# RaptorMai/online-continual-learning

Measured on AMD Instinct MI355X. Metric: replay-step images/sec (SCR, Split-CIFAR100-shaped synthetic stream, Reduced-ResNet18, mem_size 5000), higher is better.
Workload: dtype f32; 1 GPU; BASELINE.json configs[1]: agent=SCR, data=cifar100, eps_mem_batch=100, head=mlp, mem_size=5000, retrieve=random, temp=0.07, update=random; stream_batch=10, parallelism=1 independent stream(s), one per GPU

## Files before the change

include/ocl_hip.h:

```cpp
#ifndef OCL_HIP_H
#define OCL_HIP_H

#include <stdint.h>

#ifdef __cplusplus
extern "C" {
#endif

#define OCL_OK 0
#define OCL_ERR_ARG (-1)
#define OCL_ERR_HIP (-2)
#define OCL_ERR_STATE (-3)
#define OCL_ERR_UNSUPPORTED (-4)

int ocl_version(void);
const char* ocl_last_error(void);
int ocl_init(int device);

int ocl_gather_rows(const void* src, const int64_t* idx, int64_t n, int64_t row_bytes, void* dst,
                    void* stream);
int ocl_scatter_rows(void* dst, const int64_t* idx, int64_t n, int64_t row_bytes, const void* src,
                     void* stream);
int ocl_gather_rows_pair(const void* src_a, int64_t row_bytes_a, void* dst_a, const void* src_b, int64_t row_bytes_b, void* dst_b,
                         const int64_t* idx_host, int64_t* idx_dev, int64_t n, void* stream);
// ... 101 lines not shown
                    const float* gamma, int64_t m_per_group, int groups, int c, float* dy, float* dgamma,
                    float* dbeta, int accumulate, double* scratch, void* stream);

#define OCL_EPI_STATS 1
#define OCL_EPI_AFFINE 2
#define OCL_EPI_RES 4
#define OCL_EPI_RESMASK 8
#define OCL_EPI_RELU 16
#define OCL_EPI_ACCUM 32
#define OCL_EPI_BNB 64

typedef struct {
    int32_t cin, cout, k, stride, hin, win;
    int32_t n, groups, dir, merge, xf, bnb;
    int32_t force_mt, force_nt, force_pipe, force_q4, force_cs, force_cw;
} ocl_test_conv_desc;
typedef struct {
    int32_t family, mt, nt, q4, pipe, wres, ncls, pf, bnb_room, grid_x, grid_y, reserved;
} ocl_test_conv_form;
int ocl_test_conv_plan(const ocl_test_conv_desc* desc, ocl_test_conv_form* forms, int cap);
typedef struct {
    const float* in;
    const float* w;
    float* out;
    int32_t flags;
    int32_t xf;
    const float *scale, *shift, *res, *resmask;
    void* stats;
    const void* xf_stats;
    const float *xf_gamma, *xf_beta;
    float *xf_save_mean, *xf_save_invstd, *xf_running_mean, *xf_running_var;
    int64_t* xf_nbt;
    const float *bnb_y, *bnb_z, *bnb_mean, *bnb_invstd, *bnb_gamma, *bnb_beta;
} ocl_test_conv_ops;
int ocl_test_conv(const ocl_test_conv_desc* desc, const ocl_test_conv_ops* ops, ocl_test_conv_form* forms, int cap, void* stream);

typedef struct {
    int32_t cin, cout, k, stride, hin, win, n, xf_groups, wg_target, reserved;
} ocl_test_wgrad_desc;
typedef struct {
    int32_t mtw, ntw, q_rgw, pf, multi, s, grid_x, grid_y;
} ocl_test_wgrad_form;
typedef struct {
    const float* x;
    const float* dy;
    float* grad;
    int32_t xf;
    int32_t reserved;
    const float *xf_mean, *xf_invstd, *xf_gamma, *xf_beta;
} ocl_test_wgrad_ops;
int ocl_test_wgrad(const ocl_test_wgrad_desc* descs, const ocl_test_wgrad_ops* ops, int n_layers, int multi, int accumulate,
                   ocl_test_wgrad_form* forms, void* stream);

typedef struct {
    const float* y; float* z; const float* res; const void* stats;
    const float *gamma, *beta; float *running_mean, *running_var; int64_t* nbt; float *save_mean, *save_invstd;
    const float *frozen_mean, *frozen_var;
    const float* yb; const void* stats_b; const float *gamma_b, *beta_b; float *running_mean_b, *running_var_b; int64_t* nbt_b;
    float *save_mean_b, *save_invstd_b; const float *frozen_mean_b, *frozen_var_b;
    int64_t m_per_group; int32_t groups, c, relu; float momentum, eps; int32_t reserved;
} ocl_test_bn_fwd_args;
int ocl_test_bn_fwd(const ocl_test_bn_fwd_args* a, void* stream);
typedef struct {
    const float* dz; const float* z;
    const float* y[2]; const float* mean[2]; const float* invstd[2]; const float* gamma[2]; const float* beta[2];
    float* dy[2]; float* dgamma[2]; float* dbeta[2];
    int64_t m_per_group; int32_t groups, c, nsets, accumulate, frozen, mask_from_y, one_pass, reserved;
} ocl_test_bn_bwd_args;
int ocl_test_bn_bwd(const ocl_test_bn_bwd_args* a, void* stream);
int ocl_test_bn_apply_e(const float* d, const float* y, const float* mean, const float* invstd, const float* gamma, const void* esums,
                        int64_t m_per_group, int groups, int c, float* dy, float* dgamma, float* dbeta, int accumulate, void* stream);

typedef struct {
    int32_t layer, dir, wg_merged, reserved;
    ocl_test_conv_desc desc;
    ocl_test_conv_form form;
    ocl_test_wgrad_desc wdesc;
    ocl_test_wgrad_form wform;
} ocl_test_net_form;
int ocl_test_net_forms(int hw, int nf, int n, int groups, int train, ocl_test_net_form* out, int cap);

enum {
    OCL_SOP_ROWS = 0, OCL_SOP_PAIR = 1, OCL_SOP_U8 = 2, OCL_SOP_SGD = 3, OCL_SOP_COSINE = 4, OCL_SOP_CE = 5, OCL_SOP_CE_SEG = 6,
    OCL_SOP_KD = 7, OCL_SOP_MIR = 8, OCL_SOP_SUPCON = 9, OCL_SOP_KNN = 10, OCL_SOP_COL_REDUCE = 11, OCL_SOP_ASER = 12,
    OCL_SOP_ARGSORT = 13, OCL_SOP_NCM_MEANS = 14, OCL_SOP_NCM_PREDICT = 15, OCL_SOP_GEMM = 16
};
enum {
    OCL_PATH_ROWS_COPY16 = 1,
    OCL_PATH_ROWS_COPY16_YCAP = 2,
    OCL_PATH_ROWS_COPY4 = 3,
    OCL_PATH_ROWS_COPY4_YCAP = 4,
    OCL_PATH_PAIR_FUSED = 5,
    OCL_PATH_PAIR_FUSED_BLOOP = 6,
    OCL_PATH_PAIR_FALLBACK = 7,
    OCL_PATH_U8_GATHER = 8,
    OCL_PATH_SGD_VEC = 9,
    OCL_PATH_SGD_TAIL = 10,
    OCL_PATH_SGD_GRID_CAP = 11,
    OCL_PATH_SGD_REFUSED = 12,
    OCL_PATH_COS_VEC_ONE = 13,
    OCL_PATH_COS_VEC_MULTI = 14,
    OCL_PATH_COS_VEC_CAP = 15,
    OCL_PATH_COS_SCALAR_ONE = 16,
    OCL_PATH_COS_SCALAR_MULTI = 17,
// ... 51 lines not shown
```

online-continual-learning_amd/csrc/conv.h:

```cpp
#pragma once
#include "common.h"
#include <vector>

namespace ocl {

constexpr int kStatReps = 8;

struct alignas(16) StatCell {
    unsigned long long lo;
    long long hi;
};

enum ConvEpi : int {
    EPI_STORE = 0,
    EPI_STATS = 1,
    EPI_AFFINE = 2,
    EPI_RES = 4,
    EPI_RESMASK = 8,
    EPI_RELU = 16,
    EPI_ACCUM = 32,
    EPI_BNB = 64,
};

struct ConvArgs {
// ... 22 lines not shown
    int n_splits;
    const float* wT;
    int C4tot, WPT;
    int Qc, Qpad;
    int QS, nstage, wres;
    int pipe;
    int aligned;
    int cls_pack, cls_oyx;
    unsigned m_tpg, m_tpi, m_lw, m_ppi, m_kc4, m_pc, m_pr;
    int xf;
    int patch_floats;
    int qstat_off;
    const StatCell* xf_stats;
    int64_t xf_rep_stride;
    int64_t xf_m_per_group;
    const float* xf_gamma;
    const float* xf_beta;
    float* xf_save_mean;
    float* xf_save_invstd;
    float* xf_running_mean;
    float* xf_running_var;
    int64_t* xf_nbt;
    float xf_momentum, xf_eps;
    const float* bnb_y;
    const float* bnb_z;
    const float* bnb_mean;
    const float* bnb_invstd;
    const float* bnb_gamma;
    const float* bnb_beta;
    int bnb_lds;
    const int* blob;
    int off_tdesc, off_pu, off_loc, blob_ints;
    unsigned long long* trace;
};

struct ConvPlan {
    ConvArgs a;
    int cs;
    int cw;
    int q4;
    int MT, NT;
    int grid_x, grid_y;
    size_t lds_bytes;
    hipEvent_t ready;
    hipStream_t ready_stream;
};

struct ConvGeomDesc {
    int N, groups;
    int Hin, Win, Cin;
    int Hout, Wout, Cout;
    int LH, LW, os, oy0, ox0, is;
    int ntaps;
    int tdy[9], tdx[9], tw[9];
    int force_MT, force_NT, force_bpc;
    int force_cs;
    int force_q4;
    int force_pipe;
    int force_cw;
    int WPT;
    int xf;
    int bnb;
    int ncls;
    int cls_ntaps[4], cls_oy[4], cls_ox[4];
};

// ... 111 lines not shown
constexpr int kMaxInputSegments = 8;
struct InputSegments {
    const float* x[kMaxInputSegments];
    int first[kMaxInputSegments];
    int n;
};
int launch_nchw3_to_nhwc4_segments(const InputSegments& sg, float* out, int N, int H, int W, hipStream_t s);

struct BnFwdArgs {
    const float* y;
    float* z;
    const float* res;
    const StatCell* stats;
    int64_t stat_rep_stride;
    const float* gamma;
    const float* beta;
    float* running_mean;
    float* running_var;
    int64_t* nbt;
    float* save_mean;
    float* save_invstd;
    int64_t m_per_group;
    int G, C, relu;
    float momentum, eps;
    const float* frozen_mean;
    const float* frozen_var;
    const float* yb;
    const StatCell* stats_b;
    const float *gamma_b, *beta_b;
    float *running_mean_b, *running_var_b;
    int64_t* nbt_b;
    float *save_mean_b, *save_invstd_b;
    const float *frozen_mean_b, *frozen_var_b;
};
int launch_bn_fwd(const BnFwdArgs& a, hipStream_t s);
int launch_bn_apply_saved(const float* y, const float* mean, const float* invstd, const float* gamma, const float* beta, float* z,
                          int64_t m_per_group, int G, int C, hipStream_t s);

struct BnFoldDesc {
    int64_t gamma_off, beta_off, stat_off, out_off;
    int C;
};
int launch_bn_fold(const float* params, const float* running, float* out, const BnFoldDesc* descs_dev, int n_bn, float eps,
                   hipStream_t s);

struct BnBwdArgs {
    const float* dz;
    const float* z;
    int64_t m_per_group;
    int G, C;
    int nsets;
    const float* y[2];
    const float* mean[2];
    const float* invstd[2];
    const float* gamma[2];
    float* dy[2];
    float* dgamma[2];
    float* dbeta[2];
    StatCell* sums;
    unsigned* barrier;
    StatCell* fsums;
    StatCell* fsums_b;
    int accumulate;
    unsigned* err;
    int frozen;
    int mask_from_y;
    const float* beta[2];
};
int launch_bn_bwd(const BnBwdArgs& a, hipStream_t s);
struct BnApplyEArgs {
    const float* d;
    const float* y;
    const float* mean;
    const float* invstd;
    const float* gamma;
    float* dy;
    float* dgamma;
    float* dbeta;
    const StatCell* esums;
    int64_t esums_rep_stride;
    int64_t m_per_group;
    int G, C, accumulate;
};
int launch_bn_apply_e(const BnApplyEArgs& a, hipStream_t s);
int bn_bwd_last_path();
void bn_bwd_tune(int block_cap, int unroll, int phase);
void bn_bwd_fused_enable(int on);

int launch_avgpool_fwd(const float* z, float* feat, int N, int H, int W, int C, hipStream_t s);
int launch_avgpool_bwd(const float* dfeat, float* dz, int N, int H, int W, int C, hipStream_t s);

int launch_l2norm_fwd(const float* v, float* out, float* norms, int n, int d, hipStream_t s, float* out2 = nullptr);
int launch_l2norm_bwd(const float* out, const float* norms, const float* dout, float* dv, int n, int d, hipStream_t s);
int launch_relu_bwd(const float* dy, const float* a, float* dx, int64_t n, hipStream_t s);
int launch_colsum(const float* m, int rows, int cols, float* out, int accumulate, hipStream_t s);
int launch_fill(float* p, int64_t n, float v, hipStream_t s);

ConvShape test_conv_shape(const ocl_test_conv_desc& d);
void test_conv_form(const ConvPlan& p, ocl_test_conv_form* f);
void test_wgrad_form(const WgradPlan& p, ocl_test_wgrad_form* f);

int conv_kernels_init();
int wgrad_kernels_init();
int set_deterministic_sums(int on);

}
```

online-continual-learning_amd/csrc/conv.hip:

```cpp
#include "conv_dev.h"
#include "conv_stats_dev.h"
#include <string.h>
#include <algorithm>
#include <type_traits>
#include <cmath>

namespace ocl {




static const int kMaxDevices = 64;
static int g_det_dev[kMaxDevices] = {0};
static int det_host() {
    int dev = 0;
    if (hipGetDevice(&dev) != hipSuccess || dev < 0 || dev >= kMaxDevices) return 0;
    return g_det_dev[dev];
}
int set_deterministic_sums(int on) {
    const int v = on ? 1 : 0;
    int dev = 0;
    OCL_HIP(hipGetDevice(&dev));
    OCL_REQUIRE(dev >= 0 && dev < kMaxDevices, "set_deterministic: device %d", dev);
    OCL_HIP(hipDeviceSynchronize());
// ... 516 lines not shown
                    if (pv_ok && co < a.Cout) {
                        const float4 v = make_float4(acc[mt][nt][0], acc[mt][nt][1], acc[mt][nt][2], acc[mt][nt][3]);
                        s1[mt][0] += v.x; s1[mt][1] += v.y; s1[mt][2] += v.z; s1[mt][3] += v.w;
                        s2[mt][0] = fmaf(v.x, v.x, s2[mt][0]); s2[mt][1] = fmaf(v.y, v.y, s2[mt][1]);
                        s2[mt][2] = fmaf(v.z, v.z, s2[mt][2]); s2[mt][3] = fmaf(v.w, v.w, s2[mt][3]);
                        *(float4*)(a.out + (int64_t)ooff[nt] + ct.z + co) = v;
                    }
                }
            }
        } else
#pragma unroll
        for (int nt = 0; nt < NT; ++nt) {
            const bool pv_ok = ooff[nt] >= 0;
#pragma unroll
            for (int mt = 0; mt < MT; ++mt) {
                const int co = n0 + mt * 16 + 4 * g;
                if (!pv_ok || co >= a.Cout) continue;
                float4 v = make_float4(acc[mt][nt][0], acc[mt][nt][1], acc[mt][nt][2], acc[mt][nt][3]);
                if (flags & EPI_STATS) {
                    s1[mt][0] += v.x; s1[mt][1] += v.y; s1[mt][2] += v.z; s1[mt][3] += v.w;
                    s2[mt][0] = fmaf(v.x, v.x, s2[mt][0]); s2[mt][1] = fmaf(v.y, v.y, s2[mt][1]);
                    s2[mt][2] = fmaf(v.z, v.z, s2[mt][2]); s2[mt][3] = fmaf(v.w, v.w, s2[mt][3]);
                }
                float* op = a.out + (int64_t)ooff[nt] + ct.z + co;
                if (flags & EPI_AFFINE) {
                    const float4 sc = *(const float4*)(a.scale + co), sh = *(const float4*)(a.shift + co);
                    v.x = fmaf(v.x, sc.x, sh.x); v.y = fmaf(v.y, sc.y, sh.y); v.z = fmaf(v.z, sc.z, sh.z); v.w = fmaf(v.w, sc.w, sh.w);
                }
                if (flags & EPI_RES) {
                    const float4 r = *(const float4*)(a.res + (int64_t)ooff[nt] + ct.z + co);
                    v.x += r.x; v.y += r.y; v.z += r.z; v.w += r.w;
                }
                if (flags & EPI_RESMASK) {
                    const float4 r = *(const float4*)(a.res + (int64_t)ooff[nt] + ct.z + co);
                    const float4 m = *(const float4*)(a.resmask + (int64_t)ooff[nt] + ct.z + co);
                    v.x += m.x > 0.f ? r.x : 0.f; v.y += m.y > 0.f ? r.y : 0.f; v.z += m.z > 0.f ? r.z : 0.f; v.w += m.w > 0.f ? r.w : 0.f;
                }
                if (flags & EPI_ACCUM) {
                    const float4 o = *(const float4*)op;
                    v.x += o.x; v.y += o.y; v.z += o.z; v.w += o.w;
                }
                if (BNB && (flags & EPI_BNB)) {
                    const int64_t eo = (int64_t)ooff[nt] + ct.z + co;
                    const float* t = bnt + (size_t)(d1.y * (a.Cout >> 2) + (co >> 2)) * 12;
                    bnb_apply(a, *(const float4*)t, *(const float4*)(t + 4), *(const float4*)(t + 8), eo, v, s1[mt], s2[mt]);
                }
                if (flags & EPI_RELU) {
                    v.x = fmaxf(v.x, 0.f); v.y = fmaxf(v.y, 0.f); v.z = fmaxf(v.z, 0.f); v.w = fmaxf(v.w, 0.f);
                }
                *(float4*)op = v;
            }
        }
        }
        stamp();
    }
    if ((flags & (EPI_STATS | EPI_BNB)) && run_grp >= 0) flush_stats();
    stamp();
}


template <int NTQ, int PF, int STATS, int TRACE = 0>
__global__ void __launch_bounds__(256, 2) conv_q_kernel(const ConvArgs a) {
    extern __shared__ __attribute__((aligned(16))) unsigned char lds_raw[];
    constexpr int MB = kQBlocks, COPW = 4 * MB;
    int* tdesc = (int*)lds_raw;
    int* ctab = tdesc + kMaxWgTiles * 8;
    int* qoff = ctab + 16;
    int* qrow = qoff + a.Qpad;
    float* wl = (float*)(qrow + a.Qpad);
// ... 223 lines not shown
                    float t1 = 0.f, t2 = 0.f;
#pragma unroll
                    for (int nt = 0; nt < NTQ; ++nt) {
                        const float v = ooff[nt] >= 0 ? acc[m][nt][e] : 0.f;
                        t1 += v;
                        t2 = fmaf(v, v, t2);
                    }
                    t1 = row16_sum(t1);
                    t2 = row16_sum(t2);
                    if ((lane & 15) == 0) {
                        rw[m * 4 + e] = t1;
                        rw[COPW + m * 4 + e] = t2;
                    }
                }
            if (lane < 2 * COPW) {
                const float* r0 = qrows + (size_t)(wave * 4) * 2 * COPW + lane;
                qacc[wave * 2 * COPW + lane] += (r0[0] + r0[2 * COPW]) + (r0[4 * COPW] + r0[6 * COPW]);
            }
        }
        auto epi_one = [&](int nt, int m, float (&b1)[4], float (&b2)[4]) __attribute__((always_inline)) {
            const int co = 4 * m;
            if (ooff[nt] < 0 || co >= a.Cout) return;
            float4 v = make_float4(acc[m][nt][0], acc[m][nt][1], acc[m][nt][2], acc[m][nt][3]);
            float* op = a.out + (int64_t)ooff[nt] + co;
            if (flags & EPI_AFFINE) {
                const float4 sc = *(const float4*)(a.scale + co), sh = *(const float4*)(a.shift + co);
                v.x = fmaf(v.x, sc.x, sh.x); v.y = fmaf(v.y, sc.y, sh.y); v.z = fmaf(v.z, sc.z, sh.z); v.w = fmaf(v.w, sc.w, sh.w);
            }
            if (flags & EPI_RES) {
                const float4 r = *(const float4*)(a.res + (int64_t)ooff[nt] + co);
                v.x += r.x; v.y += r.y; v.z += r.z; v.w += r.w;
            }
            if (flags & EPI_RESMASK) {
                const float4 r = *(const float4*)(a.res + (int64_t)ooff[nt] + co);
                const float4 mk = *(const float4*)(a.resmask + (int64_t)ooff[nt] + co);
                v.x += mk.x > 0.f ? r.x : 0.f; v.y += mk.y > 0.f ? r.y : 0.f; v.z += mk.z > 0.f ? r.z : 0.f; v.w += mk.w > 0.f ? r.w : 0.f;
            }
            if (flags & EPI_ACCUM) {
                const float4 o = *(const float4*)op;
                v.x += o.x; v.y += o.y; v.z += o.z; v.w += o.w;
            }
            if (STATS == 2 && (flags & EPI_BNB)) {
                const float* t = bnt + (size_t)(d1.y * (a.Cout >> 2) + m) * 12;
                bnb_apply(a, *(const float4*)t, *(const float4*)(t + 4), *(const float4*)(t + 8), (int64_t)ooff[nt] + co, v, b1, b2);
            }
            if (flags & EPI_RELU) {
                v.x = fmaxf(v.x, 0.f); v.y = fmaxf(v.y, 0.f); v.z = fmaxf(v.z, 0.f); v.w = fmaxf(v.w, 0.f);
            }
            *(float4*)op = v;
        };
        if (STATS == 2 && (flags & EPI_BNB)) {
            float* rw = qrows + (size_t)(wave * 4 + (lane >> 4)) * 2 * COPW;
#pragma unroll
            for (int m = 0; m < MB; ++m) {
                float b1[4] = {0.f, 0.f, 0.f, 0.f}, b2[4] = {0.f, 0.f, 0.f, 0.f};
#pragma unroll
                for (int nt = 0; nt < NTQ; ++nt) epi_one(nt, m, b1, b2);
#pragma unroll
                for (int e = 0; e < 4; ++e) {
                    const float r1 = row16_sum(b1[e]), r2 = row16_sum(b2[e]);
                    if ((lane & 15) == 0) {
                        rw[m * 4 + e] = r1;
                        rw[COPW + m * 4 + e] = r2;
                    }
                }
            }
            if (lane < 2 * COPW) {
                const float* r0 = qrows + (size_t)(wave * 4) * 2 * COPW + lane;
                qacc[wave * 2 * COPW + lane] += (r0[0] + r0[2 * COPW]) + (r0[4 * COPW] + r0[6 * COPW]);
// ... 220 lines not shown
        const float* rj = patch0 + (size_t)(wave * 64 + lane) * 4;
        const size_t ws = (size_t)a.patch_floats;
        const float4 p0 = *(const float4*)(rj), p1 = *(const float4*)(rj + ws);
        const float4 p2 = *(const float4*)(rj + 2 * ws), p3 = *(const float4*)(rj + 3 * ws);
        v = make_float4((p0.x + p1.x) + (p2.x + p3.x), (p0.y + p1.y) + (p2.y + p3.y), (p0.z + p1.z) + (p2.z + p3.z), (p0.w + p1.w) + (p2.w + p3.w));
    }
    int oo = ooff[0];
#pragma unroll
    for (int nt = 1; nt < NT; ++nt) oo = wave == nt ? ooff[nt] : oo;
    const int co = n0 + 4 * g;
    const bool live = oo >= 0 && co < a.Cout;
    if (flags & EPI_STATS) {
        const float4 z = live ? v : make_float4(0.f, 0.f, 0.f, 0.f);
        const float s1x = row16_sum(z.x), s1y = row16_sum(z.y), s1z = row16_sum(z.z), s1w = row16_sum(z.w);
        const float s2x = row16_sum(z.x * z.x), s2y = row16_sum(z.y * z.y), s2z = row16_sum(z.z * z.z), s2w = row16_sum(z.w * z.w);
        if (r16 < 8 && co < a.Cout) {
            const int j = r16;
            const float v = j == 0 ? s1x : j == 1 ? s1y : j == 2 ? s1z : j == 3 ? s1w : j == 4 ? s2x : j == 5 ? s2y : j == 6 ? s2z : s2w;
            StatCell* st_ = a.stats + (int64_t)((blockIdx.x + blockIdx.y + wave) % kStatReps) * a.stat_rep_stride + ((int64_t)d1.y * 2) * a.Cout + co;
            fx_add<FXM>(st_ + (j >> 2) * a.Cout + (j & 3), (double)v);
        }
    }
    float* op = a.out + (int64_t)oo + co;
    if (live) {
        if (flags & EPI_AFFINE) {
            const float4 sc = *(const float4*)(a.scale + co), sh = *(const float4*)(a.shift + co);
            v.x = fmaf(v.x, sc.x, sh.x); v.y = fmaf(v.y, sc.y, sh.y); v.z = fmaf(v.z, sc.z, sh.z); v.w = fmaf(v.w, sc.w, sh.w);
        }
        if (flags & EPI_RES) {
            const float4 r = *(const float4*)(a.res + (int64_t)oo + co);
            v.x += r.x; v.y += r.y; v.z += r.z; v.w += r.w;
        }
        if (flags & EPI_RESMASK) {
            const float4 r = *(const float4*)(a.res + (int64_t)oo + co);
            const float4 mk = *(const float4*)(a.resmask + (int64_t)oo + co);
            v.x += mk.x > 0.f ? r.x : 0.f; v.y += mk.y > 0.f ? r.y : 0.f; v.z += mk.z > 0.f ? r.z : 0.f; v.w += mk.w > 0.f ? r.w : 0.f;
        }
        if (flags & EPI_ACCUM) {
            const float4 o = *(const float4*)op;
            v.x += o.x; v.y += o.y; v.z += o.z; v.w += o.w;
        }
    }
    if (BNB && (flags & EPI_BNB)) {
        float b1[4] = {0.f, 0.f, 0.f, 0.f}, b2[4] = {0.f, 0.f, 0.f, 0.f};
        if (live) {
            const int j = d1.y * a.Cout + co;
            const float4 mu = *(const float4*)(a.bnb_mean + j);
            float4 sc = make_float4(0.f, 0.f, 0.f, 0.f), sh = sc;
            if (!a.bnb_z) {
                const float4 is = *(const float4*)(a.bnb_invstd + j), gm = *(const float4*)(a.bnb_gamma + co), bt = *(const float4*)(a.bnb_beta + co);
                bn_scale_shift(gm.x, bt.x, mu.x, is.x, sc.x, sh.x); bn_scale_shift(gm.y, bt.y, mu.y, is.y, sc.y, sh.y);
                bn_scale_shift(gm.z, bt.z, mu.z, is.z, sc.z, sh.z); bn_scale_shift(gm.w, bt.w, mu.w, is.w, sc.w, sh.w);
            }
            bnb_apply(a, sc, sh, mu, (int64_t)oo + co, v, b1, b2);
        }
        const float s1x = row16_sum(b1[0]), s1y = row16_sum(b1[1]), s1z = row16_sum(b1[2]), s1w = row16_sum(b1[3]);
        const float s2x = row16_sum(b2[0]), s2y = row16_sum(b2[1]), s2z = row16_sum(b2[2]), s2w = row16_sum(b2[3]);
        if (r16 < 8 && co < a.Cout) {
            const int j = r16;
            const float v = j == 0 ? s1x : j == 1 ? s1y : j == 2 ? s1z : j == 3 ? s1w : j == 4 ? s2x : j == 5 ? s2y : j == 6 ? s2z : s2w;
            StatCell* st_ = a.stats + (int64_t)((blockIdx.x + blockIdx.y + wave) % kStatReps) * a.stat_rep_stride + ((int64_t)d1.y * 2) * a.Cout + co;
            fx_add<FXM>(st_ + (j >> 2) * a.Cout + (j & 3), (double)v);
        }
    }
    if (!live) return;
    if (flags & EPI_RELU) {
        v.x = fmaxf(v.x, 0.f); v.y = fmaxf(v.y, 0.f); v.z = fmaxf(v.z, 0.f); v.w = fmaxf(v.w, 0.f);
    }
    *(float4*)op = v;
// ... 848 lines not shown
            a.save_mean[(int64_t)g * a.C + c] = (float)mean;
            a.save_invstd[(int64_t)g * a.C + c] = (float)invstd;
        }
    }
    if (blockIdx.x == 0 && g == 0 && a.running_mean)
        bn_running_update(a.stats, a.stat_rep_stride, a.G, a.C, M, a.momentum, a.eps, a.running_mean, a.running_var, a.nbt, tid, 256);
    float* scb = sm + 2 * a.C;
    float* shb = sm + 3 * a.C;
    if (a.yb) {
        for (int c = tid; c < a.C; c += 256) {
            double mean, var;
            bn_batch_moments(a.stats_b, a.stat_rep_stride, g, c, a.C, M, a.eps, mean, var);
            if (a.frozen_mean_b) {
                mean = (double)a.frozen_mean_b[c];
                var = (double)a.frozen_var_b[c];
            }
            const double invstd = 1.0 / sqrt(var + (double)a.eps);
            bn_scale_shift(a.gamma_b[c], a.beta_b[c], (float)mean, (float)invstd, scb[c], shb[c]);
            if (blockIdx.x == 0) {
                a.save_mean_b[(int64_t)g * a.C + c] = (float)mean;
                a.save_invstd_b[(int64_t)g * a.C + c] = (float)invstd;
            }
        }
        if (blockIdx.x == 0 && g == 0 && a.running_mean_b)
            bn_running_update(a.stats_b, a.stat_rep_stride, a.G, a.C, M, a.momentum, a.eps, a.running_mean_b, a.running_var_b, a.nbt_b, tid, 256);
    }
    __syncthreads();
    const int C4 = a.C >> 2;
    const int64_t units = a.m_per_group * C4;
    const float4* y4 = (const float4*)a.y + (int64_t)g * units;
    const float4* b4 = a.yb ? (const float4*)a.yb + (int64_t)g * units : nullptr;
    const float4* r4 = a.res ? (const float4*)a.res + (int64_t)g * units : nullptr;
    float4* z4 = (float4*)a.z + (int64_t)g * units;
    for (int64_t u = (int64_t)blockIdx.x * 256 + tid; u < units; u += (int64_t)gridDim.x * 256) {
        const int c = (int)(u % C4) * 4;
        float4 v = y4[u];
        v.x = __fmaf_rn(v.x, sc[c], sh[c]);
        v.y = __fmaf_rn(v.y, sc[c + 1], sh[c + 1]);
        v.z = __fmaf_rn(v.z, sc[c + 2], sh[c + 2]);
        v.w = __fmaf_rn(v.w, sc[c + 3], sh[c + 3]);
        if (r4) {
            const float4 r = r4[u];
            v.x += r.x; v.y += r.y; v.z += r.z; v.w += r.w;
        }
        if (b4) {
            float4 r = b4[u];
            r.x = __fmaf_rn(r.x, scb[c], shb[c]);
            r.y = __fmaf_rn(r.y, scb[c + 1], shb[c + 1]);
            r.z = __fmaf_rn(r.z, scb[c + 2], shb[c + 2]);
            r.w = __fmaf_rn(r.w, scb[c + 3], shb[c + 3]);
            v.x += r.x; v.y += r.y; v.z += r.z; v.w += r.w;
        }
        if (a.relu) {
            v.x = fmaxf(v.x, 0.f); v.y = fmaxf(v.y, 0.f); v.z = fmaxf(v.z, 0.f); v.w = fmaxf(v.w, 0.f);
        }
        z4[u] = v;
    }
}

int launch_bn_fwd(const BnFwdArgs& a, hipStream_t s) {
    const int64_t units = a.m_per_group * (a.C / 4);
    const int bx = (int)std::max<int64_t>(1, std::min<int64_t>(1024, (units + 1023) / 1024));
    ProfScope ps(PROF_BN, s);
    hipLaunchKernelGGL(bn_fwd_kernel, dim3(bx, a.G), dim3(256), (size_t)a.C * (a.yb ? 16 : 8), s, a);
    OCL_LAUNCH_CHECK();
    return OCL_OK;
}

__global__ void __launch_bounds__(256) bn_apply_saved_kernel(const float* __restrict__ y, const float* __restrict__ mean, const float* __restrict__ invstd,
                                                             const float* __restrict__ gamma, const float* __restrict__ beta, float* __restrict__ z,
                                                             int64_t m_per_group, int C) {
    const int g = blockIdx.y, C4 = C >> 2;
    const int64_t units = m_per_group * C4;
    for (int64_t u = (int64_t)blockIdx.x * 256 + threadIdx.x; u < units; u += (int64_t)gridDim.x * 256) {
        const int c = (int)(u % C4) * 4;
        float4 v = ((const float4*)y)[(int64_t)g * units + u];
        float o[4] = {v.x, v.y, v.z, v.w};
#pragma unroll
        for (int e = 0; e < 4; ++e) {
            float sc, sh;
            bn_scale_shift(gamma[c + e], beta[c + e], mean[(int64_t)g * C + c + e], invstd[(int64_t)g * C + c + e], sc, sh);
            o[e] = fmaxf(__fmaf_rn(o[e], sc, sh), 0.f);
        }
        ((float4*)z)[(int64_t)g * units + u] = make_float4(o[0], o[1], o[2], o[3]);
    }
}
int launch_bn_apply_saved(const float* y, const float* mean, const float* invstd, const float* gamma, const float* beta, float* z,
                          int64_t m_per_group, int G, int C, hipStream_t s) {
    const int64_t units = m_per_group * (C / 4);
    const int bx = (int)std::max<int64_t>(1, std::min<int64_t>(1024, (units + 1023) / 1024));
    hipLaunchKernelGGL(bn_apply_saved_kernel, dim3(bx, G), dim3(256), 0, s, y, mean, invstd, gamma, beta, z, m_per_group, C);
    OCL_LAUNCH_CHECK();
    return OCL_OK;
}

__global__ void __launch_bounds__(256) bn_fold_kernel(const float* __restrict__ params, const float* __restrict__ running,
                                                      float* __restrict__ out, const BnFoldDesc* __restrict__ descs, float eps) {
    const BnFoldDesc d = descs[blockIdx.x];
    for (int c = threadIdx.x; c < d.C; c += 256) {
        const float rm = running[d.stat_off + c], rv = running[d.stat_off + d.C + c];
        const float invstd = (float)(1.0 / sqrt((double)rv + (double)eps));
        const float scale = params[d.gamma_off + c] * invstd;
        out[d.out_off + c] = scale;
        out[d.out_off + d.C + c] = params[d.beta_off + c] - rm * scale;
    }
}
int launch_bn_fold(const float* params, const float* running, float* out, const BnFoldDesc* descs_dev, int n_bn, float eps,
                   hipStream_t s) {
    ProfScope ps(PROF_BN, s);
    hipLaunchKernelGGL(bn_fold_kernel, dim3(n_bn), dim3(256), 0, s, params, running, out, descs_dev, eps);
    OCL_LAUNCH_CHECK();
    return OCL_OK;
}

template <int U>
__global__ void __launch_bounds__(256) bn_bwd_reduce_kernel(const BnBwdArgs a) {
    extern __shared__ __attribute__((aligned(16))) float sm[];
    const int C4 = a.C >> 2;
    const int PT = 256 / C4;
    const int tid = threadIdx.x;
    const int c4 = tid % C4, pl = tid / C4;
    const int g = blockIdx.y;
    const int64_t M = a.m_per_group;
    const int64_t per = (M + gridDim.x - 1) / gridDim.x;
    const int64_t pbeg = (int64_t)blockIdx.x * per, pend = min(M, pbeg + per);
    float4 sd[2], sx[2];
    float4 mean[2], istd[2];
#pragma unroll
    for (int k = 0; k < 2; ++k) {
        sd[k] = sx[k] = make_float4(0.f, 0.f, 0.f, 0.f);
        mean[k] = istd[k] = make_float4(0.f, 0.f, 0.f, 0.f);
    }
    if (pl < PT) {
#pragma unroll
        for (int k = 0; k < 2; ++k)
            if (k < a.nsets) {
                mean[k] = *(const float4*)(a.mean[k] + (int64_t)g * a.C + c4 * 4);
                istd[k] = *(const float4*)(a.invstd[k] + (int64_t)g * a.C + c4 * 4);
            }
        const float4* dz4 = (const float4*)a.dz + (int64_t)g * M * C4;
        const float4* z4 = a.z ? (const float4*)a.z + (int64_t)g * M * C4 : nullptr;
        const float4* y40 = (const float4*)a.y[0] + (int64_t)g * M * C4;
        const float4* y41 = a.nsets > 1 ? (const float4*)a.y[1] + (int64_t)g * M * C4 : y40;
        const int64_t step = (int64_t)PT * C4;
        const int64_t eend = pend * C4;
        int64_t e = (pbeg + pl) * C4 + c4;
        float4 msc = make_float4(0.f, 0.f, 0.f, 0.f), msh = msc;
        if (a.mask_from_y) {
            const float4 gm = *(const float4*)(a.gamma[0] + c4 * 4), bt = *(const float4*)(a.beta[0] + c4 * 4);
            bn_scale_shift(gm.x, bt.x, mean[0].x, istd[0].x, msc.x, msh.x); bn_scale_shift(gm.y, bt.y, mean[0].y, istd[0].y, msc.y, msh.y);
            bn_scale_shift(gm.z, bt.z, mean[0].z, istd[0].z, msc.z, msh.z); bn_scale_shift(gm.w, bt.w, mean[0].w, istd[0].w, msc.w, msh.w);
        }
        auto consume = [&](float4 d, float4 zz, const float4& ya, const float4& yb) __attribute__((always_inline)) {
            if (a.mask_from_y)
                zz = make_float4(__fmaf_rn(ya.x, msc.x, msh.x), __fmaf_rn(ya.y, msc.y, msh.y), __fmaf_rn(ya.z, msc.z, msh.z), __fmaf_rn(ya.w, msc.w, msh.w));
            if (z4 || a.mask_from_y) {
                d.x = zz.x > 0.f ? d.x : 0.f; d.y = zz.y > 0.f ? d.y : 0.f;
                d.z = zz.z > 0.f ? d.z : 0.f; d.w = zz.w > 0.f ? d.w : 0.f;
            }
#pragma unroll
            for (int k = 0; k < 2; ++k)
                if (k < a.nsets) {
                    const float4& y = k ? yb : ya;
                    sd[k].x += d.x; sd[k].y += d.y; sd[k].z += d.z; sd[k].w += d.w;
                    sx[k].x = fmaf(d.x, (y.x - mean[k].x) * istd[k].x, sx[k].x);
                    sx[k].y = fmaf(d.y, (y.y - mean[k].y) * istd[k].y, sx[k].y);
                    sx[k].z = fmaf(d.z, (y.z - mean[k].z) * istd[k].z, sx[k].z);
                    sx[k].w = fmaf(d.w, (y.w - mean[k].w) * istd[k].w, sx[k].w);
                }
        };
        const float4 zero4 = make_float4(0.f, 0.f, 0.f, 0.f);
        for (; e + (U - 1) * step < eend; e += U * step) {
            float4 d[U], zz[U], ya[U], yb[U];
#pragma unroll
            for (int u = 0; u < U; ++u) {
                d[u] = dz4[e + u * step];
                zz[u] = z4 ? z4[e + u * step] : zero4;
                ya[u] = y40[e + u * step];
                yb[u] = a.nsets > 1 ? y41[e + u * step] : zero4;
            }
#pragma unroll
            for (int u = 0; u < U; ++u) consume(d[u], zz[u], ya[u], yb[u]);
        }
        for (; e < eend; e += step)
            consume(dz4[e], z4 ? z4[e] : zero4, y40[e], a.nsets > 1 ? y41[e] : zero4);
    }
    float* base = sm;
    if (pl < PT) {
#pragma unroll
        for (int k = 0; k < 2; ++k)
            if (k < a.nsets) {
                *(float4*)(base + ((size_t)(k * 2 + 0) * PT + pl) * a.C + c4 * 4) = sd[k];
                *(float4*)(base + ((size_t)(k * 2 + 1) * PT + pl) * a.C + c4 * 4) = sx[k];
            }
    }
    __syncthreads();
    for (int j = tid; j < a.nsets * 2 * a.C; j += 256) {
        const int c = j % a.C, kk = j / a.C;
        double t = 0.0;
        for (int r = 0; r < PT; ++r) t += (double)base[((size_t)kk * PT + r) * a.C + c];
        const int k = kk >> 1, which = kk & 1;
        fx_add(&a.sums[(((int64_t)k * a.G + g) * 2 + which) * a.C + c], t);
    }
}

__global__ void __launch_bounds__(256) bn_bwd_apply_kernel(const BnBwdArgs a) {
    extern __shared__ __attribute__((aligned(16))) float sm[];
    const int g = blockIdx.y, tid = threadIdx.x;
    const double Md = (double)a.m_per_group;
    for (int j = tid; j < a.nsets * a.C; j += 256) {
        const int c = j % a.C, k = j / a.C;
        const StatCell cdy = a.sums[(((int64_t)k * a.G + g) * 2 + 0) * a.C + c], cdx = a.sums[(((int64_t)k * a.G + g) * 2 + 1) * a.C + c];
        const double sdy = fx_decode(cdy.hi, cdy.lo), sdx = fx_decode(cdx.hi, cdx.lo);
        float* s = sm + (size_t)k * 6 * a.C;
        const float istd = a.invstd[k][(int64_t)g * a.C + c];
        s[c] = a.frozen ? 0.f : (float)(sdy / Md);
        s[a.C + c] = a.frozen ? 0.f : (float)(sdx / Md);
        s[2 * a.C + c] = a.gamma[k][c] * istd;
        s[3 * a.C + c] = a.mean[k][(int64_t)g * a.C + c];
        s[4 * a.C + c] = istd;
        if (a.mask_from_y) {
            float sc_, sh_;
            bn_scale_shift(a.gamma[k][c], a.beta[k][c], a.mean[k][(int64_t)g * a.C + c], istd, sc_, sh_);
            s[5 * a.C + c] = sh_;
        }
        if (blockIdx.x == 0 && g == 0) {
            double dg = 0.0, db = 0.0;
            for (int gg = 0; gg < a.G; ++gg) {
                const StatCell cb = a.sums[(((int64_t)k * a.G + gg) * 2 + 0) * a.C + c], cg = a.sums[(((int64_t)k * a.G + gg) * 2 + 1) * a.C + c];
                db += fx_decode(cb.hi, cb.lo);
                dg += fx_decode(cg.hi, cg.lo);
            }
            if (a.accumulate) {
                a.dgamma[k][c] += (float)dg;
                a.dbeta[k][c] += (float)db;
            } else {
                a.dgamma[k][c] = (float)dg;
                a.dbeta[k][c] = (float)db;
            }
        }
    }
    __syncthreads();
    const int C4 = a.C >> 2;
    const int64_t units = a.m_per_group * C4;
    for (int64_t u = (int64_t)blockIdx.x * 256 + tid; u < units; u += (int64_t)gridDim.x * 256) {
        const int c = (int)(u % C4) * 4;
        const int64_t e = (int64_t)g * units + u;
        float4 d = ((const float4*)a.dz)[e];
        if (a.z) {
            const float4 zz = ((const float4*)a.z)[e];
            d.x = zz.x > 0.f ? d.x : 0.f; d.y = zz.y > 0.f ? d.y : 0.f;
            d.z = zz.z > 0.f ? d.z : 0.f; d.w = zz.w > 0.f ? d.w : 0.f;
        } else if (a.mask_from_y) {
            const float4 y = ((const float4*)a.y[0])[e];
            d.x = __fmaf_rn(y.x, sm[2 * a.C + c], sm[5 * a.C + c]) > 0.f ? d.x : 0.f;
            d.y = __fmaf_rn(y.y, sm[2 * a.C + c + 1], sm[5 * a.C + c + 1]) > 0.f ? d.y : 0.f;
            d.z = __fmaf_rn(y.z, sm[2 * a.C + c + 2], sm[5 * a.C + c + 2]) > 0.f ? d.z : 0.f;
            d.w = __fmaf_rn(y.w, sm[2 * a.C + c + 3], sm[5 * a.C + c + 3]) > 0.f ? d.w : 0.f;
        }
#pragma unroll
        for (int k = 0; k < 2; ++k)
            if (k < a.nsets) {
                const float* s = sm + (size_t)k * 6 * a.C;
                const float4 y = ((const float4*)a.y[k])[e];
                float4 o;
                o.x = s[2 * a.C + c] * (d.x - s[c] - (y.x - s[3 * a.C + c]) * s[4 * a.C + c] * s[a.C + c]);
                o.y = s[2 * a.C + c + 1] * (d.y - s[c + 1] - (y.y - s[3 * a.C + c + 1]) * s[4 * a.C + c + 1] * s[a.C + c + 1]);
                o.z = s[2 * a.C + c + 2] * (d.z - s[c + 2] - (y.z - s[3 * a.C + c + 2]) * s[4 * a.C + c + 2] * s[a.C + c + 2]);
                o.w = s[2 * a.C + c + 3] * (d.w - s[c + 3] - (y.w - s[3 * a.C + c + 3]) * s[4 * a.C + c + 3] * s[a.C + c + 3]);
                ((float4*)a.dy[k])[e] = o;
            }
    }
}

constexpr int kBnFusedThreads = 512;
constexpr int kBnFusedReps = 8;
#ifndef OCL_BN_FLAT
#define OCL_BN_FLAT 40
#endif
constexpr int kBnFusedFlat = OCL_BN_FLAT;
template <int E, int NS = 1>
__global__ void __launch_bounds__(kBnFusedThreads) bn_bwd_fused_kernel(const BnBwdArgs a) {
    __shared__ float4 red[1 + NS][kBnFusedThreads];
    __shared__ float kk[1 + NS][4 * 40];
    __shared__ bool timed_out;
    const int C4 = a.C >> 2;
    const int tid = threadIdx.x;
    if (tid == 0) timed_out = false;
    const int wpg = gridDim.x / a.G;
    const int g = blockIdx.x / wpg;
    const int S = (wpg * kBnFusedThreads / C4) * C4;
    const int gt = (blockIdx.x - g * wpg) * kBnFusedThreads + tid;
    const int c4 = gt % C4;
    const int64_t M = a.m_per_group;
    const int64_t units = M * C4;
    const float4* dz4 = (const float4*)a.dz + (int64_t)g * units;
    const float4* z4 = a.z ? (const float4*)a.z + (int64_t)g * units : nullptr;
    const bool live = g < a.G && gt < S;
    float4 d[E], xh[NS][E];
    float4 sd = make_float4(0.f, 0.f, 0.f, 0.f), sx[NS];
#pragma unroll
    for (int k = 0; k < NS; ++k) sx[k] = sd;
    if (live) {
        float4 zz[E];
#pragma unroll
        for (int e = 0; e < E; ++e) {
            const int64_t u = (int64_t)gt + (int64_t)e * S;
            const bool in = u < units;
            const int64_t uu = in ? u : 0;
            d[e] = dz4[uu];
#pragma unroll
            for (int k = 0; k < NS; ++k) xh[k][e] = ((const float4*)a.y[k] + (int64_t)g * units)[uu];
            zz[e] = z4 ? z4[uu] : make_float4(1.f, 1.f, 1.f, 1.f);
            if (!in) d[e] = make_float4(0.f, 0.f, 0.f, 0.f);
        }
        if (a.mask_from_y) {
            const float4 gm = *(const float4*)(a.gamma[0] + c4 * 4), bt = *(const float4*)(a.beta[0] + c4 * 4);
            const float4 mn = *(const float4*)(a.mean[0] + (int64_t)g * a.C + c4 * 4), is = *(const float4*)(a.invstd[0] + (int64_t)g * a.C + c4 * 4);
            float4 sc, sh;
            bn_scale_shift(gm.x, bt.x, mn.x, is.x, sc.x, sh.x); bn_scale_shift(gm.y, bt.y, mn.y, is.y, sc.y, sh.y);
            bn_scale_shift(gm.z, bt.z, mn.z, is.z, sc.z, sh.z); bn_scale_shift(gm.w, bt.w, mn.w, is.w, sc.w, sh.w);
#pragma unroll
            for (int e = 0; e < E; ++e)
                zz[e] = make_float4(__fmaf_rn(xh[0][e].x, sc.x, sh.x), __fmaf_rn(xh[0][e].y, sc.y, sh.y), __fmaf_rn(xh[0][e].z, sc.z, sh.z),
                                    __fmaf_rn(xh[0][e].w, sc.w, sh.w));
        }
#pragma unroll
        for (int e = 0; e < E; ++e) {
            d[e].x = zz[e].x > 0.f ? d[e].x : 0.f; d[e].y = zz[e].y > 0.f ? d[e].y : 0.f;
            d[e].z = zz[e].z > 0.f ? d[e].z : 0.f; d[e].w = zz[e].w > 0.f ? d[e].w : 0.f;
            sd.x += d[e].x; sd.y += d[e].y; sd.z += d[e].z; sd.w += d[e].w;
        }
#pragma unroll
        for (int k = 0; k < NS; ++k) {
            const float4 mean = *(const float4*)(a.mean[k] + (int64_t)g * a.C + c4 * 4);
            const float4 istd = *(const float4*)(a.invstd[k] + (int64_t)g * a.C + c4 * 4);
#pragma unroll
            for (int e = 0; e < E; ++e) {
                xh[k][e].x = (xh[k][e].x - mean.x) * istd.x; xh[k][e].y = (xh[k][e].y - mean.y) * istd.y;
                xh[k][e].z = (xh[k][e].z - mean.z) * istd.z; xh[k][e].w = (xh[k][e].w - mean.w) * istd.w;
                sx[k].x = fmaf(d[e].x, xh[k][e].x, sx[k].x); sx[k].y = fmaf(d[e].y, xh[k][e].y, sx[k].y);
                sx[k].z = fmaf(d[e].z, xh[k][e].z, sx[k].z); sx[k].w = fmaf(d[e].w, xh[k][e].w, sx[k].w);
            }
        }
    }
    red[0][tid] = sd;
// ... 67 lines not shown
            const float4 istd = *(const float4*)(a.invstd[k] + (int64_t)g * a.C + c4 * 4);
            const float4 sc = make_float4(gm.x * istd.x, gm.y * istd.y, gm.z * istd.z, gm.w * istd.w);
            float4* o4 = (float4*)a.dy[k] + (int64_t)g * units;
#pragma unroll
            for (int e = 0; e < E; ++e) {
                const int64_t u = (int64_t)gt + (int64_t)e * S;
                if (u < units) {
                    float4 o;
                    o.x = sc.x * (d[e].x - k1.x - xh[k][e].x * k2.x);
                    o.y = sc.y * (d[e].y - k1.y - xh[k][e].y * k2.y);
                    o.z = sc.z * (d[e].z - k1.z - xh[k][e].z * k2.z);
                    o.w = sc.w * (d[e].w - k1.w - xh[k][e].w * k2.w);
                    o4[u] = o;
                }
            }
        }
    }
}

constexpr int kBnChanThreads = 512;
template <int E, int NS>
__global__ void __launch_bounds__(kBnChanThreads) bn_bwd_chan_kernel(const BnBwdArgs a) {
    constexpr int NW = kBnChanThreads / 64;
    __shared__ double wred[1 + NS][4][NW];
    __shared__ double tot[2][1 + NS][4];
    __shared__ float kk[2][1 + NS][4];
    const int c4 = blockIdx.x, tid = threadIdx.x, lane = tid & 63, wave = tid >> 6;
    const int C4 = a.C >> 2;
    const int T = kBnChanThreads / a.G;
    const int g = tid / T, pt = tid - g * T;
    const int64_t M = a.m_per_group;
    const float4 f4z = make_float4(0.f, 0.f, 0.f, 0.f);
    const int64_t base = (int64_t)g * M * C4 + c4;
    float4 d[E], xh[NS][E], zz[E];
    float4 sd = f4z, sx[NS];
#pragma unroll
    for (int k = 0; k < NS; ++k) sx[k] = f4z;
#pragma unroll
    for (int e = 0; e < E; ++e) {
        const int64_t pix = pt + (int64_t)e * T;
        const bool in = pix < M;
        const int64_t u = base + (in ? pix : 0) * C4;
        d[e] = ((const float4*)a.dz)[u];
#pragma unroll
        for (int k = 0; k < NS; ++k) xh[k][e] = ((const float4*)a.y[k])[u];
        zz[e] = a.z ? ((const float4*)a.z)[u] : make_float4(1.f, 1.f, 1.f, 1.f);
        if (!in) d[e] = f4z;
    }
    if (a.mask_from_y) {
        const float4 gm = *(const float4*)(a.gamma[0] + c4 * 4), bt = *(const float4*)(a.beta[0] + c4 * 4);
        const float4 mn = *(const float4*)(a.mean[0] + (int64_t)g * a.C + c4 * 4), is = *(const float4*)(a.invstd[0] + (int64_t)g * a.C + c4 * 4);
        float4 sc, sh;
        bn_scale_shift(gm.x, bt.x, mn.x, is.x, sc.x, sh.x); bn_scale_shift(gm.y, bt.y, mn.y, is.y, sc.y, sh.y);
        bn_scale_shift(gm.z, bt.z, mn.z, is.z, sc.z, sh.z); bn_scale_shift(gm.w, bt.w, mn.w, is.w, sc.w, sh.w);
#pragma unroll
        for (int e = 0; e < E; ++e)
            zz[e] = make_float4(__fmaf_rn(xh[0][e].x, sc.x, sh.x), __fmaf_rn(xh[0][e].y, sc.y, sh.y), __fmaf_rn(xh[0][e].z, sc.z, sh.z),
                                __fmaf_rn(xh[0][e].w, sc.w, sh.w));
    }
#pragma unroll
    for (int e = 0; e < E; ++e) {
        d[e].x = zz[e].x > 0.f ? d[e].x : 0.f; d[e].y = zz[e].y > 0.f ? d[e].y : 0.f;
        d[e].z = zz[e].z > 0.f ? d[e].z : 0.f; d[e].w = zz[e].w > 0.f ? d[e].w : 0.f;
        sd.x += d[e].x; sd.y += d[e].y; sd.z += d[e].z; sd.w += d[e].w;
    }
#pragma unroll
    for (int k = 0; k < NS; ++k) {
        const float4 mean = *(const float4*)(a.mean[k] + (int64_t)g * a.C + c4 * 4);
        const float4 istd = *(const float4*)(a.invstd[k] + (int64_t)g * a.C + c4 * 4);
#pragma unroll
        for (int e = 0; e < E; ++e) {
            xh[k][e].x = (xh[k][e].x - mean.x) * istd.x; xh[k][e].y = (xh[k][e].y - mean.y) * istd.y;
            xh[k][e].z = (xh[k][e].z - mean.z) * istd.z; xh[k][e].w = (xh[k][e].w - mean.w) * istd.w;
            sx[k].x = fmaf(d[e].x, xh[k][e].x, sx[k].x); sx[k].y = fmaf(d[e].y, xh[k][e].y, sx[k].y);
            sx[k].z = fmaf(d[e].z, xh[k][e].z, sx[k].z); sx[k].w = fmaf(d[e].w, xh[k][e].w, sx[k].w);
        }
    }
    auto wsum = [&](float v) __attribute__((always_inline)) -> double {
        double t = (double)v;
// ... 40 lines not shown
#pragma unroll
    for (int k = 0; k < NS; ++k) {
        const float4 k2 = *(const float4*)&kk[g][1 + k][0];
        const float4 gm = *(const float4*)(a.gamma[k] + c4 * 4);
        const float4 istd = *(const float4*)(a.invstd[k] + (int64_t)g * a.C + c4 * 4);
        const float4 sc = make_float4(gm.x * istd.x, gm.y * istd.y, gm.z * istd.z, gm.w * istd.w);
#pragma unroll
        for (int e = 0; e < E; ++e) {
            const int64_t pix = pt + (int64_t)e * T;
            if (pix < M) {
                float4 o;
                o.x = sc.x * (d[e].x - k1.x - xh[k][e].x * k2.x);
                o.y = sc.y * (d[e].y - k1.y - xh[k][e].y * k2.y);
                o.z = sc.z * (d[e].z - k1.z - xh[k][e].z * k2.z);
                o.w = sc.w * (d[e].w - k1.w - xh[k][e].w * k2.w);
                ((float4*)a.dy[k])[base + pix * C4] = o;
            }
        }
    }
}

static int g_bn_bwd_cap = 0, g_bn_bwd_unroll = 0, g_bn_bwd_phase = 0;
void bn_bwd_tune(int cap, int unroll, int phase) { g_bn_bwd_cap = cap; g_bn_bwd_unroll = unroll; g_bn_bwd_phase = phase; }

static int g_bn_fused = -1;
static int g_num_cus = 0;
void bn_bwd_fused_enable(int on) { g_bn_fused = on; }

static int g_bn_bwd_last_path = 0;
int bn_bwd_last_path() { return g_bn_bwd_last_path; }

int launch_bn_bwd(const BnBwdArgs& a, hipStream_t s) {
    OCL_REQUIRE(a.nsets == 1 || a.nsets == 2, "bn_bwd: nsets=%d", a.nsets);
    const int C4 = a.C / 4, PT = 256 / C4;
    if (g_bn_fused < 0) {
        const char* e = getenv("OCL_BN_FUSED");
        g_bn_fused = e ? atoi(e) : 1;
    }
    static const bool bn_chan = [] { const char* e = getenv("OCL_BN_CHAN"); return !(e && e[0] == '0'); }();
    if (bn_chan && g_bn_fused && !a.frozen && g_bn_bwd_phase == 0 && a.G <= 2 && C4 >= 16 && a.m_per_group * a.G <= kBnChanThreads) {
        ProfScope ps(PROF_BN, s);
        g_bn_bwd_last_path = 1010 + a.nsets;
        if (a.nsets == 2) hipLaunchKernelGGL((bn_bwd_chan_kernel<1, 2>), dim3(C4), dim3(kBnChanThreads), 0, s, a);
        else hipLaunchKernelGGL((bn_bwd_chan_kernel<1, 1>), dim3(C4), dim3(kBnChanThreads), 0, s, a);
        OCL_LAUNCH_CHECK();
        return OCL_OK;
    }
    if (g_bn_fused && a.barrier && a.fsums && (a.nsets == 1 || a.fsums_b) && a.G <= 2 && a.C <= 160 && g_bn_bwd_phase == 0 && !a.frozen) {
        if (!g_num_cus) {
            int dev = 0;
            hipDeviceProp_t prop;
            OCL_HIP(hipGetDevice(&dev));
            OCL_HIP(hipGetDeviceProperties(&prop, dev));
            int b3 = 0, b6 = 0, b12 = 0, c3 = 0, c6 = 0;
            OCL_HIP(hipOccupancyMaxActiveBlocksPerMultiprocessor(&b3, bn_bwd_fused_kernel<3>, kBnFusedThreads, 0));
            OCL_HIP(hipOccupancyMaxActiveBlocksPerMultiprocessor(&b6, bn_bwd_fused_kernel<6>, kBnFusedThreads, 0));
            OCL_HIP(hipOccupancyMaxActiveBlocksPerMultiprocessor(&b12, bn_bwd_fused_kernel<12>, kBnFusedThreads, 0));
            OCL_HIP(hipOccupancyMaxActiveBlocksPerMultiprocessor(&c3, (bn_bwd_fused_kernel<3, 2>), kBnFusedThreads, 0));
            OCL_HIP(hipOccupancyMaxActiveBlocksPerMultiprocessor(&c6, (bn_bwd_fused_kernel<6, 2>), kBnFusedThreads, 0));
            if (std::min(std::min(b3, std::min(b6, b12)), std::min(c3, c6)) < 1) g_bn_fused = 0;
            g_num_cus = std::max(2, prop.multiProcessorCount);
        }
        const int64_t total_units = a.m_per_group * C4 * a.G;
        const int per_thread = a.nsets == 2 ? 5 : 6;
        int grid = (int)std::min<int64_t>(g_num_cus, std::max<int64_t>(8, (total_units + kBnFusedThreads * per_thread - 1) / (kBnFusedThreads * per_thread)));
        grid = std::max(a.G, grid / a.G * a.G);
// ... 1 lines not shown
        const int64_t S = (int64_t)(wpg * kBnFusedThreads / C4) * C4;
        const int64_t need = (a.m_per_group * C4 + S - 1) / S;
        if (a.nsets == 2 && need <= 6 && g_bn_fused) {
            ProfScope ps(PROF_BN, s);
            BnBwdArgs af = a;
            af.err = async_error_word_device();
            g_bn_bwd_last_path = 2000 + (need <= 3 ? 30 : 60) + 2;
            if (need <= 3) hipLaunchKernelGGL((bn_bwd_fused_kernel<3, 2>), dim3(grid), dim3(kBnFusedThreads), 0, s, af);
            else hipLaunchKernelGGL((bn_bwd_fused_kernel<6, 2>), dim3(grid), dim3(kBnFusedThreads), 0, s, af);
            OCL_LAUNCH_CHECK();
            return OCL_OK;
        }
        if (a.nsets == 1 && need <= 12 && g_bn_fused) {
            ProfScope ps(PROF_BN, s);
            BnBwdArgs af = a;
            af.err = async_error_word_device();
            g_bn_bwd_last_path = 2000 + (need <= 3 ? 30 : need <= 6 ? 60 : 120) + 1;
            if (need <= 3) hipLaunchKernelGGL(bn_bwd_fused_kernel<3>, dim3(grid), dim3(kBnFusedThreads), 0, s, af);
            else if (need <= 6) hipLaunchKernelGGL(bn_bwd_fused_kernel<6>, dim3(grid), dim3(kBnFusedThreads), 0, s, af);
            else hipLaunchKernelGGL(bn_bwd_fused_kernel<12>, dim3(grid), dim3(kBnFusedThreads), 0, s, af);
            OCL_LAUNCH_CHECK();
            return OCL_OK;
        }
    }
    const int U = g_bn_bwd_unroll ? g_bn_bwd_unroll : 4;
    const int passes = g_bn_bwd_cap > 1024 ? (g_bn_bwd_cap > 2048 ? 2 : 4) : (g_bn_bwd_cap == 0 && a.m_per_group / PT < 1024 ? 4 : 8);
    const int cap = g_bn_bwd_cap ? g_bn_bwd_cap : 1024;
    const int64_t per_block_pixels = (int64_t)PT * passes;
    const int bx = (int)std::max<int64_t>(1, std::min<int64_t>(std::max(1, cap / a.G), (a.m_per_group + per_block_pixels - 1) / per_block_pixels));
    ProfScope ps(PROF_BN, s);
    g_bn_bwd_last_path = 3000 + a.nsets;
    const size_t sm1 = (size_t)a.nsets * 2 * PT * a.C * 4;
    if (g_bn_bwd_phase != 2) {
        if (U == 1) hipLaunchKernelGGL(bn_bwd_reduce_kernel<1>, dim3(bx, a.G), dim3(256), sm1, s, a);
        else if (U == 2) hipLaunchKernelGGL(bn_bwd_reduce_kernel<2>, dim3(bx, a.G), dim3(256), sm1, s, a);
        else hipLaunchKernelGGL(bn_bwd_reduce_kernel<4>, dim3(bx, a.G), dim3(256), sm1, s, a);
        OCL_LAUNCH_CHECK();
    }
    if (g_bn_bwd_phase == 1) return OCL_OK;
    const int64_t units = a.m_per_group * C4;
    const int bx2 = (int)std::max<int64_t>(1, std::min<int64_t>(1024, (units + 1023) / 1024));
    hipLaunchKernelGGL(bn_bwd_apply_kernel, dim3(bx2, a.G), dim3(256), (size_t)a.nsets * 6 * a.C * 4, s, a);
    OCL_LAUNCH_CHECK();
    return OCL_OK;
}

__global__ void __launch_bounds__(256) bn_bwd_apply_e_kernel(const BnApplyEArgs a) {
    extern __shared__ __attribute__((aligned(16))) float sm[];
    const int g = blockIdx.y, tid = threadIdx.x;
    const double Md = (double)a.m_per_group;
    for (int c = tid; c < a.C; c += 256) {
        const float istd = a.invstd[(int64_t)g * a.C + c];
        double s1, s2;
        fx_total2(a.esums, a.esums_rep_stride, ((int64_t)g * 2 + 0) * a.C + c, ((int64_t)g * 2 + 1) * a.C + c, s1, s2);
        sm[c] = (float)(s1 / Md);
        sm[a.C + c] = (float)(s2 * (double)istd / Md);
        sm[2 * a.C + c] = a.gamma[c] * istd;
        sm[3 * a.C + c] = a.mean[(int64_t)g * a.C + c];
        sm[4 * a.C + c] = istd;
        if (blockIdx.x == 0 && g == 0) {
            double dg = 0.0, db = 0.0;
            for (int gg = 0; gg < a.G; ++gg) {
                double t1, t2;
                fx_total2(a.esums, a.esums_rep_stride, ((int64_t)gg * 2 + 0) * a.C + c, ((int64_t)gg * 2 + 1) * a.C + c, t1, t2);
                db += t1;
                dg += t2 * (double)a.invstd[(int64_t)gg * a.C + c];
            }
// ... 131 lines not shown
    OCL_LAUNCH_CHECK();
    return OCL_OK;
}

__global__ void __launch_bounds__(256) colsum_kernel(const float* __restrict__ m, int rows, int cols, float* __restrict__ out,
                                                     int accumulate) {
    __shared__ float red[8][33];
    const int cl = threadIdx.x & 31, rl = threadIdx.x >> 5;
    const int c = blockIdx.x * 32 + cl;
    float s = 0.f;
    if (c < cols)
        for (int r = rl; r < rows; r += 8) s += m[(int64_t)r * cols + c];
    red[rl][cl] = s;
    __syncthreads();
    if (rl == 0 && c < cols) {
        const float v = ((red[0][cl] + red[1][cl]) + (red[2][cl] + red[3][cl])) + ((red[4][cl] + red[5][cl]) + (red[6][cl] + red[7][cl]));
        out[c] = accumulate ? out[c] + v : v;
    }
}
int launch_colsum(const float* m, int rows, int cols, float* out, int accumulate, hipStream_t s) {
    ProfScope ps(PROF_HEAD, s);
    hipLaunchKernelGGL(colsum_kernel, dim3(cdiv(cols, 32)), dim3(256), 0, s, m, rows, cols, out, accumulate);
    OCL_LAUNCH_CHECK();
    return OCL_OK;
}

__global__ void __launch_bounds__(256) fill_kernel(float* __restrict__ p, int64_t n, float v) {
    for (int64_t i = (int64_t)blockIdx.x * 256 + threadIdx.x; i < n; i += (int64_t)gridDim.x * 256) p[i] = v;
}
int launch_fill(float* p, int64_t n, float v, hipStream_t s) {
    if (n <= 0) return OCL_OK;
    ProfScope ps(PROF_HEAD, s);
    hipLaunchKernelGGL(fill_kernel, dim3((unsigned)std::min<int64_t>(1024, (n + 255) / 256)), dim3(256), 0, s, p, n, v);
    OCL_LAUNCH_CHECK();
    return OCL_OK;
}

int conv_kernels_init() {
    static bool done_dev[kMaxDevices] = {false};
    int dev = 0;
    OCL_HIP(hipGetDevice(&dev));
    OCL_REQUIRE(dev >= 0 && dev < kMaxDevices, "conv_kernels_init: device %d", dev);
    bool& done = done_dev[dev];
    if (done) return OCL_OK;
    {
        const char* e = getenv("OCL_DETERMINISTIC");
        if (e && e[0] == '1') {
            int rc = set_deterministic_sums(1);
            if (rc != OCL_OK) return rc;
        }
    }
    if (int rc = wgrad_kernels_init()) return rc;
    if (int rc = convw_kernels_init()) return rc;
    for (int m = 1; m <= 5; ++m)
        for (int n = 1; n <= 2; ++n)
            for (int pf = 4; pf <= 8; pf += 4)
                for (int res = 0; res < 2; ++res)
                    OCL_HIP(hipFuncSetAttribute((const void*)convt_fn(m, n, pf, res), hipFuncAttributeMaxDynamicSharedMemorySize, (int)kLdsLimit));
    for (int m = 1; m <= 5; ++m)
        for (int pf = 4; pf <= 8; pf += 4)
            for (int res = 0; res < 2; ++res)
                OCL_HIP(hipFuncSetAttribute((const void*)convt_fn(m, 1, pf, res, 1), hipFuncAttributeMaxDynamicSharedMemorySize, (int)kLdsLimit));
    for (int m = 1; m <= 5; ++m)
        for (int pf = 4; pf <= 8; pf += 4)
            for (int cls = 0; cls < 2; ++cls)
                OCL_HIP(hipFuncSetAttribute((const void*)convt_fn(m, 1, pf, 0, cls, 1), hipFuncAttributeMaxDynamicSharedMemorySize, (int)kLdsLimit));
// ... 25 lines not shown
```

online-continual-learning_amd/csrc/conv_dev.h:

```cpp
#pragma once
#include "conv.h"

namespace ocl {

static const size_t kLdsLimit = 160 * 1024;
static const size_t kLdsTarget = 72 * 1024;
constexpr int kQBlocks = 5;

__device__ __forceinline__ int fdiv(int u, int d, float inv, int& rem) {
    int q = (int)((float)u * inv);
    int r = u - q * d;
    if (r < 0) { --q; r += d; }
    else if (r >= d) { ++q; r -= d; }
    rem = r;
    return q;
}

typedef unsigned int u32x4 __attribute__((ext_vector_type(4)));
constexpr int kOob = 0x7fffffff;
__device__ __forceinline__ __amdgpu_buffer_rsrc_t make_rsrc(const void* p) {
    return __builtin_amdgcn_make_buffer_rsrc(const_cast<void*>(p), 0, 0x7ffffff0, 0x00020000);
}
__device__ __forceinline__ float4 buf_load16(__amdgpu_buffer_rsrc_t r, int byte_off) {
    const u32x4 v = __builtin_amdgcn_raw_buffer_load_b128(r, byte_off, 0, 0);
    return make_float4(__uint_as_float(v.x), __uint_as_float(v.y), __uint_as_float(v.z), __uint_as_float(v.w));
}

__device__ __forceinline__ int tap_sel(const int (&tab)[9], int t) {
    int v = tab[0];
#pragma unroll
    for (int i = 1; i < 9; ++i) v = (t == i) ? tab[i] : v;
    return v;
}

constexpr int kPatchPF = 8;
constexpr int kConvPatchPF = 8;

__device__ __forceinline__ void bn_scale_shift(float gamma, float beta, float mean, float invstd, float& sc, float& sh) {
    sc = gamma * invstd;
    sh = __fmaf_rn(-mean, sc, beta);
}

}
```

online-continual-learning_amd/csrc/convw.hip:

```cpp
#include "conv_stats_dev.h"
#include <string.h>
#include <stdlib.h>
#include <algorithm>
#include <vector>
#include <type_traits>

namespace ocl {

constexpr int kWNU = 16;
constexpr int kWWaves = 4;
constexpr int kWOob = (int)0x80010000;

__host__ __device__ constexpr int wunit_pack(int go16, int c4, int pr, int pc, int il) { return go16 | (c4 << 13) | (pr << 19) | (pc << 23) | (il << 29); }

__device__ __forceinline__ void lds_dma16(__amdgpu_buffer_rsrc_t rs, float* lds_dst, int voff) {
    __builtin_amdgcn_raw_ptr_buffer_load_lds(rs, (__attribute__((address_space(3))) void*)lds_dst, 16, voff, 0, 0, 0);
}

#ifndef OCL_CW_FAKE_B
#define OCL_CW_FAKE_B 0
#endif
#ifndef OCL_CW_SGB
#define OCL_CW_SGB 1
#endif
// ... 313 lines not shown
                        if (pv_ok && co < a.Cout) {
                            const float4 v = make_float4(acc[0][mt][nt][0], acc[0][mt][nt][1], acc[0][mt][nt][2], acc[0][mt][nt][3]);
                            s1[mt][0] += v.x; s1[mt][1] += v.y; s1[mt][2] += v.z; s1[mt][3] += v.w;
                            s2[mt][0] = fmaf(v.x, v.x, s2[mt][0]); s2[mt][1] = fmaf(v.y, v.y, s2[mt][1]);
                            s2[mt][2] = fmaf(v.z, v.z, s2[mt][2]); s2[mt][3] = fmaf(v.w, v.w, s2[mt][3]);
                            *(float4*)(a.out + (int64_t)ooff[nt] + co) = v;
                        }
                    }
                }
            } else
#pragma unroll
            for (int nt = 0; nt < NT; ++nt) {
                const bool pv_ok = ooff[nt] >= 0;
#pragma unroll
                for (int mt = 0; mt < MT; ++mt) {
                    const int co = n0 + mt * 16 + 4 * g;
                    if (!pv_ok || co >= a.Cout) continue;
                    float4 v = make_float4(acc[0][mt][nt][0], acc[0][mt][nt][1], acc[0][mt][nt][2], acc[0][mt][nt][3]);
                    if (flags & EPI_STATS) {
                        s1[mt][0] += v.x; s1[mt][1] += v.y; s1[mt][2] += v.z; s1[mt][3] += v.w;
                        s2[mt][0] = fmaf(v.x, v.x, s2[mt][0]); s2[mt][1] = fmaf(v.y, v.y, s2[mt][1]);
                        s2[mt][2] = fmaf(v.z, v.z, s2[mt][2]); s2[mt][3] = fmaf(v.w, v.w, s2[mt][3]);
                    }
                    float* op = a.out + (int64_t)ooff[nt] + co;
                    if (flags & EPI_AFFINE) {
                        const float4 sc = *(const float4*)(a.scale + co), sh = *(const float4*)(a.shift + co);
                        v.x = fmaf(v.x, sc.x, sh.x); v.y = fmaf(v.y, sc.y, sh.y); v.z = fmaf(v.z, sc.z, sh.z); v.w = fmaf(v.w, sc.w, sh.w);
                    }
                    if (flags & EPI_RES) {
                        const float4 r = *(const float4*)(a.res + (int64_t)ooff[nt] + co);
                        v.x += r.x; v.y += r.y; v.z += r.z; v.w += r.w;
                    }
                    if (flags & EPI_RESMASK) {
                        const float4 r = *(const float4*)(a.res + (int64_t)ooff[nt] + co);
                        const float4 m = *(const float4*)(a.resmask + (int64_t)ooff[nt] + co);
                        v.x += m.x > 0.f ? r.x : 0.f; v.y += m.y > 0.f ? r.y : 0.f; v.z += m.z > 0.f ? r.z : 0.f; v.w += m.w > 0.f ? r.w : 0.f;
                    }
                    if (flags & EPI_ACCUM) {
                        const float4 o = *(const float4*)op;
                        v.x += o.x; v.y += o.y; v.z += o.z; v.w += o.w;
                    }
                    if (BNB && (flags & EPI_BNB)) {
                        const int64_t eo = (int64_t)ooff[nt] + co;
                        const float* tq = bnt + (size_t)(t_grp * (a.Cout >> 2) + (co >> 2)) * 12;
                        bnb_apply(a, *(const float4*)tq, *(const float4*)(tq + 4), *(const float4*)(tq + 8), eo, v, s1[mt], s2[mt]);
                    }
                    if (flags & EPI_RELU) {
                        v.x = fmaxf(v.x, 0.f); v.y = fmaxf(v.y, 0.f); v.z = fmaxf(v.z, 0.f); v.w = fmaxf(v.w, 0.f);
                    }
                    *(float4*)op = v;
                }
            }
            cur_c = 0;
            ++cur_t;
        } else {
            ++cur_c;
        }
        stamp();
    }
    if (flags & (EPI_STATS | EPI_BNB)) {
        double* slot = (double*)patch;
#pragma unroll
        for (int mt = 0; mt < MT; ++mt)
#pragma unroll
            for (int e = 0; e < 4; ++e) {
                const float x = row16_sum(s1[mt][e]), y = row16_sum(s2[mt][e]);
                if (r16 == 0) {
                    slot[mt * 16 + 4 * g + e] = (double)x;
                    slot[COPW + mt * 16 + 4 * g + e] = (double)y;
// ... 329 lines not shown
                        const int co = n0 + mt * 16 + 4 * g;
                        if (co < a.Cout) {
                            const float4 v = make_float4(acc[0][mt][nt][0], acc[0][mt][nt][1], acc[0][mt][nt][2], acc[0][mt][nt][3]);
                            s1[mt][0] += v.x; s1[mt][1] += v.y; s1[mt][2] += v.z; s1[mt][3] += v.w;
                            s2[mt][0] = fmaf(v.x, v.x, s2[mt][0]); s2[mt][1] = fmaf(v.y, v.y, s2[mt][1]);
                            s2[mt][2] = fmaf(v.z, v.z, s2[mt][2]); s2[mt][3] = fmaf(v.w, v.w, s2[mt][3]);
                            *(float4*)(a.out + (int64_t)ooff[nt] + co) = v;
                        }
                    }
                }
            } else
#pragma unroll
            for (int nt = 0; nt < NT; ++nt) {
#pragma unroll
                for (int mt = 0; mt < MT; ++mt) {
                    const int co = n0 + mt * 16 + 4 * g;
                    if (co >= a.Cout) continue;
                    float4 v = make_float4(acc[0][mt][nt][0], acc[0][mt][nt][1], acc[0][mt][nt][2], acc[0][mt][nt][3]);
                    if (flags & EPI_STATS) {
                        s1[mt][0] += v.x; s1[mt][1] += v.y; s1[mt][2] += v.z; s1[mt][3] += v.w;
                        s2[mt][0] = fmaf(v.x, v.x, s2[mt][0]); s2[mt][1] = fmaf(v.y, v.y, s2[mt][1]);
                        s2[mt][2] = fmaf(v.z, v.z, s2[mt][2]); s2[mt][3] = fmaf(v.w, v.w, s2[mt][3]);
                    }
                    float* op = a.out + (int64_t)ooff[nt] + co;
                    if (flags & EPI_AFFINE) {
                        const float4 sc = *(const float4*)(a.scale + co), sh = *(const float4*)(a.shift + co);
                        v.x = fmaf(v.x, sc.x, sh.x); v.y = fmaf(v.y, sc.y, sh.y); v.z = fmaf(v.z, sc.z, sh.z); v.w = fmaf(v.w, sc.w, sh.w);
                    }
                    if (flags & EPI_RES) {
                        const float4 r = *(const float4*)(a.res + (int64_t)ooff[nt] + co);
                        v.x += r.x; v.y += r.y; v.z += r.z; v.w += r.w;
                    }
                    if (flags & EPI_RESMASK) {
                        const float4 r = *(const float4*)(a.res + (int64_t)ooff[nt] + co);
                        const float4 m = *(const float4*)(a.resmask + (int64_t)ooff[nt] + co);
                        v.x += m.x > 0.f ? r.x : 0.f; v.y += m.y > 0.f ? r.y : 0.f; v.z += m.z > 0.f ? r.z : 0.f; v.w += m.w > 0.f ? r.w : 0.f;
                    }
                    if (flags & EPI_ACCUM) {
                        const float4 o = *(const float4*)op;
                        v.x += o.x; v.y += o.y; v.z += o.z; v.w += o.w;
                    }
                    if (BNB && (flags & EPI_BNB)) {
                        const int64_t eo = (int64_t)ooff[nt] + co;
                        const float* tq = bnt + (size_t)(t_grp * (a.Cout >> 2) + (co >> 2)) * 12;
                        bnb_apply(a, *(const float4*)tq, *(const float4*)(tq + 4), *(const float4*)(tq + 8), eo, v, s1[mt], s2[mt]);
                    }
                    if (flags & EPI_RELU) {
                        v.x = fmaxf(v.x, 0.f); v.y = fmaxf(v.y, 0.f); v.z = fmaxf(v.z, 0.f); v.w = fmaxf(v.w, 0.f);
                    }
                    *(float4*)op = v;
                }
            }
            cur_c = 0;
            ++cur_t;
        } else {
            ++cur_c;
        }
        stamp();
    };
    for (int j = 0; j < n_items; j += 2) {
        item(std::integral_constant<int, 0>());
        if (j + 1 < n_items) item(std::integral_constant<int, 1>());
    }
    if (flags & (EPI_STATS | EPI_BNB)) {
        double* slot = (double*)patch;
#pragma unroll
        for (int mt = 0; mt < MT; ++mt)
#pragma unroll
            for (int e = 0; e < 4; ++e) {
// ... 264 lines not shown
```

online-continual-learning_amd/csrc/layer_api.hip:

```cpp
#include "conv.h"
#include <string.h>
#include <algorithm>
#include <vector>

using namespace ocl;

namespace ocl {

ConvShape test_conv_shape(const ocl_test_conv_desc& d) {
    ConvShape s;
    memset(&s, 0, sizeof(s));
    s.Cin = d.cin; s.CinT = d.cin == 3 ? 4 : d.cin; s.Cout = d.cout; s.k = d.k; s.stride = d.stride;
    s.Hin = d.hin; s.Win = d.win;
    const int pad = d.k == 3 ? 1 : 0;
    s.Ho = (d.hin + 2 * pad - d.k) / d.stride + 1;
    s.Wo = (d.win + 2 * pad - d.k) / d.stride + 1;
    s.CoutP = pack_width(d.cout);
    s.CiP = d.cin == 3 ? 0 : pack_width(d.cin);
    return s;
}

static int test_conv_geoms(const ocl_test_conv_desc& d, std::vector<ConvGeomDesc>* out) {
    OCL_REQUIRE(d.n > 0 && d.groups > 0 && (d.k == 1 || d.k == 3) && (d.stride == 1 || d.stride == 2) && d.hin > 0 && d.win > 0 &&
                    (d.cin == 3 || d.cin % 4 == 0) && d.cout % 4 == 0 && (d.dir == 0 || d.dir == 1),
// ... 111 lines not shown
    OCL_REQUIRE(!(o->flags & EPI_BNB) || (d.bnb && d.dir == 1 && o->bnb_y && o->bnb_mean && o->bnb_invstd && o->bnb_gamma && o->bnb_beta),
                "test_conv: EPI_BNB without its reservation / operands");
    int rc = conv_kernels_init();
    if (rc != OCL_OK) return rc;
    std::vector<ConvGeomDesc> gs;
    if ((rc = test_conv_geoms(d, &gs)) != OCL_OK) return rc;
    const ConvShape c = test_conv_shape(d);
    hipStream_t s = (hipStream_t)stream;
    Scratch sc;
    sc.s = s;
    PackDesc pd;
    memset(&pd, 0, sizeof(pd));
    pd.w_off = 0; pd.Cout = c.Cout; pd.Cin = c.Cin; pd.ntaps = c.k * c.k; pd.CinP = c.CinT; pd.CoutP = c.CoutP; pd.CiP = c.CiP;
    const size_t pack_floats = d.dir == 0 ? (size_t)pd.ntaps * c.CinT * c.CoutP : (size_t)pd.ntaps * c.Cout * c.CiP;
    pd.tf_off = d.dir == 0 ? 0 : -1;
    pd.td_off = d.dir == 0 ? -1 : 0;
    float* pack = (float*)sc.take((pack_floats + 65536) * 4, 0);
    PackDesc* pd_dev = (PackDesc*)sc.take(sizeof(PackDesc), 0);
    if (!pack || !pd_dev) { set_error("test_conv: out of device memory"); return OCL_ERR_HIP; }
    OCL_HIP(hipMemsetD32Async((hipDeviceptr_t)(pack + pack_floats), 0x45800000, 65536, s));
    OCL_HIP(hipMemcpyAsync(pd_dev, &pd, sizeof(pd), hipMemcpyHostToDevice, s));
    if ((rc = launch_pack_weights(o->w, pack, pd_dev, 1, c.Cout * c.Cin * pd.ntaps, s, d.dir == 0 ? PACK_TF : PACK_TD)) != OCL_OK) return rc;
    for (size_t i = 0; i < gs.size(); ++i) {
        ConvPlan p;
        if ((rc = plan_conv(gs[i], &p)) != OCL_OK) return rc;
        if ((int)i < cap && forms) test_conv_form(p, &forms[i]);
        if ((rc = conv_plan_finalize(&p, nullptr, s)) != OCL_OK) {
            conv_plan_release(&p);
            return rc;
        }
        ConvPlan q = p;
        ConvArgs& a = q.a;
        a.in = o->in; a.wT = pack; a.out = o->out; a.flags = o->flags;
        a.scale = o->scale; a.shift = o->shift; a.res = o->res; a.resmask = o->resmask;
        a.stats = (StatCell*)o->stats;
        a.stat_rep_stride = (int64_t)gs[i].groups * 2 * (d.dir == 0 ? c.Cout : c.Cin);
        if (o->xf) {
            a.xf = 1;
            a.xf_stats = (const StatCell*)o->xf_stats;
            a.xf_rep_stride = (int64_t)d.groups * 2 * c.Cin;
            a.xf_m_per_group = (int64_t)(d.n / d.groups) * c.Hin * c.Win;
            a.xf_gamma = o->xf_gamma; a.xf_beta = o->xf_beta;
            a.xf_save_mean = o->xf_save_mean; a.xf_save_invstd = o->xf_save_invstd;
            a.xf_running_mean = o->xf_running_mean; a.xf_running_var = o->xf_running_var; a.xf_nbt = o->xf_nbt;
            a.xf_momentum = 0.1f; a.xf_eps = 1e-5f;
        }
        if (o->flags & EPI_BNB) {
            if (a.bnb_lds < 0) {
                conv_plan_release(&p);
                set_error("test_conv: plan has no room for the BatchNorm-backward epilogue");
                return OCL_ERR_STATE;
            }
            a.bnb_y = o->bnb_y; a.bnb_z = o->bnb_z; a.bnb_mean = o->bnb_mean; a.bnb_invstd = o->bnb_invstd;
            a.bnb_gamma = o->bnb_gamma; a.bnb_beta = o->bnb_beta;
        }
        rc = launch_conv(q, s);
        if (rc == OCL_OK && hipStreamSynchronize(s) != hipSuccess) rc = OCL_ERR_HIP;
        conv_plan_release(&p);
        if (rc != OCL_OK) return rc;
    }
    return (int)gs.size();
}

int ocl_test_wgrad(const ocl_test_wgrad_desc* descs, const ocl_test_wgrad_ops* ops, int n_layers, int multi, int accumulate,
                   ocl_test_wgrad_form* forms, void* stream) {
    OCL_REQUIRE(descs && n_layers >= 1 && n_layers <= kMaxReduceLayers && n_layers <= kMaxWgradMulti, "test_wgrad: %d layers", n_layers);
    std::vector<WgradPlan> plans((size_t)n_layers);
// ... 39 lines not shown
        memset(&m, 0, sizeof(m));
        m.partial = partial;
        m.grads = ops[0].grad;
        m.accumulate = accumulate;
        m.n = n_layers;
        for (int i = 0; i < n_layers; ++i) {
            OCL_REQUIRE(ops[i].grad >= ops[0].grad, "test_wgrad: multi wants the layers' gradients in one array, the first layer's first");
            wgrad_reduce_layer(plans[i], off[i], ops[i].grad - ops[0].grad, &m.L[i]);
        }
        if (rc == OCL_OK) rc = launch_wgrad_reduce_multi(m, s);
        (void)hipStreamSynchronize(s);
        wgrad_multi_release(&t);
        if (rc != OCL_OK) return rc;
    }
    OCL_HIP(hipStreamSynchronize(s));
    return OCL_OK;
}

int ocl_test_bn_fwd(const ocl_test_bn_fwd_args* t, void* stream) {
    OCL_REQUIRE(t && t->y && t->z && t->stats && t->gamma && t->beta && t->save_mean && t->save_invstd, "test_bn_fwd: null pointer");
    OCL_REQUIRE(t->groups >= 1 && t->c % 4 == 0 && t->m_per_group > 0, "test_bn_fwd: bad sizes");
    int rc = conv_kernels_init();
    if (rc != OCL_OK) return rc;
    BnFwdArgs a;
    memset(&a, 0, sizeof(a));
    a.y = t->y; a.z = t->z; a.res = t->res; a.stats = (const StatCell*)t->stats; a.stat_rep_stride = (int64_t)t->groups * 2 * t->c;
    a.gamma = t->gamma; a.beta = t->beta; a.running_mean = t->running_mean; a.running_var = t->running_var; a.nbt = t->nbt;
    a.save_mean = t->save_mean; a.save_invstd = t->save_invstd;
    a.m_per_group = t->m_per_group; a.G = t->groups; a.C = t->c; a.relu = t->relu; a.momentum = t->momentum; a.eps = t->eps;
    a.frozen_mean = t->frozen_mean; a.frozen_var = t->frozen_var;
    a.yb = t->yb; a.stats_b = (const StatCell*)t->stats_b; a.gamma_b = t->gamma_b; a.beta_b = t->beta_b;
    a.running_mean_b = t->running_mean_b; a.running_var_b = t->running_var_b; a.nbt_b = t->nbt_b;
    a.save_mean_b = t->save_mean_b; a.save_invstd_b = t->save_invstd_b; a.frozen_mean_b = t->frozen_mean_b; a.frozen_var_b = t->frozen_var_b;
    hipStream_t s = (hipStream_t)stream;
    if ((rc = launch_bn_fwd(a, s)) != OCL_OK) return rc;
    OCL_HIP(hipStreamSynchronize(s));
    return OCL_OK;
}

int ocl_test_bn_bwd(const ocl_test_bn_bwd_args* t, void* stream) {
    OCL_REQUIRE(t && t->dz && (t->nsets == 1 || t->nsets == 2) && t->groups >= 1 && t->c % 4 == 0 && t->m_per_group > 0, "test_bn_bwd: bad arguments");
    for (int k = 0; k < t->nsets; ++k)
        OCL_REQUIRE(t->y[k] && t->mean[k] && t->invstd[k] && t->gamma[k] && t->dy[k] && t->dgamma[k] && t->dbeta[k], "test_bn_bwd: null pointer (set %d)", k);
    OCL_REQUIRE(!t->mask_from_y || (t->nsets == 1 && !t->z && t->beta[0]), "test_bn_bwd: mask_from_y wants one set, no z, beta");
    int rc = conv_kernels_init();
    if (rc != OCL_OK) return rc;
    hipStream_t s = (hipStream_t)stream;
    Scratch sc;
    sc.s = s;
    BnBwdArgs a;
    memset(&a, 0, sizeof(a));
    a.dz = t->dz; a.z = t->z; a.m_per_group = t->m_per_group; a.G = t->groups; a.C = t->c; a.nsets = t->nsets;
    for (int k = 0; k < 2; ++k) {
        a.y[k] = t->y[k]; a.mean[k] = t->mean[k]; a.invstd[k] = t->invstd[k]; a.gamma[k] = t->gamma[k]; a.beta[k] = t->beta[k];
        a.dy[k] = t->dy[k]; a.dgamma[k] = t->dgamma[k]; a.dbeta[k] = t->dbeta[k];
    }
    a.accumulate = t->accumulate; a.frozen = t->frozen; a.mask_from_y = t->mask_from_y;
    const size_t cells = (size_t)t->nsets * t->groups * 2 * t->c;
    a.sums = (StatCell*)sc.take(cells * sizeof(StatCell), 0);
    if (t->one_pass) {
        const size_t fcells = (size_t)8 * 2 * 2 * t->c;
        a.fsums = (StatCell*)sc.take((fcells + 8) * sizeof(StatCell), 0);
        if (a.fsums) a.barrier = (unsigned*)(a.fsums + fcells);
        if (t->nsets == 2) a.fsums_b = (StatCell*)sc.take((fcells + 8) * sizeof(StatCell), 0);
    }
    if (!a.sums || (t->one_pass && (!a.fsums || !a.barrier || (t->nsets == 2 && !a.fsums_b)))) {
        set_error("test_bn_bwd: out of device memory");
        return OCL_ERR_HIP;
    }
    if ((rc = launch_bn_bwd(a, s)) != OCL_OK) return rc;
    OCL_HIP(hipStreamSynchronize(s));
    return bn_bwd_last_path();
}

int ocl_test_bn_apply_e(const float* d, const float* y, const float* mean, const float* invstd, const float* gamma, const void* esums,
                        int64_t m_per_group, int groups, int c, float* dy, float* dgamma, float* dbeta, int accumulate, void* stream) {
    OCL_REQUIRE(d && y && mean && invstd && gamma && esums && dy && dgamma && dbeta, "test_bn_apply_e: null pointer");
    int rc = conv_kernels_init();
    if (rc != OCL_OK) return rc;
    BnApplyEArgs a;
    memset(&a, 0, sizeof(a));
    a.d = d; a.y = y; a.mean = mean; a.invstd = invstd; a.gamma = gamma; a.dy = dy; a.dgamma = dgamma; a.dbeta = dbeta;
    a.esums = (const StatCell*)esums; a.esums_rep_stride = (int64_t)groups * 2 * c;
    a.m_per_group = m_per_group; a.G = groups; a.C = c; a.accumulate = accumulate;
    hipStream_t s = (hipStream_t)stream;
    if ((rc = launch_bn_apply_e(a, s)) != OCL_OK) return rc;
    OCL_HIP(hipStreamSynchronize(s));
    return OCL_OK;
}

int ocl_set_deterministic(int on) { return set_deterministic_sums(on); }

}
```

online-continual-learning_amd/csrc/net.hip:

```cpp
#include "conv.h"
#include <chrono>
#include <string.h>
#include <stdlib.h>
#include <string>
#include <vector>
#include <map>
#include <algorithm>
#include <tuple>
#include <array>

using namespace ocl;

namespace {

const int kGmax = 8;

struct TensorInfo {
    std::string name;
    int64_t off;
    int ndim;
    int64_t shape[4];
    int64_t numel;
};
struct BnInfo {
    std::string name;
    int C;
    int gamma_t, beta_t;
    int64_t stat_off;
    int64_t arena_off;
    int64_t fused_off;
    int64_t save_off;
};
struct ConvInfo : ConvShape {
    int w_t;
    int bn;
    int64_t tf_off, td_off;
    int64_t y_off;
    int xf_src;
};
struct BlockInfo {
    int conv1, conv2, convs;
    int64_t a1_off, z_off;
};

struct PlanSet {
    std::vector<ConvPlan> fwd;
    std::vector<std::vector<ConvPlan>> dgrad;
    std::vector<WgradPlan> wgrad;
    std::vector<int64_t> partial_off;
    bool batched_reduce = false;
    std::vector<char> dgrad_bnb;
    std::vector<int> wgrad_target;
};

}

struct ocl_net {
    ocl_net_desc d;
    std::vector<TensorInfo> tensors;
    std::vector<BnInfo> bns;
    std::vector<ConvInfo> convs;
    std::vector<BlockInfo> blocks;
    int64_t n_params = 0, n_stats = 0;
    int feat_dim = 0, out_dim = 0, Hf = 0, Wf = 0;
    int t_linear_w = -1, t_linear_b = -1, t_h0_w = -1, t_h0_b = -1, t_h2_w = -1, t_h2_b = -1;

    int64_t ws_bytes = 0;
    int64_t slot_bytes = 0, slot_base = 0;
    int64_t x4_off = 0, zstem_off = 0, save_off_base = 0, feat_off = 0, h1_off = 0, h2_off = 0, norms_off = 0, out_off = 0;
    int64_t slot_floats = 0;
    int64_t gbuf_floats = 0;
    int64_t off_g[5] = {0, 0, 0, 0, 0};
    static const int kDyRing = 6;
    int64_t off_dy[6] = {0, 0, 0, 0, 0, 0};
    static const int kDyKeep = 24;
    int64_t off_dykeep = 0, dykeep_floats = 0;
    int64_t off_partial = 0, partial_floats = 0;
    int64_t off_stats = 0, stats_doubles = 0, stats_rep_stride = 0;
    int64_t off_bsums = 0, bsums_doubles = 0;
    int64_t off_pack = 0, pack_floats = 0;
    int64_t off_fold = 0, fold_floats = 0;
    int64_t off_descs = 0;
    int64_t off_head = 0, head_floats = 0;
    int64_t max_act_floats = 0;

    float* params = nullptr;
    float* grads = nullptr;
    float* running = nullptr;
    int64_t* nbt = nullptr;
    unsigned char* ws = nullptr;
    bool bound = false;
    bool descs_uploaded = false;
    const float* pack_src = nullptr;
    int pack_have = 0;
    hipStream_t pack_stream = nullptr;
    bool bsums_clean = false;
    int pack_need_fwd = 0, pack_need_bwd = 0;

    int dbg_stop = -1;
    float* dbg_role[5] = {nullptr, nullptr, nullptr, nullptr, nullptr};
    std::vector<int> slot_n, slot_groups;
// ... 142 lines not shown

    int64_t pk = 0;
    for (auto& cv : n->convs) {
        cv.CoutP = pack_width(cv.Cout);
        cv.tf_off = pk;
        pk += (int64_t)cv.k * cv.k * cv.CinT * cv.CoutP;
        if (cv.Cin != 3) {
            cv.CiP = pack_width(cv.Cin);
            pk = align_up(pk, 64);
            cv.td_off = pk;
            pk += (int64_t)cv.k * cv.k * cv.Cout * cv.CiP;
        } else {
            cv.CiP = 0;
            cv.td_off = -1;
        }
        pk = align_up(pk, 64);
    }
    n->pack_floats = pk;

    const int64_t N = d.max_batch;
    int64_t o = 0;
    auto take = [&](int64_t nfl) {
        const int64_t r = o;
        o = align_up(o + nfl, 64);
        return r;
    };
    n->x4_off = take(N * d.in_h * d.in_w * 4);
    int64_t max_act = N * d.in_h * d.in_w * 4;
    for (auto& cv : n->convs) {
        const int64_t sz = N * cv.Ho * cv.Wo * cv.Cout;
        cv.y_off = take(sz);
        max_act = std::max(max_act, sz);
    }
    n->zstem_off = take(N * n->convs[0].Ho * n->convs[0].Wo * n->convs[0].Cout);
    for (auto& b : n->blocks) {
        const ConvInfo& c1 = n->convs[b.conv1];
        const int64_t sz = N * c1.Ho * c1.Wo * c1.Cout;
        b.a1_off = take(sz);
        b.z_off = take(sz);
    }
    n->save_off_base = o;
    for (auto& b : n->bns) {
        b.save_off = take((int64_t)2 * kGmax * b.C);
    }
    n->feat_off = take(N * n->feat_dim);
    n->h1_off = take(N * n->feat_dim);
    n->h2_off = take(N * std::max(n->out_dim, 1));
    n->norms_off = take(N);
    n->out_off = take(N * n->out_dim);
    n->slot_floats = o;
    n->max_act_floats = max_act;

    int64_t w = 0;
    auto takeb = [&](int64_t bytes) {
        const int64_t r = w;
        w = align_up(w + bytes, 256);
        return r;
    };
    n->gbuf_floats = max_act;
    for (int i = 0; i < 5; ++i) n->off_g[i] = takeb(max_act * 4);
    for (int i = 0; i < ocl_net::kDyRing; ++i) n->off_dy[i] = takeb(max_act * 4);
    n->dykeep_floats = align_up(max_act, 64);
    n->off_dykeep = takeb(n->dykeep_floats * 4 * ocl_net::kDyKeep);
    int64_t pmax = 0;
    for (auto& cv : n->convs) {
        WgradPlan wp;
        int rc = plan_wgrad((int)N, cv.Hin, cv.Win, cv.CinT, cv.Ho, cv.Wo, cv.Cout, cv.k, cv.stride, &wp);
        if (rc != OCL_OK) return rc;
        pmax = std::max<int64_t>(pmax, (int64_t)wp.partial_floats);
    }
    n->partial_floats = std::max<int64_t>(pmax, (int64_t)(64ll << 20) / 4) + 1024;
    n->off_partial = takeb(n->partial_floats * 4);
// ... 147 lines not shown
        fd[i].out_off = n->bns[i].stat_off;
        fd[i].C = n->bns[i].C;
    }
    unsigned char* dst = n->ws + n->off_descs;
    OCL_HIP(hipMemcpyAsync(dst, pd.data(), pd.size() * sizeof(PackDesc), hipMemcpyHostToDevice, s));
    OCL_HIP(hipMemcpyAsync(dst + align_up((int64_t)(pd.size() * sizeof(PackDesc)), 64), fd.data(), fd.size() * sizeof(BnFoldDesc),
                           hipMemcpyHostToDevice, s));
    OCL_HIP(hipMemsetAsync(n->ws + n->off_pack, 0, n->pack_floats * 4, s));
    OCL_HIP(hipStreamSynchronize(s));
    n->descs_uploaded = true;
    return OCL_OK;
}
static const PackDesc* pack_descs(const ocl_net* n) { return (const PackDesc*)(n->ws + n->off_descs); }
static const BnFoldDesc* fold_descs(const ocl_net* n) {
    return (const BnFoldDesc*)(n->ws + n->off_descs + align_up((int64_t)(n->convs.size() * sizeof(PackDesc)), 64));
}

struct BnbEpi {
    const float *y, *z, *mean, *invstd, *gamma, *beta;
    StatCell* sums;
    int64_t rep_stride;
};

struct XfBn {
    const StatCell* stats;
    const float *gamma, *beta;
    float *save_mean, *save_invstd, *running_mean, *running_var;
    int64_t* nbt;
    int64_t m_per_group;
};

static int run_conv(ocl_net* n, ConvPlan& cached, const float* in, const float* wT, float* out, int flags, StatCell* stats,
                    const float* scale, const float* shift, const float* res, const float* resmask, hipStream_t s, const XfBn* xf = nullptr,
                    const BnbEpi* be = nullptr) {
    if (!cached.a.blob) {
        int rc = conv_plan_finalize(&cached, &n->plan_arena, s);
        if (rc != OCL_OK) return rc;
    }
    if (cached.ready && s != cached.ready_stream && !n->capturing) OCL_HIP(hipStreamWaitEvent(s, cached.ready, 0));
    ConvPlan p = cached;
    if (xf) {
        p.a.xf = 1;
        p.a.xf_stats = xf->stats;
        p.a.xf_rep_stride = n->stats_rep_stride;
        p.a.xf_m_per_group = xf->m_per_group;
        p.a.xf_gamma = xf->gamma; p.a.xf_beta = xf->beta;
        p.a.xf_save_mean = xf->save_mean; p.a.xf_save_invstd = xf->save_invstd;
        p.a.xf_running_mean = xf->running_mean; p.a.xf_running_var = xf->running_var; p.a.xf_nbt = xf->nbt;
        p.a.xf_momentum = 0.1f; p.a.xf_eps = 1e-5f;
    }
    p.a.stat_rep_stride = n->stats_rep_stride;
    p.a.in = in;
    p.a.wT = wT;
    p.a.out = out;
    p.a.flags = flags;
    p.a.stats = stats;
    p.a.scale = scale;
    p.a.shift = shift;
    p.a.res = res;
    p.a.resmask = resmask;
    if (be) {
        if (p.a.bnb_lds < 0) {
            set_error("run_conv: plan has no room for the BatchNorm-backward epilogue");
            return OCL_ERR_STATE;
        }
        p.a.flags |= EPI_BNB;
        p.a.stats = be->sums;
        p.a.stat_rep_stride = be->rep_stride;
        p.a.bnb_y = be->y; p.a.bnb_z = be->z;
        p.a.bnb_mean = be->mean; p.a.bnb_invstd = be->invstd; p.a.bnb_gamma = be->gamma; p.a.bnb_beta = be->beta;
    }
    return launch_conv(p, s);
}

static int head_forward(ocl_net* n, const float* P, float* feat, float* h1, float* h2, float* norms, float* out, int N,
                        hipStream_t s, float* out2, bool* wrote_out2) {
    const int FD = n->feat_dim;
    auto T = [&](int t) { return P + n->tensors[t].off; };
    int rc = OCL_OK;
    switch (n->d.head) {
        case 0:
            rc = ocl_gemm_small(feat, FD, 1, T(n->t_linear_w), 1, FD, out, n->out_dim, N, n->out_dim, FD, T(n->t_linear_b), 0, 0, s);
            break;
        case 1:
            rc = ocl_gemm_small(feat, FD, 1, T(n->t_h0_w), 1, FD, h1, FD, N, FD, FD, T(n->t_h0_b), 1, 0, s);
            if (rc) return rc;
            rc = ocl_gemm_small(h1, FD, 1, T(n->t_h2_w), 1, FD, h2, n->out_dim, N, n->out_dim, FD, T(n->t_h2_b), 0, 0, s);
            if (rc) return rc;
            rc = launch_l2norm_fwd(h2, out, norms, N, n->out_dim, s, out2);
            *wrote_out2 = true;
            break;
        case 2:
            rc = ocl_gemm_small(feat, FD, 1, T(n->t_h2_w), 1, FD, h2, n->out_dim, N, n->out_dim, FD, T(n->t_h2_b), 0, 0, s);
            if (rc) return rc;
            rc = launch_l2norm_fwd(h2, out, norms, N, n->out_dim, s, out2);
            *wrote_out2 = true;
            break;
        default:
            rc = launch_l2norm_fwd(feat, out, norms, N, FD, s, out2);
            *wrote_out2 = true;
            break;
    }
    return rc;
}

static const int kSideExtraMinBatch = [] { const char* e = getenv("OCL_SIDE_EXTRA_MIN"); return e ? atoi(e) : 96; }();

static int ensure_side_stream(ocl_net* n) {
    if (n->s2) return OCL_OK;
    {
        int lo = 0, hi = 0;
        OCL_HIP(hipDeviceGetStreamPriorityRange(&lo, &hi));
        OCL_HIP(hipStreamCreateWithPriority(&n->s2, hipStreamNonBlocking, lo));
    }
    for (int i = 0; i < ocl_net::kDyRing; ++i) OCL_HIP(hipEventCreateWithFlags(&n->ev_done[i], hipEventDisableTiming));
    OCL_HIP(hipEventCreateWithFlags(&n->ev_join, hipEventDisableTiming));
    OCL_HIP(hipEventCreateWithFlags(&n->ev_fork, hipEventDisableTiming));
    for (int i = 0; i < 48; ++i) {
        hipEvent_t e;
        OCL_HIP(hipEventCreateWithFlags(&e, hipEventDisableTiming));
        n->ev_ready.push_back(e);
    }
    return OCL_OK;
}

static int side_wait(ocl_net* n, hipStream_t s) {
    hipEvent_t e = n->ev_ready[n->ev_next++ % n->ev_ready.size()];
    OCL_HIP(hipEventRecord(e, s));
    OCL_HIP(hipStreamWaitEvent(n->s2, e, 0));
// ... 131 lines not shown
    net->params = params;
    net->grads = grads;
    net->running = running;
    net->nbt = nbt;
    net->ws = (unsigned char*)workspace;
    net->bound = true;
    net->descs_uploaded = false;
    net->pack_src = nullptr;
    for (size_t i = 0; i < net->slot_valid.size(); ++i) net->slot_valid[i] = false;
    for (auto& kv : net->graphs)
        if (kv.second.exec) (void)hipGraphExecDestroy(kv.second.exec);
    net->graphs.clear();
    return OCL_OK;
}

}

static bool dbg_skip_bn2fwd() {
    static const bool v = [] { const char* e = getenv("OCL_DEBUG_SKIP_BN2FWD"); return e && e[0] == '1'; }();
    return v;
}
static bool dbg_skip_shortcut() {
    static const bool v = [] { const char* e = getenv("OCL_DEBUG_SKIP_SHORTCUT"); return e && e[0] == '1'; }();
    return v;
}

static int trunk_forward_train(ocl_net* n, PlanSet* ps, const float* P, float* S, int Nc, int G, bool upd, float* feat, hipStream_t st,
                               bool side = false, bool frozen = false, bool fuse = false) {
    const int img0 = 0, g0 = 0;
    float* pack = (float*)(n->ws + n->off_pack);
    StatCell* stats = n->statsbuf();
    int rc = OCL_OK;
    auto at = [&](int64_t off, const ConvInfo& c) { return S + off + (int64_t)img0 * c.Ho * c.Wo * c.Cout; };
    auto bn_fwd = [&](int conv_i, const float* y, float* z, const float* res, int relu, hipStream_t st, int conv_b = -1) -> int {
        const ConvInfo& c = n->convs[conv_i];
        const BnInfo& b = n->bns[c.bn];
        BnFwdArgs a;
        memset(&a, 0, sizeof(a));
        a.y = y; a.z = z; a.res = res;
        a.stats = stats + b.arena_off;
        a.stat_rep_stride = n->stats_rep_stride;
        a.gamma = P + n->tensors[b.gamma_t].off;
        a.beta = P + n->tensors[b.beta_t].off;
        a.running_mean = upd ? n->running + b.stat_off : nullptr;
        a.running_var = upd ? n->running + b.stat_off + b.C : nullptr;
        a.nbt = upd ? n->nbt + c.bn : nullptr;
        a.save_mean = S + b.save_off + (int64_t)g0 * b.C;
        a.save_invstd = S + b.save_off + (int64_t)kGmax * b.C + (int64_t)g0 * b.C;
        a.m_per_group = (int64_t)(Nc / G) * c.Ho * c.Wo;
        a.G = G; a.C = b.C; a.relu = relu;
        a.momentum = 0.1f; a.eps = 1e-5f;
        if (frozen) {
            a.frozen_mean = n->running + b.stat_off;
            a.frozen_var = n->running + b.stat_off + b.C;
        }
        if (conv_b >= 0) {
            const ConvInfo& cb = n->convs[conv_b];
            const BnInfo& bb = n->bns[cb.bn];
            a.yb = at(cb.y_off, cb);
            a.stats_b = stats + bb.arena_off;
            a.gamma_b = P + n->tensors[bb.gamma_t].off;
            a.beta_b = P + n->tensors[bb.beta_t].off;
            a.running_mean_b = upd ? n->running + bb.stat_off : nullptr;
            a.running_var_b = upd ? n->running + bb.stat_off + bb.C : nullptr;
            a.nbt_b = upd ? n->nbt + cb.bn : nullptr;
            a.save_mean_b = S + bb.save_off + (int64_t)g0 * bb.C;
            a.save_invstd_b = S + bb.save_off + (int64_t)kGmax * bb.C + (int64_t)g0 * bb.C;
            if (frozen) {
                a.frozen_mean_b = n->running + bb.stat_off;
                a.frozen_var_b = n->running + bb.stat_off + bb.C;
            }
        }
        return launch_bn_fwd(a, st);
    };
    auto conv_stats = [&](int conv_i, const float* in, hipStream_t st) -> int {
        const ConvInfo& c = n->convs[conv_i];
        return run_conv(n, ps->fwd[conv_i], in, pack + c.tf_off, at(c.y_off, c), EPI_STATS, stats + n->bns[c.bn].arena_off, nullptr,
                        nullptr, nullptr, nullptr, st);
    };
    const ConvInfo& c0 = n->convs[0];
    const float* x4 = S + n->x4_off + (int64_t)img0 * n->d.in_h * n->d.in_w * 4;
    if ((rc = conv_stats(0, x4, st))) return rc;
    float* cur = at(n->zstem_off, c0);
    if ((rc = bn_fwd(0, at(c0.y_off, c0), cur, nullptr, 1, st))) return rc;
    for (auto& b : n->blocks) {
        const ConvInfo& c1 = n->convs[b.conv1];
        const ConvInfo& c2 = n->convs[b.conv2];
        float* a1 = at(b.a1_off, c1);
        float* z = at(b.z_off, c2);
        const float* res = cur;
        if (b.convs >= 0) {
            hipStream_t ss = side ? n->s2 : st;
            if (side && (rc = side_wait(n, st))) return rc;
            if (!dbg_skip_shortcut() && (rc = conv_stats(b.convs, cur, ss))) return rc;
            res = nullptr;
        }
        if ((rc = conv_stats(b.conv1, cur, st))) return rc;
        if (fuse) {
            const BnInfo& b1 = n->bns[c1.bn];
            XfBn xf;
            xf.stats = stats + b1.arena_off;
            xf.gamma = P + n->tensors[b1.gamma_t].off;
            xf.beta = P + n->tensors[b1.beta_t].off;
            xf.save_mean = S + b1.save_off;
            xf.save_invstd = S + b1.save_off + (int64_t)kGmax * b1.C;
            xf.running_mean = upd ? n->running + b1.stat_off : nullptr;
            xf.running_var = upd ? n->running + b1.stat_off + b1.C : nullptr;
            xf.nbt = upd ? n->nbt + c1.bn : nullptr;
            xf.m_per_group = (int64_t)(Nc / G) * c1.Ho * c1.Wo;
            if ((rc = run_conv(n, ps->fwd[b.conv2], at(c1.y_off, c1), pack + c2.tf_off, at(c2.y_off, c2), EPI_STATS,
                               stats + n->bns[c2.bn].arena_off, nullptr, nullptr, nullptr, nullptr, st, &xf)))
                return rc;
        } else {
            if ((rc = bn_fwd(b.conv1, at(c1.y_off, c1), a1, nullptr, 1, st))) return rc;
            if ((rc = conv_stats(b.conv2, a1, st))) return rc;
        }
        if (b.convs >= 0 && side && (rc = side_join(n, st))) return rc;
        if (!(dbg_skip_bn2fwd() && &b != &n->blocks.back()) && (rc = bn_fwd(b.conv2, at(c2.y_off, c2), z, res, 1, st, b.convs))) return rc;
        cur = z;
    }
    if (!feat) return OCL_OK;
    return launch_avgpool_fwd(cur, feat, Nc, n->Hf, n->Wf, n->convs[n->blocks.back().conv2].Cout, st);
}

extern "C" {

int ocl_net_forward(ocl_net* n, const float* x, int N, int groups, uint32_t flags, const float* params_override, float* feat_out,
                    float* out, int slot, void* stream) {
    OCL_REQUIRE(x, "net_forward: null input");
    const float* xs[1] = {x};
    const int32_t ns[1] = {N};
    return ocl_net_forward_segments(n, xs, ns, 1, groups, flags, params_override, feat_out, out, slot, stream);
}

int ocl_net_forward_segments(ocl_net* n, const float* const* xs, const int32_t* ns, int nseg, int groups, uint32_t flags,
                             const float* params_override, float* feat_out, float* out, int slot, void* stream) {
    OCL_REQUIRE(n && n->bound, "net_forward: net not bound");
    if (int arc = check_async_error("net_forward")) return arc;
    OCL_REQUIRE(xs && ns && nseg >= 1 && nseg <= kMaxInputSegments, "net_forward: %d input segments (1 .. %d)", nseg, kMaxInputSegments);
    InputSegments sg;
    memset(&sg, 0, sizeof(sg));
    int N = 0;
    for (int i = 0; i < nseg; ++i) {
        OCL_REQUIRE(xs[i] && ns[i] > 0, "net_forward: segment %d is empty", i);
        sg.x[i] = xs[i];
        sg.first[i] = N;
        N += ns[i];
    }
    sg.n = nseg;
    OCL_REQUIRE(N > 0 && N <= n->d.max_batch, "net_forward: n=%d (max_batch %d)", N, n->d.max_batch);
    OCL_REQUIRE(groups >= 1 && groups <= kGmax && N % groups == 0, "net_forward: groups=%d must divide n=%d (<= %d)", groups, N, kGmax);
    OCL_REQUIRE(slot >= 0 && slot < n->d.n_slots, "net_forward: slot %d", slot);
    hipStream_t s = (hipStream_t)stream;
    const bool frozen = (flags & OCL_FWD_FROZEN_BN) != 0;
// ... 103 lines not shown
    }
    if (feat_out && !feat_direct) OCL_HIP(hipMemcpyAsync(feat_out, feat, (size_t)N * n->feat_dim * 4, hipMemcpyDeviceToDevice, s));
    if (out && want_head && !(wrote && head_out2))
        OCL_HIP(hipMemcpyAsync(out, S + n->out_off, (size_t)N * n->out_dim * 4, hipMemcpyDeviceToDevice, s));
    if (train && (flags & OCL_FWD_SAVE_TAPE) && !params_override) {
        n->slot_valid[slot] = true;
        n->slot_frozen[slot] = frozen;
        n->slot_n[slot] = N;
        n->slot_groups[slot] = groups;
    }
    return OCL_OK;
}

}

static int trunk_backward(ocl_net* n, PlanSet* ps, const float* P, float* Gr, float* S, int Nc, int G, int accumulate, const float* dfeat,
                          hipStream_t s, hipStream_t side, bool frozen = false, bool fused = false) {
    const int img0 = 0, g0 = 0;
    float* pack = (float*)(n->ws + n->off_pack);
    float* partial = n->partialbuf();
    StatCell* bsums = n->bsumsbuf();
    int rc = OCL_OK;
    if (!n->bsums_clean) OCL_HIP(hipMemsetAsync(bsums, 0, n->bsums_doubles * sizeof(StatCell), s));
    n->bsums_clean = false;
    auto T = [&](int t) { return P + n->tensors[t].off; };
    auto GT = [&](int t) { return Gr + n->tensors[t].off; };
    auto at = [&](int64_t off, const ConvInfo& c) { return S + off + (int64_t)img0 * c.Ho * c.Wo * c.Cout; };
    float* gA = n->gbuf(0);
    float* gD = n->gbuf(3);
    float* gE = n->gbuf(4);
    float* gB = nullptr;
    float* gC = nullptr;
    const int Clast = n->convs[n->blocks.back().conv2].Cout;
    if ((rc = launch_avgpool_bwd(dfeat, gA, Nc, n->Hf, n->Wf, Clast, s))) return rc;

    const bool two_streams = side != nullptr;
    hipStream_t sw = two_streams ? side : s;
    n->dy_next = 0;
    for (int i = 0; i < ocl_net::kDyRing; ++i) n->ev_done_pending[i] = false;
    const bool batched = Nc < kTwoStreamMinBatch && ps->batched_reduce && n->dbg_stop < 0;
    static const bool env_multi = [] { const char* e = getenv("OCL_WGRAD_MULTI"); return !e || e[0] != '0'; }();
    int n_dy = 1;
    for (auto& b : n->blocks) n_dy += b.convs >= 0 ? 3 : 2;
    const bool defer = env_multi && batched && !two_streams && !n->capturing && n_dy <= ocl_net::kDyKeep;
    static const bool env_keep = [] { const char* e = getenv("OCL_DY_KEEP"); return !e || e[0] != '0'; }();
    const bool keep = defer || (env_keep && two_streams && n_dy <= ocl_net::kDyKeep);
    static const int env_flush = [] { const char* e = getenv("OCL_WGRAD_FLUSH"); return e ? std::max(1, atoi(e)) : 0; }();
    const int flush_every = env_flush > 0 ? env_flush : (Nc >= 128 ? 3 : 1);
    const bool coarse = two_streams && keep && flush_every > 1;
    std::vector<WgradPlan> deferred;
    auto take_dy = [&](int* slot_out) -> float* {
        if (keep) {
            *slot_out = n->dy_next;
            return n->dykeep(n->dy_next++);
        }
        const int r = n->dy_next;
        n->dy_next = (r + 1) % ocl_net::kDyRing;
        if (two_streams && n->ev_done_pending[r]) {
            (void)hipStreamWaitEvent(s, n->ev_done[r], 0);
            n->ev_done_pending[r] = false;
        }
        *slot_out = r;
        return n->dybuf(r);
    };
    auto publish = [&]() -> int {
        return two_streams && !coarse ? side_wait(n, s) : OCL_OK;
    };
    auto release = [&](int r) -> int {
        if (!two_streams || keep) return OCL_OK;
        OCL_HIP(hipEventRecord(n->ev_done[r], sw));
        n->ev_done_pending[r] = true;
        return OCL_OK;
    };

    auto bn_bwd = [&](const float* dz, const float* zmask, int conv_a, float* dya, int conv_b, float* dyb, bool from_y = false) -> int {
        BnBwdArgs a;
        memset(&a, 0, sizeof(a));
        const ConvInfo& ca = n->convs[conv_a];
        a.dz = dz; a.z = zmask;
        a.mask_from_y = from_y ? 1 : 0;
        a.m_per_group = (int64_t)(Nc / G) * ca.Ho * ca.Wo;
        a.G = G; a.C = ca.Cout;
        a.nsets = conv_b >= 0 ? 2 : 1;
        const int cs[2] = {conv_a, conv_b};
        float* dys[2] = {dya, dyb};
        for (int k = 0; k < a.nsets; ++k) {
            const ConvInfo& c = n->convs[cs[k]];
            const BnInfo& b = n->bns[c.bn];
            a.y[k] = at(c.y_off, c);
            a.mean[k] = S + b.save_off + (int64_t)g0 * b.C;
            a.invstd[k] = S + b.save_off + (int64_t)kGmax * b.C + (int64_t)g0 * b.C;
            a.gamma[k] = T(b.gamma_t);
            a.beta[k] = T(b.beta_t);
            a.dy[k] = dys[k];
            a.dgamma[k] = GT(b.gamma_t);
            a.dbeta[k] = GT(b.beta_t);
        }
        a.sums = bsums + n->bns[ca.bn].arena_off;
        if (G <= 2) {
            a.fsums = bsums + n->bns[ca.bn].fused_off;
            a.barrier = (unsigned*)(a.fsums + (int64_t)8 * 2 * 2 * ca.Cout);
            if (conv_b >= 0) a.fsums_b = bsums + n->bns[n->convs[conv_b].bn].fused_off;
        }
        if (conv_b >= 0 && 2 * G > kGmax) {
            set_error("bn_bwd: groups=%d too large for a shared reduction arena", G);
            return OCL_ERR_ARG;
        }
        a.accumulate = accumulate;
        a.frozen = frozen ? 1 : 0;
        return launch_bn_bwd(a, s);
    };
    WgradReduceMulti rm;
// ... 31 lines not shown
                int r = launch_wgrad(wp, sw);
                if (r) return r;
                wgrad_reduce_layer(wp, off, n->tensors[n->convs[conv_i].w_t].off, &rm.L[rm.n++]);
                return OCL_OK;
            }
        }
        wp.a.partial = batched ? partial + ps->partial_off[conv_i] : partial;
        if (defer) {
            deferred.push_back(wp);
            wgrad_reduce_layer(wp, ps->partial_off[conv_i], n->tensors[n->convs[conv_i].w_t].off, &rm.L[rm.n++]);
            return OCL_OK;
        }
        int r = launch_wgrad(wp, sw);
        if (r) return r;
        if (batched) {
            wgrad_reduce_layer(wp, ps->partial_off[conv_i], n->tensors[n->convs[conv_i].w_t].off, &rm.L[rm.n++]);
            return OCL_OK;
        }
        return launch_wgrad_reduce(wp, GT(n->convs[conv_i].w_t), accumulate, sw);
    };
    auto flush_pending = [&]() -> int {
        if (pending.empty()) return OCL_OK;
        int r = side_wait(n, s);
        for (size_t i = 0; i < pending.size() && !r; ++i) r = wgrad_now(pending[i].conv_i, pending[i].xin, pending[i].dy, pending[i].xf_conv);
        pending.clear();
        return r;
    };
    auto wgrad = [&](int conv_i, const float* xin, const float* dy, int xf_conv = -1) -> int {
        if (!coarse) return wgrad_now(conv_i, xin, dy, xf_conv);
        pending.push_back({conv_i, xin, dy, xf_conv});
        return (int)pending.size() >= flush_every ? flush_pending() : OCL_OK;
    };
    auto dgrad = [&](int conv_i, const float* dy, float* dx, const float* res, const float* resmask, int extra_flags,
                     const BnbEpi* be = nullptr) -> int {
        const ConvInfo& c = n->convs[conv_i];
        for (auto& p : ps->dgrad[conv_i]) {
            int fl = extra_flags | (res ? (resmask ? EPI_RESMASK : EPI_RES) : 0);
            int r = run_conv(n, p, dy, pack + c.td_off, dx, fl, nullptr, nullptr, nullptr, res, resmask, s, nullptr, be);
            if (r) return r;
        }
        return OCL_OK;
    };
    auto bnb_desc = [&](int bn_conv, const float* zmask) -> BnbEpi {
        const ConvInfo& c = n->convs[bn_conv];
        const BnInfo& b = n->bns[c.bn];
        BnbEpi e;
        e.y = at(c.y_off, c);
        e.z = zmask;
        e.mean = S + b.save_off;
        e.invstd = S + b.save_off + (int64_t)kGmax * b.C;
        e.gamma = T(b.gamma_t);
        e.beta = T(b.beta_t);
        e.sums = bsums + b.fused_off;
        e.rep_stride = (int64_t)G * 2 * b.C;
        return e;
    };
    auto bn_apply_e = [&](int bn_conv, const float* d, float* dy) -> int {
        const ConvInfo& c = n->convs[bn_conv];
        const BnInfo& b = n->bns[c.bn];
        BnApplyEArgs a;
        memset(&a, 0, sizeof(a));
        a.d = d; a.y = at(c.y_off, c); a.dy = dy;
        a.mean = S + b.save_off;
        a.invstd = S + b.save_off + (int64_t)kGmax * b.C;
        a.gamma = T(b.gamma_t);
        a.dgamma = GT(b.gamma_t);
        a.dbeta = GT(b.beta_t);
        a.esums = bsums + b.fused_off;
        a.esums_rep_stride = (int64_t)G * 2 * b.C;
        a.m_per_group = (int64_t)(Nc / G) * c.Ho * c.Wo;
        a.G = G; a.C = b.C; a.accumulate = accumulate;
        return launch_bn_apply_e(a, s);
    };

    auto stop_here = [&](int bi, int step) -> bool {
        if (n->dbg_stop != bi * 10 + step) return false;
        n->dbg_role[0] = gA; n->dbg_role[1] = gB; n->dbg_role[2] = gC; n->dbg_role[3] = gD; n->dbg_role[4] = gE;
        return true;
    };
    if (stop_here(99, 0)) return OCL_OK;
    bool prev_epi = false;
    const ConvInfo& c0 = n->convs[0];
    for (int bi = (int)n->blocks.size() - 1; bi >= 0; --bi) {
        const BlockInfo& b = n->blocks[bi];
        const ConvInfo& c1 = n->convs[b.conv1];
        const ConvInfo& c2 = n->convs[b.conv2];
        const float* xin = bi == 0 ? at(n->zstem_off, c0) : at(n->blocks[bi - 1].z_off, n->convs[n->blocks[bi - 1].conv2]);
        const float* a1 = at(b.a1_off, c1);
        const float* z = at(b.z_off, c2);
        int rB, rC = -1;
        gB = take_dy(&rB);
        if (b.convs >= 0) gC = take_dy(&rC);
        if (prev_epi) {
            if ((rc = bn_apply_e(b.conv2, gA, gB))) return rc;
        } else if ((rc = bn_bwd(gA, z, b.conv2, gB, b.convs, gC))) return rc;
        prev_epi = false;
        if (stop_here(bi, 1)) return OCL_OK;
        if ((rc = publish())) return rc;
        if (b.convs >= 0) {
            if (!dbg_skip_shortcut() && (rc = wgrad(b.convs, xin, gC))) return rc;
            if ((rc = release(rC))) return rc;
        }
        if ((rc = fused ? wgrad(b.conv2, at(c1.y_off, c1), gB, b.conv1) : wgrad(b.conv2, a1, gB))) return rc;
        if ((rc = release(rB))) return rc;
        const bool epi1 = ps->dgrad_bnb[b.conv2] && !frozen && G <= 2 && n->dbg_stop < 0;
        BnbEpi be1;
        if (epi1) be1 = bnb_desc(b.conv1, fused ? nullptr : a1);
        if ((rc = dgrad(b.conv2, gB, gD, nullptr, nullptr, 0, epi1 ? &be1 : nullptr))) return rc;
        if (stop_here(bi, 2)) return OCL_OK;
        int rB1;
        float* gB1 = take_dy(&rB1);
        if (epi1) {
            if ((rc = bn_apply_e(b.conv1, gD, gB1))) return rc;
        } else if ((rc = bn_bwd(gD, fused ? nullptr : a1, b.conv1, gB1, -1, nullptr, fused))) return rc;
        gB = gB1;
        if (stop_here(bi, 3)) return OCL_OK;
        if ((rc = publish())) return rc;
        if ((rc = wgrad(b.conv1, xin, gB1))) return rc;
        if ((rc = release(rB1))) return rc;
        if (b.convs >= 0) {
            if ((rc = dgrad(b.conv1, gB1, gE, nullptr, nullptr, 0))) return rc;
            if (stop_here(bi, 4)) return OCL_OK;
            if (!dbg_skip_shortcut() && (rc = dgrad(b.convs, gC, gE, nullptr, nullptr, EPI_ACCUM))) return rc;
        } else {
            const bool single_target = bi == 0 || n->blocks[bi - 1].convs < 0;
            const bool epi2 = ps->dgrad_bnb[b.conv1] && single_target && !frozen && G <= 2 && n->dbg_stop < 0;
            BnbEpi be2;
            if (epi2) be2 = bnb_desc(bi == 0 ? 0 : n->blocks[bi - 1].conv2, xin);
            if ((rc = dgrad(b.conv1, gB1, gE, gA, z, 0, epi2 ? &be2 : nullptr))) return rc;
            prev_epi = epi2;
        }
        if (stop_here(bi, 5)) return OCL_OK;
        std::swap(gA, gE);
    }
    int rS;
    float* gS = take_dy(&rS);
    if (prev_epi) {
        if ((rc = bn_apply_e(0, gA, gS))) return rc;
    } else if ((rc = bn_bwd(gA, at(n->zstem_off, c0), 0, gS, -1, nullptr))) return rc;
    (void)rS;
    if ((rc = flush_pending())) return rc;
    if (two_streams && batched) {
        if ((rc = publish())) return rc;
        if ((rc = wgrad(0, S + n->x4_off + (int64_t)img0 * n->d.in_h * n->d.in_w * 4, gS))) return rc;
        if ((rc = flush_pending())) return rc;
        if (rm.n > 0 && (rc = launch_wgrad_reduce_multi(rm, sw))) return rc;
        OCL_HIP(hipEventRecord(n->ev_join, sw));
        OCL_HIP(hipStreamWaitEvent(s, n->ev_join, 0));
        for (int i = 0; i < ocl_net::kDyRing; ++i) n->ev_done_pending[i] = false;
        return OCL_OK;
    }
    if (two_streams) {
        if (grouped && rm.n > 0) {
            if ((rc = launch_wgrad_reduce_multi(rm, sw))) return rc;
            rm.n = 0;
        }
        WgradPlan wp = ps->wgrad[0];
        wp.a.x = S + n->x4_off + (int64_t)img0 * n->d.in_h * n->d.in_w * 4;
        wp.a.dy = gS;
        wp.a.partial = partial + stem_region / 4;
        if (stem_region / 4 + (int64_t)wp.partial_floats > n->partial_floats) wp.a.partial = nullptr;
        for (size_t i = 1; i < ps->wgrad.size(); ++i)
            if ((int64_t)ps->wgrad[i].partial_floats * 4 > (grouped ? kGroupRegion : (16ll << 20))) wp.a.partial = nullptr;
        if (wp.a.partial && !env_skip_wgrad) {
            if ((rc = launch_wgrad(wp, s))) return rc;
            if ((rc = launch_wgrad_reduce(wp, GT(n->convs[0].w_t), accumulate, s))) return rc;
        }
        OCL_HIP(hipEventRecord(n->ev_join, sw));
        OCL_HIP(hipStreamWaitEvent(s, n->ev_join, 0));
        for (int i = 0; i < ocl_net::kDyRing; ++i) n->ev_done_pending[i] = false;
        sw = s;
        if (wp.a.partial) return OCL_OK;
// ... 51 lines not shown
        OCL_HIP(hipMemcpyAsync(stage, dout, (size_t)N * OD * 4, hipMemcpyDeviceToDevice, s));
        dout = stage;
    }
    float* feat = S + n->feat_off;
    float* h1 = S + n->h1_off;
    float* o = S + n->out_off;
    float* norms = S + n->norms_off;

    static const bool env_single = [] { const char* e = getenv("OCL_SINGLE_STREAM"); return e && e[0] == '1'; }();
    const bool two_streams = n->dbg_stop < 0 && (int64_t)N * n->d.in_h * n->d.in_w >= (int64_t)kTwoStreamMinBatch * 1024 && !prof_on() && !env_single;
    if (two_streams && (rc = ensure_side_stream(n))) return rc;
    auto lin_bwd = [&](const float* dy, int ncol, const float* xin, int kin, int tw, int tb, float* dx) -> int {
        const bool hs_big = (int64_t)N * n->d.in_h * n->d.in_w >= (int64_t)kSideExtraMinBatch * 1024;
        const bool hs = two_streams && hs_big;
        hipStream_t sw = hs ? n->s2 : s;
        int r = hs ? side_wait(n, s) : OCL_OK;
        if (r) return r;
        if ((r = ocl_gemm_small(dy, 1, ncol, xin, kin, 1, GT(tw), kin, ncol, kin, N, nullptr, 0, accumulate, sw))) return r;
        if ((r = launch_colsum(dy, N, ncol, GT(tb), accumulate, sw))) return r;
        if (dx) r = ocl_gemm_small(dy, ncol, 1, T(tw), kin, 1, dx, kin, N, kin, ncol, nullptr, 0, 0, s);
        return r;
    };
    const bool fused_tape = n->slot_fused[slot];
    auto body = [&]() -> int {
        int rc = OCL_OK;
        if (repack) {
            int max_elems = 0;
            for (auto& c : n->convs) max_elems = std::max(max_elems, c.Cout * c.Cin * c.k * c.k);
            if ((rc = launch_pack_weights(P, pack, pack_descs(n), (int)n->convs.size(), max_elems, s, repack_mask))) return rc;
        }
        if (n->d.head == 0) {
            if ((rc = lin_bwd(dout, OD, feat, FD, n->t_linear_w, n->t_linear_b, dfeat))) return rc;
        } else {
            if (!accumulate) {
                if ((rc = launch_fill(GT(n->t_linear_w), n->tensors[n->t_linear_w].numel + n->tensors[n->t_linear_b].numel, 0.f, s))) return rc;
            }
            if (n->d.head == 1) {
                if ((rc = launch_l2norm_bwd(o, norms, dout, dh2, N, OD, s))) return rc;
                if ((rc = lin_bwd(dh2, OD, h1, FD, n->t_h2_w, n->t_h2_b, dh1))) return rc;
                if ((rc = launch_relu_bwd(dh1, h1, dh1, (int64_t)N * FD, s))) return rc;
                if ((rc = lin_bwd(dh1, FD, feat, FD, n->t_h0_w, n->t_h0_b, dfeat))) return rc;
            } else if (n->d.head == 2) {
                if ((rc = launch_l2norm_bwd(o, norms, dout, dh2, N, OD, s))) return rc;
                if ((rc = lin_bwd(dh2, OD, feat, FD, n->t_h2_w, n->t_h2_b, dfeat))) return rc;
            } else {
                if ((rc = launch_l2norm_bwd(o, norms, dout, dfeat, N, FD, s))) return rc;
            }
        }
        n->bsums_clean = !bsums_dirty;
        return trunk_backward(n, ps, P, Gr, S, N, G, accumulate, dfeat, s, two_streams ? n->s2 : nullptr, frozen, fused_tape);
    };
    ocl_net::GraphKey key;
    memset(&key, 0, sizeof(key));
    key.kind = 1; key.N = N; key.G = G; key.slot = slot;
    key.a = (accumulate ? 1 : 0) | (frozen ? 2 : 0) | (fused_tape ? 4 : 0) | (two_streams ? 8 : 0);
    key.b = (repack ? 1 : 0) | (bsums_dirty ? 2 : 0);
    key.c = repack_mask;
    key.p = (uint64_t)(uintptr_t)P;
    rc = two_streams ? body() : run_replayed(n, key, s, body);
    if (repack) {
        n->pack_src = P;
        n->pack_have = repack_mask;
        n->pack_stream = s;
    }
    n->bsums_clean = false;
    return rc;
}

int ocl_test_net_forms(int hw, int nf, int N, int groups, int train, ocl_test_net_form* out, int cap) {
    OCL_REQUIRE(N > 0 && groups > 0 && N % groups == 0 && (train || groups == 1), "test_net_forms: N=%d groups=%d train=%d", N, groups, train);
// ... 108 lines not shown
```

online-continual-learning_amd/ffi.py:

```python
import ctypes as C
import os

import torch

_HERE = os.path.dirname(os.path.abspath(__file__))
LIB_PATH = os.environ.get("OCL_LIB") or os.path.join(_HERE, "libocl_hip.so")
_lib = None

i64 = C.c_int64
i32 = C.c_int32
f32 = C.c_float
vp = C.c_void_p


class NetDesc(C.Structure):
    _fields_ = [("in_h", i32), ("in_w", i32), ("nf", i32), ("n_classes", i32), ("head", i32),
                ("feat_dim", i32), ("max_batch", i32), ("n_slots", i32)]



def _ints(*names):
    return [(n, i32) for n in names]


class TestConvDesc(C.Structure):
    _fields_ = _ints("cin", "cout", "k", "stride", "hin", "win", "n", "groups", "dir", "merge", "xf", "bnb",
                     "force_mt", "force_nt", "force_pipe", "force_q4", "force_cs", "force_cw")


class TestConvForm(C.Structure):
    _fields_ = _ints("family", "mt", "nt", "q4", "pipe", "wres", "ncls", "pf", "bnb_room", "grid_x", "grid_y", "reserved")


class TestConvOps(C.Structure):
    _fields_ = [("in_", vp), ("w", vp), ("out", vp), ("flags", i32), ("xf", i32), ("scale", vp), ("shift", vp), ("res", vp),
                ("resmask", vp), ("stats", vp), ("xf_stats", vp), ("xf_gamma", vp), ("xf_beta", vp), ("xf_save_mean", vp),
                ("xf_save_invstd", vp), ("xf_running_mean", vp), ("xf_running_var", vp), ("xf_nbt", vp), ("bnb_y", vp), ("bnb_z", vp),
                ("bnb_mean", vp), ("bnb_invstd", vp), ("bnb_gamma", vp), ("bnb_beta", vp)]


class TestWgradDesc(C.Structure):
    _fields_ = _ints("cin", "cout", "k", "stride", "hin", "win", "n", "xf_groups", "wg_target", "reserved")


class TestWgradForm(C.Structure):
    _fields_ = _ints("mtw", "ntw", "q_rgw", "pf", "multi", "s", "grid_x", "grid_y")


class TestWgradOps(C.Structure):
    _fields_ = [("x", vp), ("dy", vp), ("grad", vp), ("xf", i32), ("reserved", i32), ("xf_mean", vp), ("xf_invstd", vp),
                ("xf_gamma", vp), ("xf_beta", vp)]


class TestBnFwdArgs(C.Structure):
    _fields_ = [(n, vp) for n in ("y", "z", "res", "stats", "gamma", "beta", "running_mean", "running_var", "nbt", "save_mean",
                                  "save_invstd", "frozen_mean", "frozen_var", "yb", "stats_b", "gamma_b", "beta_b", "running_mean_b",
                                  "running_var_b", "nbt_b", "save_mean_b", "save_invstd_b", "frozen_mean_b", "frozen_var_b")] + \
              [("m_per_group", i64), ("groups", i32), ("c", i32), ("relu", i32), ("momentum", f32), ("eps", f32), ("reserved", i32)]


class TestBnBwdArgs(C.Structure):
    _fields_ = [("dz", vp), ("z", vp)] + [(n, vp * 2) for n in ("y", "mean", "invstd", "gamma", "beta", "dy", "dgamma", "dbeta")] + \
              [("m_per_group", i64)] + _ints("groups", "c", "nsets", "accumulate", "frozen", "mask_from_y", "one_pass", "reserved")


class TestNetForm(C.Structure):
    _fields_ = _ints("layer", "dir", "wg_merged", "reserved") + [("desc", TestConvDesc), ("form", TestConvForm),
                                                                   ("wdesc", TestWgradDesc), ("wform", TestWgradForm)]


class SmallOpPlan(C.Structure):
    _fields_ = [("path", i32), ("aux", i32), ("grid_x", C.c_uint32), ("grid_y", C.c_uint32), ("block", C.c_uint32),
                ("grid2_x", C.c_uint32), ("block2", C.c_uint32), ("reserved", C.c_uint32), ("lds_bytes", i64), ("lds2_bytes", i64)]


SIGNATURES = {
    "ocl_version": (C.c_int, []),
    "ocl_last_error": (C.c_char_p, []),
    "ocl_init": (C.c_int, [C.c_int]),
    "ocl_upload": (C.c_int, [vp, i64, vp, vp]),
    "ocl_gather_rows": (C.c_int, [vp, vp, i64, i64, vp, vp]),
    "ocl_scatter_rows": (C.c_int, [vp, vp, i64, i64, vp, vp]),
    "ocl_gather_rows_pair": (C.c_int, [vp, i64, vp, vp, i64, vp, vp, vp, i64, vp]),
    "ocl_gather_u8_hwc_to_f32_chw": (C.c_int, [vp, vp, i64, C.c_int, C.c_int, C.c_int, vp, vp]),
    "ocl_sgd_step": (C.c_int, [vp, vp, i64, f32, f32, f32, vp, vp]),
    "ocl_ce_fwd_bwd": (C.c_int, [vp, vp, C.c_int, C.c_int, C.c_int, vp, vp, vp]),
    "ocl_ce_segmented_fwd_bwd": (C.c_int, [vp, vp, vp, C.c_int, C.c_int, vp, vp, vp]),
    "ocl_kd_fwd_bwd": (C.c_int, [vp, vp, C.c_int, C.c_int, C.c_float, vp, vp, vp]),
    "ocl_supcon_workspace_bytes": (i64, [C.c_int]),
    "ocl_supcon_fwd_bwd": (C.c_int, [vp, vp, C.c_int, C.c_int, C.c_int, f32, vp, vp, vp, vp]),
    "ocl_knn_sv": (C.c_int, [vp, vp, C.c_int, vp, vp, C.c_int, C.c_int, C.c_int, vp, vp, vp]),
    "ocl_col_reduce": (C.c_int, [vp, C.c_int, C.c_int, C.c_int, vp, vp]),
    "ocl_aser_score": (C.c_int, [vp, C.c_int, vp, C.c_int, C.c_int, C.c_int, vp, vp]),
    "ocl_argsort_desc": (C.c_int, [vp, C.c_int, vp, vp]),
    "ocl_ncm_class_means": (C.c_int, [vp, vp, C.c_int, C.c_int, vp, C.c_int, vp, vp, vp]),
    "ocl_ncm_predict": (C.c_int, [vp, C.c_int, C.c_int, vp, C.c_int, vp, vp]),
    "ocl_mir_scores": (C.c_int, [vp, vp, vp, C.c_int, C.c_int, vp, vp]),
    "ocl_cosine_max_workspace_bytes": (i64, [C.c_int]),
    "ocl_cosine_max": (C.c_int, [vp, C.c_int, i64, vp, f32, vp, vp, vp]),
    "ocl_scr_augment": (C.c_int, [vp, vp, C.c_int, C.c_int, C.c_int, vp, vp]),
    "ocl_scr_augment_uniform": (C.c_int, [vp, vp, C.c_int, C.c_int, C.c_int, vp, C.POINTER(C.c_double), vp, vp]),
    "ocl_gemm_small": (C.c_int, [vp, i64, i64, vp, i64, i64, vp, i64, C.c_int, C.c_int, C.c_int, vp,
                                 C.c_int, C.c_int, vp]),
    "ocl_net_create": (C.c_int, [C.POINTER(NetDesc), C.POINTER(vp)]),
    "ocl_net_destroy": (None, [vp]),
    "ocl_net_param_count": (i64, [vp]),
    "ocl_net_num_tensors": (i32, [vp]),
    "ocl_net_tensor_info": (C.c_int, [vp, C.c_int, C.c_char_p, C.POINTER(i64), C.POINTER(i32),
                                      C.POINTER(i64)]),
    "ocl_net_num_bn": (i32, [vp]),
    "ocl_net_bn_stat_count": (i64, [vp]),
    "ocl_net_bn_info": (C.c_int, [vp, C.c_int, C.c_char_p, C.POINTER(i64), C.POINTER(i32)]),
    "ocl_net_feature_dim": (i32, [vp]),
    "ocl_net_out_dim": (i32, [vp]),
    "ocl_net_workspace_bytes": (i64, [vp]),
    "ocl_net_bind": (C.c_int, [vp, vp, vp, vp, vp, vp, i64]),
    "ocl_net_forward": (C.c_int, [vp, vp, C.c_int, C.c_int, C.c_uint32, vp, vp, vp, C.c_int, vp]),
    "ocl_net_forward_segments": (C.c_int, [vp, C.POINTER(vp), C.POINTER(i32), C.c_int, C.c_int, C.c_uint32, vp, vp, vp, C.c_int, vp]),
    "ocl_net_backward": (C.c_int, [vp, C.c_int, vp, C.c_int, vp]),
    "ocl_net_debug_stop": (C.c_int, [vp, C.c_int]),
    "ocl_net_debug_copy": (C.c_int, [vp, C.c_int, C.c_int, C.c_int, vp, i64, C.POINTER(i64), vp]),
    "ocl_bn_bwd_nhwc": (C.c_int, [vp, vp, vp, vp, vp, vp, i64, C.c_int, C.c_int, vp, vp, vp, C.c_int, vp, vp]),
    "ocl_set_deterministic": (C.c_int, [C.c_int]),
    "ocl_test_conv_plan": (C.c_int, [C.POINTER(TestConvDesc), C.POINTER(TestConvForm), C.c_int]),
    "ocl_test_conv": (C.c_int, [C.POINTER(TestConvDesc), C.POINTER(TestConvOps), C.POINTER(TestConvForm), C.c_int, vp]),
    "ocl_test_wgrad": (C.c_int, [C.POINTER(TestWgradDesc), C.POINTER(TestWgradOps), C.c_int, C.c_int, C.c_int, C.POINTER(TestWgradForm), vp]),
    "ocl_test_bn_fwd": (C.c_int, [C.POINTER(TestBnFwdArgs), vp]),
    "ocl_test_bn_bwd": (C.c_int, [C.POINTER(TestBnBwdArgs), vp]),
    "ocl_test_bn_apply_e": (C.c_int, [vp, vp, vp, vp, vp, vp, i64, C.c_int, C.c_int, vp, vp, vp, C.c_int, vp]),
    "ocl_test_net_forms": (C.c_int, [C.c_int, C.c_int, C.c_int, C.c_int, C.c_int, C.POINTER(TestNetForm), C.c_int]),
    "ocl_test_small_op_path": (C.c_int, [C.c_int, C.POINTER(i64), C.c_int, C.POINTER(SmallOpPlan)]),
    "ocl_prof_enable": (C.c_int, [C.c_int]),
    "ocl_prof_reset": (C.c_int, []),
    "ocl_prof_query": (C.c_int, [C.c_int, C.POINTER(C.c_double), C.POINTER(i64)]),
    "ocl_mfma_calibrate": (C.c_int, [C.c_int, vp, C.POINTER(C.c_double), C.POINTER(C.c_double), vp]),
}

FWD_TRAIN, FWD_SAVE_TAPE, FWD_UPDATE_RUNNING, FWD_FROZEN_BN, FWD_SAME_WEIGHTS, FWD_PACK_ALL = 1, 2, 4, 8, 16, 32


KNOWN_ENV = frozenset("""
OCL_ASER_AUTOGRAD OCL_ASER_PIPELINE OCL_ASER_SPLIT OCL_BNB_EPI OCL_BN_CHAN OCL_BN_FUSED OCL_CBRS_EMULATE OCL_CBRS_VERIFY_EVERY
OCL_CONV_PIPE OCL_CONV_Q4 OCL_CONV_S OCL_CONV_S_NT OCL_CONV_W OCL_CONV_WX OCL_DATA_STREAM OCL_DEBUG_SKIP_BN2FWD OCL_DEBUG_SKIP_SHORTCUT
OCL_DEBUG_SKIP_WGRAD OCL_DETERMINISTIC OCL_DIST_BACKEND OCL_DY_KEEP OCL_GC_FREEZE OCL_GRAPH OCL_GRAPH_VERBOSE OCL_LIB OCL_LOG_PLANS
OCL_PIN OCL_SIDE_EXTRA_MIN OCL_SINGLE_STREAM OCL_WGRAD_ENOUGH OCL_WGRAD_FLUSH OCL_WGRAD_MULTI OCL_WGRAD_MULTI_TARGET OCL_WGRAD_Q
OCL_WGRAD_TARGET""".split())
HARNESS_ENV = frozenset("OCL_NONE OCL_TEST_CASES OCL_TEST_PORT OCL_SHARD_BACKEND OCL_PROBE_STREAM OCL_EAGER_DEVICE OCL_PARITY_REPORT".split())


def unknown_env(environ=None):
    environ = os.environ if environ is None else environ
    return sorted(k for k in environ if k.startswith("OCL_") and k not in KNOWN_ENV and k not in HARNESS_ENV)


def lib():
    global _lib
    if _lib is None:
        dead = unknown_env()
        if dead:
            import warnings
            warnings.warn("environment variables %s are not read by ocl_amd / libocl_hip.so (removed or misspelt switch?): "
                          "they change nothing" % ", ".join(dead), RuntimeWarning, stacklevel=2)
# ... 54 lines not shown
```

Measured before the change: 5127 stream images/s.

## Fuse avgpool into BN kernels, bit-pack ReLU masks, fuse head l2norm-linear

The BN forward kernel now also writes a bit-packed ReLU mask and, for the last block, computes the 4x4 average-pooled features in extra blocks. BN backward reads the bit mask instead of the float activation and rebuilds the pooled gradient on the fly, so the separate avgpool forward and backward kernels are gone. The MLP head backward fuses l2norm backward with the first linear backward and the zero-fill of gradients. This cuts kernel launches and memory traffic for masks, at the cost of more complex kernels and extra index arithmetic in the pooling path.

```diff
diff --git a/include/ocl_hip.h b/include/ocl_hip.h
--- a/include/ocl_hip.h
+++ b/include/ocl_hip.h
@@ -157,6 +157,7 @@
     float *xf_save_mean, *xf_save_invstd, *xf_running_mean, *xf_running_var;
     int64_t* xf_nbt;
     const float *bnb_y, *bnb_z, *bnb_mean, *bnb_invstd, *bnb_gamma, *bnb_beta;
+    const void* resmask_bits;
 } ocl_test_conv_ops;
 int ocl_test_conv(const ocl_test_conv_desc* desc, const ocl_test_conv_ops* ops, ocl_test_conv_form* forms, int cap, void* stream);
 
@@ -184,6 +185,7 @@
     const float* yb; const void* stats_b; const float *gamma_b, *beta_b; float *running_mean_b, *running_var_b; int64_t* nbt_b;
     float *save_mean_b, *save_invstd_b; const float *frozen_mean_b, *frozen_var_b;
     int64_t m_per_group; int32_t groups, c, relu; float momentum, eps; int32_t reserved;
+    void* mask; float* feat; int32_t pool_h, pool_w;
 } ocl_test_bn_fwd_args;
 int ocl_test_bn_fwd(const ocl_test_bn_fwd_args* a, void* stream);
 typedef struct {
@@ -191,10 +193,16 @@
     const float* y[2]; const float* mean[2]; const float* invstd[2]; const float* gamma[2]; const float* beta[2];
     float* dy[2]; float* dgamma[2]; float* dbeta[2];
     int64_t m_per_group; int32_t groups, c, nsets, accumulate, frozen, mask_from_y, one_pass, reserved;
+    const void* zbits; const float* dfeat; float* dz_out; int32_t pool_h, pool_w;
 } ocl_test_bn_bwd_args;
 int ocl_test_bn_bwd(const ocl_test_bn_bwd_args* a, void* stream);
 int ocl_test_bn_apply_e(const float* d, const float* y, const float* mean, const float* invstd, const float* gamma, const void* esums,
                         int64_t m_per_group, int groups, int c, float* dy, float* dgamma, float* dbeta, int accumulate, void* stream);
+
+int ocl_test_head_fwd(const float* x, const float* w, const float* bias, float* h, float* out, float* norms, float* out2, int m, int n,
+                      int k, int fused, void* stream);
+int ocl_test_head_bwd(const float* out, const float* norms, const float* dout, float* dv, const float* w, const float* relu_src,
+                      float* dx, int m, int n, int kin, float* zero, int64_t n_zero, int fused, void* stream);
 
 typedef struct {
     int32_t layer, dir, wg_merged, reserved;
diff --git a/online-continual-learning_amd/csrc/conv.h b/online-continual-learning_amd/csrc/conv.h
--- a/online-continual-learning_amd/csrc/conv.h
+++ b/online-continual-learning_amd/csrc/conv.h
@@ -78,6 +78,7 @@
     const int* blob;
     int off_tdesc, off_pu, off_loc, blob_ints;
     unsigned long long* trace;
+    const uint8_t* resmask_bits;
 };
 
 struct ConvPlan {
@@ -255,7 +256,12 @@
     int64_t* nbt_b;
     float *save_mean_b, *save_invstd_b;
     const float *frozen_mean_b, *frozen_var_b;
-};
+    uint32_t* mask;
+    float* feat;
+    int pool_h, pool_w;
+    int pool_blocks;
+};
+static inline int64_t bn_mask_words(int64_t units_per_group) { return (units_per_group + 7) / 8; }
 int launch_bn_fwd(const BnFwdArgs& a, hipStream_t s);
 int launch_bn_apply_saved(const float* y, const float* mean, const float* invstd, const float* gamma, const float* beta, float* z,
                           int64_t m_per_group, int G, int C, hipStream_t s);
@@ -289,6 +295,10 @@
     int frozen;
     int mask_from_y;
     const float* beta[2];
+    const uint32_t* zbits;
+    const float* dfeat;
+    float* dz_out;
+    int pool_h, pool_w;
 };
 int launch_bn_bwd(const BnBwdArgs& a, hipStream_t s);
 struct BnApplyEArgs {
@@ -315,6 +325,11 @@
 
 int launch_l2norm_fwd(const float* v, float* out, float* norms, int n, int d, hipStream_t s, float* out2 = nullptr);
 int launch_l2norm_bwd(const float* out, const float* norms, const float* dout, float* dv, int n, int d, hipStream_t s);
+bool head_pair_fits(int n, int kin);
+int launch_linear_l2norm_fwd(const float* x, const float* w, const float* bias, float* h, float* out, float* norms, float* out2, int m,
+                             int n, int k, hipStream_t s);
+int launch_l2norm_linear_bwd(const float* out, const float* norms, const float* dout, float* dv, const float* w, const float* relu_src,
+                             float* dx, int m, int n, int kin, float* zero, int64_t n_zero, hipStream_t s);
 int launch_relu_bwd(const float* dy, const float* a, float* dx, int64_t n, hipStream_t s);
 int launch_colsum(const float* m, int rows, int cols, float* out, int accumulate, hipStream_t s);
 int launch_fill(float* p, int64_t n, float v, hipStream_t s);
diff --git a/online-continual-learning_amd/csrc/conv.hip b/online-continual-learning_amd/csrc/conv.hip
--- a/online-continual-learning_amd/csrc/conv.hip
+++ b/online-continual-learning_amd/csrc/conv.hip
@@ -572,9 +572,8 @@
                     v.x += r.x; v.y += r.y; v.z += r.z; v.w += r.w;
                 }
                 if (flags & EPI_RESMASK) {
-                    const float4 r = *(const float4*)(a.res + (int64_t)ooff[nt] + ct.z + co);
-                    const float4 m = *(const float4*)(a.resmask + (int64_t)ooff[nt] + ct.z + co);
-                    v.x += m.x > 0.f ? r.x : 0.f; v.y += m.y > 0.f ? r.y : 0.f; v.z += m.z > 0.f ? r.z : 0.f; v.w += m.w > 0.f ? r.w : 0.f;
+                    const int64_t eo = (int64_t)ooff[nt] + ct.z + co;
+                    add_res_masked(v, *(const float4*)(a.res + eo), a, eo);
                 }
                 if (flags & EPI_ACCUM) {
                     const float4 o = *(const float4*)op;
@@ -864,9 +863,8 @@
                 v.x += r.x; v.y += r.y; v.z += r.z; v.w += r.w;
             }
             if (flags & EPI_RESMASK) {
-                const float4 r = *(const float4*)(a.res + (int64_t)ooff[nt] + co);
-                const float4 mk = *(const float4*)(a.resmask + (int64_t)ooff[nt] + co);
-                v.x += mk.x > 0.f ? r.x : 0.f; v.y += mk.y > 0.f ? r.y : 0.f; v.z += mk.z > 0.f ? r.z : 0.f; v.w += mk.w > 0.f ? r.w : 0.f;
+                const int64_t eo = (int64_t)ooff[nt] + co;
+                add_res_masked(v, *(const float4*)(a.res + eo), a, eo);
             }
             if (flags & EPI_ACCUM) {
                 const float4 o = *(const float4*)op;
@@ -1153,9 +1151,8 @@
             v.x += r.x; v.y += r.y; v.z += r.z; v.w += r.w;
         }
         if (flags & EPI_RESMASK) {
-            const float4 r = *(const float4*)(a.res + (int64_t)oo + co);
-            const float4 mk = *(const float4*)(a.resmask + (int64_t)oo + co);
-            v.x += mk.x > 0.f ? r.x : 0.f; v.y += mk.y > 0.f ? r.y : 0.f; v.z += mk.z > 0.f ? r.z : 0.f; v.w += mk.w > 0.f ? r.w : 0.f;
+            const int64_t eo = (int64_t)oo + co;
+            add_res_masked(v, *(const float4*)(a.res + eo), a, eo);
         }
         if (flags & EPI_ACCUM) {
             const float4 o = *(const float4*)op;
@@ -2070,8 +2067,7 @@
     const float4* b4 = a.yb ? (const float4*)a.yb + (int64_t)g * units : nullptr;
     const float4* r4 = a.res ? (const float4*)a.res + (int64_t)g * units : nullptr;
     float4* z4 = (float4*)a.z + (int64_t)g * units;
-    for (int64_t u = (int64_t)blockIdx.x * 256 + tid; u < units; u += (int64_t)gridDim.x * 256) {
-        const int c = (int)(u % C4) * 4;
+    auto zval = [&](int64_t u, int c) __attribute__((always_inline)) -> float4 {
         float4 v = y4[u];
         v.x = __fmaf_rn(v.x, sc[c], sh[c]);
         v.y = __fmaf_rn(v.y, sc[c + 1], sh[c + 1]);
@@ -2092,15 +2088,65 @@
         if (a.relu) {
             v.x = fmaxf(v.x, 0.f); v.y = fmaxf(v.y, 0.f); v.z = fmaxf(v.z, 0.f); v.w = fmaxf(v.w, 0.f);
         }
-        z4[u] = v;
-    }
-}
-
-int launch_bn_fwd(const BnFwdArgs& a, hipStream_t s) {
+        return v;
+    };
+    const int nstream = (int)gridDim.x - a.pool_blocks;
+    if ((int)blockIdx.x >= nstream) {
+        const int H = a.pool_h, W = a.pool_w, PH = H / 4, PW = W / 4;
+        const int ng = (int)(a.m_per_group / ((int64_t)H * W));
+        const int64_t items = (int64_t)ng * PH * PW * C4;
+        const int64_t D = (int64_t)a.C * PH * PW;
+        for (int i = (int)(blockIdx.x - nstream) * 256 + tid; i < (int)items; i += a.pool_blocks * 256) {
+            int t = i / C4;
+            const int c4 = i - t * C4;
+            const int pw = t % PW; t /= PW;
+            const int ph = t % PH;
+            const int ni = t / PH;
+            float4 sum = make_float4(0.f, 0.f, 0.f, 0.f);
+            for (int dy = 0; dy < 4; ++dy)
+                for (int dx = 0; dx < 4; ++dx) {
+                    const float4 v = zval((((int64_t)ni * H + ph * 4 + dy) * W + pw * 4 + dx) * C4 + c4, c4 * 4);
+                    sum.x += v.x; sum.y += v.y; sum.z += v.z; sum.w += v.w;
+                }
+            float* f = a.feat + ((int64_t)g * ng + ni) * D + (int64_t)c4 * 4 * PH * PW + ph * PW + pw;
+            f[0] = sum.x * (1.0f / 16.0f);
+            f[PH * PW] = sum.y * (1.0f / 16.0f);
+            f[2 * PH * PW] = sum.z * (1.0f / 16.0f);
+            f[3 * PH * PW] = sum.w * (1.0f / 16.0f);
+        }
+        return;
+    }
+    uint32_t* mw = a.mask ? a.mask + (int64_t)g * ((units + 7) >> 3) : nullptr;
+    const int64_t lim = mw ? (units + 7) & ~(int64_t)7 : units;
+    for (int64_t u = (int64_t)blockIdx.x * 256 + tid; u < lim; u += (int64_t)nstream * 256) {
+        unsigned nb = 0u;
+        if (u < units) {
+            const float4 v = zval(u, (int)(u % C4) * 4);
+            z4[u] = v;
+            nb = relu_nibble(v) << ((tid & 7) * 4);
+        }
+        if (mw) {
+            nb |= __shfl_xor(nb, 1, 64);
+            nb |= __shfl_xor(nb, 2, 64);
+            nb |= __shfl_xor(nb, 4, 64);
+            if ((tid & 7) == 0) mw[u >> 3] = nb;
+        }
+    }
+}
+
+int launch_bn_fwd(const BnFwdArgs& a0, hipStream_t s) {
+    BnFwdArgs a = a0;
     const int64_t units = a.m_per_group * (a.C / 4);
     const int bx = (int)std::max<int64_t>(1, std::min<int64_t>(1024, (units + 1023) / 1024));
+    a.pool_blocks = 0;
+    if (a.feat) {
+        OCL_REQUIRE(a.pool_h >= 4 && a.pool_w >= 4 && a.m_per_group % ((int64_t)a.pool_h * a.pool_w) == 0, "bn_fwd: pooled map %d x %d",
+                    a.pool_h, a.pool_w);
+        const int64_t items = a.m_per_group / ((int64_t)a.pool_h * a.pool_w) * (a.pool_h / 4) * (a.pool_w / 4) * (a.C / 4);
+        a.pool_blocks = (int)std::max<int64_t>(1, std::min<int64_t>(64, (items + 255) / 256));
+    }
     ProfScope ps(PROF_BN, s);
-    hipLaunchKernelGGL(bn_fwd_kernel, dim3(bx, a.G), dim3(256), (size_t)a.C * (a.yb ? 16 : 8), s, a);
+    hipLaunchKernelGGL(bn_fwd_kernel, dim3(bx + a.pool_blocks, a.G), dim3(256), (size_t)a.C * (a.yb ? 16 : 8), s, a);
     OCL_LAUNCH_CHECK();
     return OCL_OK;
 }
@@ -2151,7 +2197,30 @@
     return OCL_OK;
 }
 
-template <int U>
+__device__ __forceinline__ float4 pooled_dz(const BnBwdArgs& a, unsigned pix, int c) {
+    const int H = a.pool_h, W = a.pool_w, PH = H / 4, PW = W / 4;
+    const unsigned n = pix / (unsigned)(H * W);
+    const int p = (int)(pix - n * (unsigned)(H * W));
+    const int y = p / W, x = p - y * W;
+    float4 v = make_float4(0.f, 0.f, 0.f, 0.f);
+    if (y < PH * 4 && x < PW * 4) {
+        const float* f = a.dfeat + (int64_t)n * a.C * PH * PW + c * PH * PW + (y >> 2) * PW + (x >> 2);
+        v = make_float4(f[0] * (1.0f / 16.0f), f[PH * PW] * (1.0f / 16.0f), f[2 * PH * PW] * (1.0f / 16.0f), f[3 * PH * PW] * (1.0f / 16.0f));
+    }
+    return v;
+}
+__device__ __forceinline__ float4 bn_load_dz(const BnBwdArgs& a, int64_t U, int C4, bool store = true) {
+    if (!a.dfeat) return ((const float4*)a.dz)[U];
+    const unsigned u32 = (unsigned)U, pix = u32 / (unsigned)C4;
+    const float4 v = pooled_dz(a, pix, (int)(u32 - pix * (unsigned)C4) * 4);
+    if (a.dz_out && store) ((float4*)a.dz_out)[U] = v;
+    return v;
+}
+__device__ __forceinline__ const uint8_t* bn_zbits(const BnBwdArgs& a, int g, int64_t units) {
+    return a.zbits ? (const uint8_t*)(a.zbits + (int64_t)g * ((units + 7) >> 3)) : nullptr;
+}
+
+template <int U, bool POOL = false, bool MASK = false>
 __global__ void __launch_bounds__(256) bn_bwd_reduce_kernel(const BnBwdArgs a) {
     extern __shared__ __attribute__((aligned(16))) float sm[];
     const int C4 = a.C >> 2;
@@ -2177,7 +2246,12 @@
                 istd[k] = *(const float4*)(a.invstd[k] + (int64_t)g * a.C + c4 * 4);
             }
         const float4* dz4 = (const float4*)a.dz + (int64_t)g * M * C4;
-        const float4* z4 = a.z ? (const float4*)a.z + (int64_t)g * M * C4 : nullptr;
+        const uint8_t* zb = MASK ? bn_zbits(a, g, M * C4) : nullptr;
+        const float4* z4 = a.z && !MASK ? (const float4*)a.z + (int64_t)g * M * C4 : nullptr;
+        auto load_z = [&](int64_t e) __attribute__((always_inline)) -> float4 {
+            if (MASK) return make_float4(__uint_as_float(mask_nibble(zb, e)), 0.f, 0.f, 0.f);
+            return z4 ? z4[e] : make_float4(0.f, 0.f, 0.f, 0.f);
+        };
         const float4* y40 = (const float4*)a.y[0] + (int64_t)g * M * C4;
         const float4* y41 = a.nsets > 1 ? (const float4*)a.y[1] + (int64_t)g * M * C4 : y40;
         const int64_t step = (int64_t)PT * C4;
@@ -2192,7 +2266,9 @@
         auto consume = [&](float4 d, float4 zz, const float4& ya, const float4& yb) __attribute__((always_inline)) {
             if (a.mask_from_y)
                 zz = make_float4(__fmaf_rn(ya.x, msc.x, msh.x), __fmaf_rn(ya.y, msc.y, msh.y), __fmaf_rn(ya.z, msc.z, msh.z), __fmaf_rn(ya.w, msc.w, msh.w));
-            if (z4 || a.mask_from_y) {
+            if (MASK) {
+                d = mask_select(__float_as_uint(zz.x), d);
+            } else if (z4 || a.mask_from_y) {
                 d.x = zz.x > 0.f ? d.x : 0.f; d.y = zz.y > 0.f ? d.y : 0.f;
                 d.z = zz.z > 0.f ? d.z : 0.f; d.w = zz.w > 0.f ? d.w : 0.f;
             }
@@ -2208,12 +2284,12 @@
                 }
         };
         const float4 zero4 = make_float4(0.f, 0.f, 0.f, 0.f);
-        for (; e + (U - 1) * step < eend; e += U * step) {
+        for (; !POOL && e + (U - 1) * step < eend; e += U * step) {
             float4 d[U], zz[U], ya[U], yb[U];
 #pragma unroll
             for (int u = 0; u < U; ++u) {
                 d[u] = dz4[e + u * step];
-                zz[u] = z4 ? z4[e + u * step] : zero4;
+                zz[u] = load_z(e + u * step);
                 ya[u] = y40[e + u * step];
                 yb[u] = a.nsets > 1 ? y41[e + u * step] : zero4;
             }
@@ -2221,7 +2297,7 @@
             for (int u = 0; u < U; ++u) consume(d[u], zz[u], ya[u], yb[u]);
         }
         for (; e < eend; e += step)
-            consume(dz4[e], z4 ? z4[e] : zero4, y40[e], a.nsets > 1 ? y41[e] : zero4);
+            consume(POOL ? bn_load_dz(a, (int64_t)g * M * C4 + e, C4) : dz4[e], load_z(e), y40[e], a.nsets > 1 ? y41[e] : zero4);
     }
     float* base = sm;
     if (pl < PT) {
@@ -2284,8 +2360,10 @@
     for (int64_t u = (int64_t)blockIdx.x * 256 + tid; u < units; u += (int64_t)gridDim.x * 256) {
         const int c = (int)(u % C4) * 4;
         const int64_t e = (int64_t)g * units + u;
-        float4 d = ((const float4*)a.dz)[e];
-        if (a.z) {
+        float4 d = a.dfeat ? bn_load_dz(a, e, C4, false) : ((const float4*)a.dz)[e];
+        if (const uint8_t* zb = bn_zbits(a, g, units)) {
+            d = mask_select(mask_nibble(zb, u), d);
+        } else if (a.z) {
             const float4 zz = ((const float4*)a.z)[e];
             d.x = zz.x > 0.f ? d.x : 0.f; d.y = zz.y > 0.f ? d.y : 0.f;
             d.z = zz.z > 0.f ? d.z : 0.f; d.w = zz.w > 0.f ? d.w : 0.f;
@@ -2333,7 +2411,8 @@
     const int64_t M = a.m_per_group;
     const int64_t units = M * C4;
     const float4* dz4 = (const float4*)a.dz + (int64_t)g * units;
-    const float4* z4 = a.z ? (const float4*)a.z + (int64_t)g * units : nullptr;
+    const uint8_t* zb = bn_zbits(a, g, units);
+    const float4* z4 = a.z && !zb ? (const float4*)a.z + (int64_t)g * units : nullptr;
     const bool live = g < a.G && gt < S;
     float4 d[E], xh[NS][E];
     float4 sd = make_float4(0.f, 0.f, 0.f, 0.f), sx[NS];
@@ -2346,10 +2425,11 @@
             const int64_t u = (int64_t)gt + (int64_t)e * S;
             const bool in = u < units;
             const int64_t uu = in ? u : 0;
-            d[e] = dz4[uu];
+            d[e] = a.dfeat ? bn_load_dz(a, (int64_t)g * units + uu, C4, in) : dz4[uu];
 #pragma unroll
             for (int k = 0; k < NS; ++k) xh[k][e] = ((const float4*)a.y[k] + (int64_t)g * units)[uu];
             zz[e] = z4 ? z4[uu] : make_float4(1.f, 1.f, 1.f, 1.f);
+            if (zb) d[e] = mask_select(mask_nibble(zb, uu), d[e]);
             if (!in) d[e] = make_float4(0.f, 0.f, 0.f, 0.f);
         }
         if (a.mask_from_y) {
@@ -2483,6 +2563,7 @@
     const int64_t M = a.m_per_group;
     const float4 f4z = make_float4(0.f, 0.f, 0.f, 0.f);
     const int64_t base = (int64_t)g * M * C4 + c4;
+    const uint8_t* zb = bn_zbits(a, g, M * C4);
     float4 d[E], xh[NS][E], zz[E];
     float4 sd = f4z, sx[NS];
 #pragma unroll
@@ -2492,10 +2573,11 @@
         const int64_t pix = pt + (int64_t)e * T;
         const bool in = pix < M;
         const int64_t u = base + (in ? pix : 0) * C4;
-        d[e] = ((const float4*)a.dz)[u];
+        d[e] = a.dfeat ? bn_load_dz(a, u, C4, in) : ((const float4*)a.dz)[u];
 #pragma unroll
         for (int k = 0; k < NS; ++k) xh[k][e] = ((const float4*)a.y[k])[u];
-        zz[e] = a.z ? ((const float4*)a.z)[u] : make_float4(1.f, 1.f, 1.f, 1.f);
+        zz[e] = a.z && !zb ? ((const float4*)a.z)[u] : make_float4(1.f, 1.f, 1.f, 1.f);
+        if (zb) d[e] = mask_select(mask_nibble(zb, u - (int64_t)g * M * C4), d[e]);
         if (!in) d[e] = f4z;
     }
     if (a.mask_from_y) {
@@ -2602,6 +2684,9 @@
 
 int launch_bn_bwd(const BnBwdArgs& a, hipStream_t s) {
     OCL_REQUIRE(a.nsets == 1 || a.nsets == 2, "bn_bwd: nsets=%d", a.nsets);
+    OCL_REQUIRE(!a.dfeat || (a.pool_h >= 4 && a.pool_w >= 4 && a.m_per_group % ((int64_t)a.pool_h * a.pool_w) == 0),
+                "bn_bwd: pooled map %d x %d", a.pool_h, a.pool_w);
+    OCL_REQUIRE(!(a.zbits && a.mask_from_y), "bn_bwd: a sign mask and mask_from_y");
     const int C4 = a.C / 4, PT = 256 / C4;
     if (g_bn_fused < 0) {
         const char* e = getenv("OCL_BN_FUSED");
@@ -2669,7 +2754,12 @@
     g_bn_bwd_last_path = 3000 + a.nsets;
     const size_t sm1 = (size_t)a.nsets * 2 * PT * a.C * 4;
     if (g_bn_bwd_phase != 2) {
-        if (U == 1) hipLaunchKernelGGL(bn_bwd_reduce_kernel<1>, dim3(bx, a.G), dim3(256), sm1, s, a);
+        if (a.dfeat && a.zbits) hipLaunchKernelGGL((bn_bwd_reduce_kernel<1, true, true>), dim3(bx, a.G), dim3(256), sm1, s, a);
+        else if (a.dfeat) hipLaunchKernelGGL((bn_bwd_reduce_kernel<1, true>), dim3(bx, a.G), dim3(256), sm1, s, a);
+        else if (a.zbits && U == 1) hipLaunchKernelGGL((bn_bwd_reduce_kernel<1, false, true>), dim3(bx, a.G), dim3(256), sm1, s, a);
+        else if (a.zbits && U == 2) hipLaunchKernelGGL((bn_bwd_reduce_kernel<2, false, true>), dim3(bx, a.G), dim3(256), sm1, s, a);
+        else if (a.zbits) hipLaunchKernelGGL((bn_bwd_reduce_kernel<4, false, true>), dim3(bx, a.G), dim3(256), sm1, s, a);
+        else if (U == 1) hipLaunchKernelGGL(bn_bwd_reduce_kernel<1>, dim3(bx, a.G), dim3(256), sm1, s, a);
         else if (U == 2) hipLaunchKernelGGL(bn_bwd_reduce_kernel<2>, dim3(bx, a.G), dim3(256), sm1, s, a);
         else hipLaunchKernelGGL(bn_bwd_reduce_kernel<4>, dim3(bx, a.G), dim3(256), sm1, s, a);
         OCL_LAUNCH_CHECK();
@@ -2867,6 +2957,141 @@
     if (n <= 0) return OCL_OK;
     ProfScope ps(PROF_HEAD, s);
     hipLaunchKernelGGL(fill_kernel, dim3((unsigned)std::min<int64_t>(1024, (n + 255) / 256)), dim3(256), 0, s, p, n, v);
+    OCL_LAUNCH_CHECK();
+    return OCL_OK;
+}
+
+__device__ __forceinline__ f32x4 gemm16_tile(const float* ap, int64_t a_cs, bool av, const float* bp, int64_t b_rs, bool bv, int k, int g) {
+    f32x4 acc = {0.f, 0.f, 0.f, 0.f};
+    int k0 = 0;
+    for (; k0 + 16 <= k; k0 += 16) {
+        float av4[4], bv4[4];
+#pragma unroll
+        for (int u = 0; u < 4; ++u) {
+            const int kk = k0 + u * 4 + g;
+            av4[u] = av ? ap[(int64_t)kk * a_cs] : 0.f;
+            bv4[u] = bv ? bp[(int64_t)kk * b_rs] : 0.f;
+        }
+#pragma unroll
+        for (int u = 0; u < 4; ++u) acc = __builtin_amdgcn_mfma_f32_16x16x4f32(av4[u], bv4[u], acc, 0, 0, 0);
+    }
+    for (; k0 < k; k0 += 4) {
+        const int kk = k0 + g;
+        const float x = (av && kk < k) ? ap[(int64_t)kk * a_cs] : 0.f;
+        const float y = (bv && kk < k) ? bp[(int64_t)kk * b_rs] : 0.f;
+        acc = __builtin_amdgcn_mfma_f32_16x16x4f32(x, y, acc, 0, 0, 0);
+    }
+    return acc;
+}
+
+__global__ void __launch_bounds__(1024) linear_l2norm_fwd_kernel(const float* __restrict__ x, const float* __restrict__ w,
+                                                                 const float* __restrict__ bias, float* __restrict__ h,
+                                                                 float* __restrict__ out, float* __restrict__ norms,
+                                                                 float* __restrict__ out2, int m, int n, int k) {
+    extern __shared__ __attribute__((aligned(16))) float tile[];
+    const int lane = threadIdx.x & 63, wave = threadIdx.x >> 6, nw = blockDim.x >> 6;
+    const int r16 = lane & 15, g = lane >> 4;
+    const int row0 = blockIdx.x * 16, col0 = wave * 16;
+    const int ar = row0 + r16, bc = col0 + r16;
+    const bool av = ar < m, bv = bc < n;
+    const f32x4 acc = gemm16_tile(x + (int64_t)(av ? ar : 0) * k, 1, av, w + (int64_t)(bv ? bc : 0) * k, 1, bv, k, g);
+    if (bv) {
+        const float bs = bias ? bias[bc] : 0.f;
+#pragma unroll
+        for (int r = 0; r < 4; ++r) {
+            const int row = row0 + g * 4 + r;
+            const float v = acc[r] + bs;
+            tile[(g * 4 + r) * n + bc] = v;
+            if (row < m) h[(int64_t)row * n + bc] = v;
+        }
+    }
+    __syncthreads();
+    for (int rr = wave; rr < 16; rr += nw) {
+        const int row = row0 + rr;
+        if (row >= m) break;
+        const float* p = tile + rr * n;
+        float ss = 0.f;
+        for (int j = lane; j < n; j += 64) ss = fmaf(p[j], p[j], ss);
+        ss = wave_sum(ss);
+        const float nrm = fmaxf(sqrtf(ss), 1e-12f);
+        if (lane == 0) norms[row] = nrm;
+        for (int j = lane; j < n; j += 64) {
+            const float q = p[j] / nrm;
+            out[(int64_t)row * n + j] = q;
+            if (out2) out2[(int64_t)row * n + j] = q;
+        }
+    }
+}
+
+__global__ void __launch_bounds__(1024) l2norm_linear_bwd_kernel(const float* __restrict__ out, const float* __restrict__ norms,
+                                                                 const float* __restrict__ dout, float* __restrict__ dv,
+                                                                 const float* __restrict__ w, const float* __restrict__ relu_src,
+                                                                 float* __restrict__ dx, int m, int n, int kin, int row_blocks,
+                                                                 float* __restrict__ zero, int64_t n_zero) {
+    extern __shared__ __attribute__((aligned(16))) float tile[];
+    if ((int)blockIdx.x >= row_blocks) {
+        const int64_t nt = (int64_t)(gridDim.x - row_blocks) * blockDim.x;
+        for (int64_t i = (int64_t)(blockIdx.x - row_blocks) * blockDim.x + threadIdx.x; i < n_zero; i += nt) zero[i] = 0.f;
+        return;
+    }
+    const int lane = threadIdx.x & 63, wave = threadIdx.x >> 6, nw = blockDim.x >> 6;
+    const int row0 = blockIdx.x * 16;
+    for (int rr = wave; rr < 16; rr += nw) {
+        const int row = row0 + rr;
+        if (row >= m) break;
+        const float* o = out + (int64_t)row * n;
+        const float* gd = dout + (int64_t)row * n;
+        float dot = 0.f;
+        for (int j = lane; j < n; j += 64) dot = fmaf(o[j], gd[j], dot);
+        dot = wave_sum(dot);
+        const float inv = 1.0f / norms[row];
+        for (int j = lane; j < n; j += 64) {
+            const float v = (gd[j] - o[j] * dot) * inv;
+            dv[(int64_t)row * n + j] = v;
+            tile[rr * n + j] = v;
+        }
+    }
+    __syncthreads();
+    const int r16 = lane & 15, g = lane >> 4;
+    const int col0 = wave * 16;
+    const int bc = col0 + r16;
+    const bool av = row0 + r16 < m, bv = bc < kin;
+    if (col0 >= kin) return;
+    const f32x4 acc = gemm16_tile(tile + r16 * n, 1, av, w + (bv ? bc : 0), kin, bv, n, g);
+    if (bv) {
+#pragma unroll
+        for (int r = 0; r < 4; ++r) {
+            const int row = row0 + g * 4 + r;
+            if (row < m) {
+                float v = acc[r] + 0.f;
+                if (relu_src) v = relu_src[(int64_t)row * kin + bc] > 0.f ? v : 0.f;
+                dx[(int64_t)row * kin + bc] = v;
+            }
+        }
+    }
+}
+
+bool head_pair_fits(int n, int kin) { return n > 0 && kin > 0 && n <= 256 && kin <= 256; }
+
+int launch_linear_l2norm_fwd(const float* x, const float* w, const float* bias, float* h, float* out, float* norms, float* out2, int m,
+                             int n, int k, hipStream_t s) {
+    OCL_REQUIRE(x && w && h && out && norms && m > 0 && k > 0 && head_pair_fits(n, k), "linear_l2norm_fwd: m=%d n=%d k=%d", m, n, k);
+    ProfScope ps(PROF_HEAD, s);
+    hipLaunchKernelGGL(linear_l2norm_fwd_kernel, dim3(cdiv(m, 16)), dim3(64 * cdiv(n, 16)), (size_t)16 * n * 4, s, x, w, bias, h, out,
+                       norms, out2, m, n, k);
+    OCL_LAUNCH_CHECK();
+    return OCL_OK;
+}
+
+int launch_l2norm_linear_bwd(const float* out, const float* norms, const float* dout, float* dv, const float* w, const float* relu_src,
+                             float* dx, int m, int n, int kin, float* zero, int64_t n_zero, hipStream_t s) {
+    OCL_REQUIRE(out && norms && dout && dv && w && dx && m > 0 && head_pair_fits(n, kin) && (n_zero <= 0 || zero),
+                "l2norm_linear_bwd: m=%d n=%d kin=%d", m, n, kin);
+    ProfScope ps(PROF_HEAD, s);
+    const int row_blocks = cdiv(m, 16), block = 64 * cdiv(kin, 16);
+    const int zero_blocks = n_zero > 0 ? (int)std::min<int64_t>(32, (n_zero + block - 1) / block) : 0;
+    hipLaunchKernelGGL(l2norm_linear_bwd_kernel, dim3(row_blocks + zero_blocks), dim3(block), (size_t)16 * n * 4, s, out, norms, dout, dv,
+                       w, relu_src, dx, m, n, kin, row_blocks, zero, std::max<int64_t>(0, n_zero));
     OCL_LAUNCH_CHECK();
     return OCL_OK;
 }
diff --git a/online-continual-learning_amd/csrc/conv_dev.h b/online-continual-learning_amd/csrc/conv_dev.h
--- a/online-continual-learning_amd/csrc/conv_dev.h
+++ b/online-continual-learning_amd/csrc/conv_dev.h
@@ -41,4 +41,21 @@
     sh = __fmaf_rn(-mean, sc, beta);
 }
 
+__device__ __forceinline__ unsigned relu_nibble(const float4 v) {
+    return (v.x > 0.f ? 1u : 0u) | (v.y > 0.f ? 2u : 0u) | (v.z > 0.f ? 4u : 0u) | (v.w > 0.f ? 8u : 0u);
 }
+__device__ __forceinline__ unsigned mask_nibble(const uint8_t* bits, int64_t u) { return (unsigned)bits[u >> 1] >> ((unsigned)(u & 1) * 4u); }
+__device__ __forceinline__ float4 mask_select(unsigned nb, const float4 d) {
+    return make_float4((nb & 1u) ? d.x : 0.f, (nb & 2u) ? d.y : 0.f, (nb & 4u) ? d.z : 0.f, (nb & 8u) ? d.w : 0.f);
+}
+__device__ __forceinline__ void add_res_masked(float4& v, const float4 r, const ConvArgs& a, int64_t eo) {
+    if (a.resmask_bits) {
+        const float4 t = mask_select(mask_nibble(a.resmask_bits, eo >> 2), r);
+        v.x += t.x; v.y += t.y; v.z += t.z; v.w += t.w;
+    } else {
+        const float4 m = *(const float4*)(a.resmask + eo);
+        v.x += m.x > 0.f ? r.x : 0.f; v.y += m.y > 0.f ? r.y : 0.f; v.z += m.z > 0.f ? r.z : 0.f; v.w += m.w > 0.f ? r.w : 0.f;
+    }
+}
+
+}
diff --git a/online-continual-learning_amd/csrc/convw.hip b/online-continual-learning_amd/csrc/convw.hip
--- a/online-continual-learning_amd/csrc/convw.hip
+++ b/online-continual-learning_amd/csrc/convw.hip
@@ -369,9 +369,8 @@
                         v.x += r.x; v.y += r.y; v.z += r.z; v.w += r.w;
                     }
                     if (flags & EPI_RESMASK) {
-                        const float4 r = *(const float4*)(a.res + (int64_t)ooff[nt] + co);
-                        const float4 m = *(const float4*)(a.resmask + (int64_t)ooff[nt] + co);
-                        v.x += m.x > 0.f ? r.x : 0.f; v.y += m.y > 0.f ? r.y : 0.f; v.z += m.z > 0.f ? r.z : 0.f; v.w += m.w > 0.f ? r.w : 0.f;
+                        const int64_t eo = (int64_t)ooff[nt] + co;
+                        add_res_masked(v, *(const float4*)(a.res + eo), a, eo);
                     }
                     if (flags & EPI_ACCUM) {
                         const float4 o = *(const float4*)op;
@@ -767,9 +766,8 @@
                         v.x += r.x; v.y += r.y; v.z += r.z; v.w += r.w;
                     }
                     if (flags & EPI_RESMASK) {
-                        const float4 r = *(const float4*)(a.res + (int64_t)ooff[nt] + co);
-                        const float4 m = *(const float4*)(a.resmask + (int64_t)ooff[nt] + co);
-                        v.x += m.x > 0.f ? r.x : 0.f; v.y += m.y > 0.f ? r.y : 0.f; v.z += m.z > 0.f ? r.z : 0.f; v.w += m.w > 0.f ? r.w : 0.f;
+                        const int64_t eo = (int64_t)ooff[nt] + co;
+                        add_res_masked(v, *(const float4*)(a.res + eo), a, eo);
                     }
                     if (flags & EPI_ACCUM) {
                         const float4 o = *(const float4*)op;
diff --git a/online-continual-learning_amd/csrc/layer_api.hip b/online-continual-learning_amd/csrc/layer_api.hip
--- a/online-continual-learning_amd/csrc/layer_api.hip
+++ b/online-continual-learning_amd/csrc/layer_api.hip
@@ -167,7 +167,7 @@
         ConvPlan q = p;
         ConvArgs& a = q.a;
         a.in = o->in; a.wT = pack; a.out = o->out; a.flags = o->flags;
-        a.scale = o->scale; a.shift = o->shift; a.res = o->res; a.resmask = o->resmask;
+        a.scale = o->scale; a.shift = o->shift; a.res = o->res; a.resmask = o->resmask; a.resmask_bits = (const uint8_t*)o->resmask_bits;
         a.stats = (StatCell*)o->stats;
         a.stat_rep_stride = (int64_t)gs[i].groups * 2 * (d.dir == 0 ? c.Cout : c.Cin);
         if (o->xf) {
@@ -273,6 +273,7 @@
     a.yb = t->yb; a.stats_b = (const StatCell*)t->stats_b; a.gamma_b = t->gamma_b; a.beta_b = t->beta_b;
     a.running_mean_b = t->running_mean_b; a.running_var_b = t->running_var_b; a.nbt_b = t->nbt_b;
     a.save_mean_b = t->save_mean_b; a.save_invstd_b = t->save_invstd_b; a.frozen_mean_b = t->frozen_mean_b; a.frozen_var_b = t->frozen_var_b;
+    a.mask = (uint32_t*)t->mask; a.feat = t->feat; a.pool_h = t->pool_h; a.pool_w = t->pool_w;
     hipStream_t s = (hipStream_t)stream;
     if ((rc = launch_bn_fwd(a, s)) != OCL_OK) return rc;
     OCL_HIP(hipStreamSynchronize(s));
@@ -280,7 +281,7 @@
 }
 
 int ocl_test_bn_bwd(const ocl_test_bn_bwd_args* t, void* stream) {
-    OCL_REQUIRE(t && t->dz && (t->nsets == 1 || t->nsets == 2) && t->groups >= 1 && t->c % 4 == 0 && t->m_per_group > 0, "test_bn_bwd: bad arguments");
+    OCL_REQUIRE(t && (t->dz || t->dfeat) && (t->nsets == 1 || t->nsets == 2) && t->groups >= 1 && t->c % 4 == 0 && t->m_per_group > 0, "test_bn_bwd: bad arguments");
     for (int k = 0; k < t->nsets; ++k)
         OCL_REQUIRE(t->y[k] && t->mean[k] && t->invstd[k] && t->gamma[k] && t->dy[k] && t->dgamma[k] && t->dbeta[k], "test_bn_bwd: null pointer (set %d)", k);
     OCL_REQUIRE(!t->mask_from_y || (t->nsets == 1 && !t->z && t->beta[0]), "test_bn_bwd: mask_from_y wants one set, no z, beta");
@@ -297,6 +298,7 @@
         a.dy[k] = t->dy[k]; a.dgamma[k] = t->dgamma[k]; a.dbeta[k] = t->dbeta[k];
     }
     a.accumulate = t->accumulate; a.frozen = t->frozen; a.mask_from_y = t->mask_from_y;
+    a.zbits = (const uint32_t*)t->zbits; a.dfeat = t->dfeat; a.dz_out = t->dz_out; a.pool_h = t->pool_h; a.pool_w = t->pool_w;
     const size_t cells = (size_t)t->nsets * t->groups * 2 * t->c;
     a.sums = (StatCell*)sc.take(cells * sizeof(StatCell), 0);
     if (t->one_pass) {
@@ -330,6 +332,40 @@
     return OCL_OK;
 }
 
+int ocl_test_head_fwd(const float* x, const float* w, const float* bias, float* h, float* out, float* norms, float* out2, int m, int n,
+                      int k, int fused, void* stream) {
+    OCL_REQUIRE(x && w && h && out && norms && m > 0 && n > 0 && k > 0, "test_head_fwd: bad arguments");
+    hipStream_t s = (hipStream_t)stream;
+    int rc;
+    if (fused) {
+        rc = launch_linear_l2norm_fwd(x, w, bias, h, out, norms, out2, m, n, k, s);
+    } else {
+        rc = ocl_gemm_small(x, k, 1, w, 1, k, h, n, m, n, k, bias, 0, 0, s);
+        if (rc == OCL_OK) rc = launch_l2norm_fwd(h, out, norms, m, n, s, out2);
+    }
+    if (rc != OCL_OK) return rc;
+    OCL_HIP(hipStreamSynchronize(s));
+    return OCL_OK;
+}
+
+int ocl_test_head_bwd(const float* out, const float* norms, const float* dout, float* dv, const float* w, const float* relu_src, float* dx,
+                      int m, int n, int kin, float* zero, int64_t n_zero, int fused, void* stream) {
+    OCL_REQUIRE(out && norms && dout && dv && w && dx && m > 0 && n > 0 && kin > 0, "test_head_bwd: bad arguments");
+    hipStream_t s = (hipStream_t)stream;
+    int rc;
+    if (fused) {
+        rc = launch_l2norm_linear_bwd(out, norms, dout, dv, w, relu_src, dx, m, n, kin, zero, n_zero, s);
+    } else {
+        rc = n_zero > 0 ? launch_fill(zero, n_zero, 0.f, s) : OCL_OK;
+        if (rc == OCL_OK) rc = launch_l2norm_bwd(out, norms, dout, dv, m, n, s);
+        if (rc == OCL_OK) rc = ocl_gemm_small(dv, n, 1, w, kin, 1, dx, kin, m, kin, n, nullptr, 0, 0, s);
+        if (rc == OCL_OK && relu_src) rc = launch_relu_bwd(dx, relu_src, dx, (int64_t)m * kin, s);
+    }
+    if (rc != OCL_OK) return rc;
+    OCL_HIP(hipStreamSynchronize(s));
+    return OCL_OK;
+}
+
 int ocl_set_deterministic(int on) { return set_deterministic_sums(on); }
 
 }
diff --git a/online-continual-learning_amd/csrc/net.hip b/online-continual-learning_amd/csrc/net.hip
--- a/online-continual-learning_amd/csrc/net.hip
+++ b/online-continual-learning_amd/csrc/net.hip
@@ -41,6 +41,7 @@
 struct BlockInfo {
     int conv1, conv2, convs;
     int64_t a1_off, z_off;
+    int64_t zmask_off;
 };
 
 struct PlanSet {
@@ -67,6 +68,7 @@
 
     int64_t ws_bytes = 0;
     int64_t slot_bytes = 0, slot_base = 0;
+    int64_t zstem_mask_off = 0;
     int64_t x4_off = 0, zstem_off = 0, save_off_base = 0, feat_off = 0, h1_off = 0, h2_off = 0, norms_off = 0, out_off = 0;
     int64_t slot_floats = 0;
     int64_t gbuf_floats = 0;
@@ -275,12 +277,15 @@
         cv.y_off = take(sz);
         max_act = std::max(max_act, sz);
     }
+    auto mask_floats = [&](int64_t sz) { return sz / 32 + kGmax + 1; };
     n->zstem_off = take(N * n->convs[0].Ho * n->convs[0].Wo * n->convs[0].Cout);
+    n->zstem_mask_off = take(mask_floats(N * n->convs[0].Ho * n->convs[0].Wo * n->convs[0].Cout));
     for (auto& b : n->blocks) {
         const ConvInfo& c1 = n->convs[b.conv1];
         const int64_t sz = N * c1.Ho * c1.Wo * c1.Cout;
         b.a1_off = take(sz);
         b.z_off = take(sz);
+        b.zmask_off = take(mask_floats(sz));
     }
     n->save_off_base = o;
     for (auto& b : n->bns) {
@@ -494,7 +499,7 @@
 
 static int run_conv(ocl_net* n, ConvPlan& cached, const float* in, const float* wT, float* out, int flags, StatCell* stats,
                     const float* scale, const float* shift, const float* res, const float* resmask, hipStream_t s, const XfBn* xf = nullptr,
-                    const BnbEpi* be = nullptr) {
+                    const BnbEpi* be = nullptr, const uint8_t* resmask_bits = nullptr) {
     if (!cached.a.blob) {
         int rc = conv_plan_finalize(&cached, &n->plan_arena, s);
         if (rc != OCL_OK) return rc;
@@ -521,6 +526,7 @@
     p.a.shift = shift;
     p.a.res = res;
     p.a.resmask = resmask;
+    p.a.resmask_bits = resmask_bits;
     if (be) {
         if (p.a.bnb_lds < 0) {
             set_error("run_conv: plan has no room for the BatchNorm-backward epilogue");
@@ -540,6 +546,13 @@
     const int FD = n->feat_dim;
     auto T = [&](int t) { return P + n->tensors[t].off; };
     int rc = OCL_OK;
+    auto proj_norm = [&](const float* x) -> int {
+        *wrote_out2 = true;
+        if (head_pair_fits(n->out_dim, FD))
+            return launch_linear_l2norm_fwd(x, T(n->t_h2_w), T(n->t_h2_b), h2, out, norms, out2, N, n->out_dim, FD, s);
+        int r = ocl_gemm_small(x, FD, 1, T(n->t_h2_w), 1, FD, h2, n->out_dim, N, n->out_dim, FD, T(n->t_h2_b), 0, 0, s);
+        return r ? r : launch_l2norm_fwd(h2, out, norms, N, n->out_dim, s, out2);
+    };
     switch (n->d.head) {
         case 0:
             rc = ocl_gemm_small(feat, FD, 1, T(n->t_linear_w), 1, FD, out, n->out_dim, N, n->out_dim, FD, T(n->t_linear_b), 0, 0, s);
@@ -547,16 +560,10 @@
         case 1:
             rc = ocl_gemm_small(feat, FD, 1, T(n->t_h0_w), 1, FD, h1, FD, N, FD, FD, T(n->t_h0_b), 1, 0, s);
             if (rc) return rc;
-            rc = ocl_gemm_small(h1, FD, 1, T(n->t_h2_w), 1, FD, h2, n->out_dim, N, n->out_dim, FD, T(n->t_h2_b), 0, 0, s);
-            if (rc) return rc;
-            rc = launch_l2norm_fwd(h2, out, norms, N, n->out_dim, s, out2);
-            *wrote_out2 = true;
+            rc = proj_norm(h1);
             break;
         case 2:
-            rc = ocl_gemm_small(feat, FD, 1, T(n->t_h2_w), 1, FD, h2, n->out_dim, N, n->out_dim, FD, T(n->t_h2_b), 0, 0, s);
-            if (rc) return rc;
-            rc = launch_l2norm_fwd(h2, out, norms, N, n->out_dim, s, out2);
-            *wrote_out2 = true;
+            rc = proj_norm(feat);
             break;
         default:
             rc = launch_l2norm_fwd(feat, out, norms, N, FD, s, out2);
@@ -754,7 +761,8 @@
     StatCell* stats = n->statsbuf();
     int rc = OCL_OK;
     auto at = [&](int64_t off, const ConvInfo& c) { return S + off + (int64_t)img0 * c.Ho * c.Wo * c.Cout; };
-    auto bn_fwd = [&](int conv_i, const float* y, float* z, const float* res, int relu, hipStream_t st, int conv_b = -1) -> int {
+    auto bn_fwd = [&](int conv_i, const float* y, float* z, const float* res, int relu, hipStream_t st, int conv_b = -1,
+                      int64_t zmask_off = -1, float* pool = nullptr) -> int {
         const ConvInfo& c = n->convs[conv_i];
         const BnInfo& b = n->bns[c.bn];
         BnFwdArgs a;
@@ -772,6 +780,10 @@
         a.m_per_group = (int64_t)(Nc / G) * c.Ho * c.Wo;
         a.G = G; a.C = b.C; a.relu = relu;
         a.momentum = 0.1f; a.eps = 1e-5f;
+        if (zmask_off >= 0) a.mask = (uint32_t*)(S + zmask_off);
+        if (pool) {
+            a.feat = pool; a.pool_h = n->Hf; a.pool_w = n->Wf;
+        }
         if (frozen) {
             a.frozen_mean = n->running + b.stat_off;
             a.frozen_var = n->running + b.stat_off + b.C;
@@ -804,7 +816,8 @@
     const float* x4 = S + n->x4_off + (int64_t)img0 * n->d.in_h * n->d.in_w * 4;
     if ((rc = conv_stats(0, x4, st))) return rc;
     float* cur = at(n->zstem_off, c0);
-    if ((rc = bn_fwd(0, at(c0.y_off, c0), cur, nullptr, 1, st))) return rc;
+    if ((rc = bn_fwd(0, at(c0.y_off, c0), cur, nullptr, 1, st, -1, n->zstem_mask_off))) return rc;
+    bool pooled = false;
     for (auto& b : n->blocks) {
         const ConvInfo& c1 = n->convs[b.conv1];
         const ConvInfo& c2 = n->convs[b.conv2];
@@ -838,10 +851,14 @@
             if ((rc = conv_stats(b.conv2, a1, st))) return rc;
         }
         if (b.convs >= 0 && side && (rc = side_join(n, st))) return rc;
-        if (!(dbg_skip_bn2fwd() && &b != &n->blocks.back()) && (rc = bn_fwd(b.conv2, at(c2.y_off, c2), z, res, 1, st, b.convs))) return rc;
+        const bool last = &b == &n->blocks.back();
+        if (!(dbg_skip_bn2fwd() && !last)) {
+            if ((rc = bn_fwd(b.conv2, at(c2.y_off, c2), z, res, 1, st, b.convs, b.zmask_off, last ? feat : nullptr))) return rc;
+            pooled = last;
+        }
         cur = z;
     }
-    if (!feat) return OCL_OK;
+    if (!feat || pooled) return OCL_OK;
     return launch_avgpool_fwd(cur, feat, Nc, n->Hf, n->Wf, n->convs[n->blocks.back().conv2].Cout, st);
 }
 
@@ -1011,7 +1028,8 @@
     float* gB = nullptr;
     float* gC = nullptr;
     const int Clast = n->convs[n->blocks.back().conv2].Cout;
-    if ((rc = launch_avgpool_bwd(dfeat, gA, Nc, n->Hf, n->Wf, Clast, s))) return rc;
+    const bool pool_in_bn = n->dbg_stop < 0;
+    if (!pool_in_bn && (rc = launch_avgpool_bwd(dfeat, gA, Nc, n->Hf, n->Wf, Clast, s))) return rc;
 
     const bool two_streams = side != nullptr;
     hipStream_t sw = two_streams ? side : s;
@@ -1052,11 +1070,16 @@
         return OCL_OK;
     };
 
-    auto bn_bwd = [&](const float* dz, const float* zmask, int conv_a, float* dya, int conv_b, float* dyb, bool from_y = false) -> int {
+    auto bn_bwd = [&](const float* dz, const float* zmask, int conv_a, float* dya, int conv_b, float* dyb, bool from_y = false,
+                      int64_t zbits_off = -1, float* pool_dz = nullptr) -> int {
         BnBwdArgs a;
         memset(&a, 0, sizeof(a));
         const ConvInfo& ca = n->convs[conv_a];
         a.dz = dz; a.z = zmask;
+        if (zbits_off >= 0) a.zbits = (const uint32_t*)(S + zbits_off);
+        if (pool_dz) {
+            a.dfeat = dfeat; a.dz_out = pool_dz; a.pool_h = n->Hf; a.pool_w = n->Wf;
+        }
         a.mask_from_y = from_y ? 1 : 0;
         a.m_per_group = (int64_t)(Nc / G) * ca.Ho * ca.Wo;
         a.G = G; a.C = ca.Cout;
@@ -1154,11 +1177,11 @@
         return (int)pending.size() >= flush_every ? flush_pending() : OCL_OK;
     };
     auto dgrad = [&](int conv_i, const float* dy, float* dx, const float* res, const float* resmask, int extra_flags,
-                     const BnbEpi* be = nullptr) -> int {
+                     const BnbEpi* be = nullptr, const uint8_t* resmask_bits = nullptr) -> int {
         const ConvInfo& c = n->convs[conv_i];
         for (auto& p : ps->dgrad[conv_i]) {
             int fl = extra_flags | (res ? (resmask ? EPI_RESMASK : EPI_RES) : 0);
-            int r = run_conv(n, p, dy, pack + c.td_off, dx, fl, nullptr, nullptr, nullptr, res, resmask, s, nullptr, be);
+            int r = run_conv(n, p, dy, pack + c.td_off, dx, fl, nullptr, nullptr, nullptr, res, resmask, s, nullptr, be, resmask_bits);
             if (r) return r;
         }
         return OCL_OK;
@@ -1215,7 +1238,9 @@
         if (b.convs >= 0) gC = take_dy(&rC);
         if (prev_epi) {
             if ((rc = bn_apply_e(b.conv2, gA, gB))) return rc;
-        } else if ((rc = bn_bwd(gA, z, b.conv2, gB, b.convs, gC))) return rc;
+        } else if ((rc = bn_bwd(gA, z, b.conv2, gB, b.convs, gC, false, b.zmask_off,
+                                bi == (int)n->blocks.size() - 1 && pool_in_bn ? gA : nullptr)))
+            return rc;
         prev_epi = false;
         if (stop_here(bi, 1)) return OCL_OK;
         if ((rc = publish())) return rc;
@@ -1249,7 +1274,9 @@
             const bool epi2 = ps->dgrad_bnb[b.conv1] && single_target && !frozen && G <= 2 && n->dbg_stop < 0;
             BnbEpi be2;
             if (epi2) be2 = bnb_desc(bi == 0 ? 0 : n->blocks[bi - 1].conv2, xin);
-            if ((rc = dgrad(b.conv1, gB1, gE, gA, z, 0, epi2 ? &be2 : nullptr))) return rc;
+            const int64_t units_g = (int64_t)(Nc / G) * c2.Ho * c2.Wo * (c2.Cout / 4);
+            const uint8_t* zbits = G == 1 || units_g % 8 == 0 ? (const uint8_t*)(S + b.zmask_off) : nullptr;
+            if ((rc = dgrad(b.conv1, gB1, gE, gA, z, 0, epi2 ? &be2 : nullptr, zbits))) return rc;
             prev_epi = epi2;
         }
         if (stop_here(bi, 5)) return OCL_OK;
@@ -1259,7 +1286,7 @@
     float* gS = take_dy(&rS);
     if (prev_epi) {
         if ((rc = bn_apply_e(0, gA, gS))) return rc;
-    } else if ((rc = bn_bwd(gA, at(n->zstem_off, c0), 0, gS, -1, nullptr))) return rc;
+    } else if ((rc = bn_bwd(gA, at(n->zstem_off, c0), 0, gS, -1, nullptr, false, n->zstem_mask_off))) return rc;
     (void)rS;
     if ((rc = flush_pending())) return rc;
     if (two_streams && batched) {
@@ -1377,10 +1404,18 @@
         if (n->d.head == 0) {
             if ((rc = lin_bwd(dout, OD, feat, FD, n->t_linear_w, n->t_linear_b, dfeat))) return rc;
         } else {
-            if (!accumulate) {
-                if ((rc = launch_fill(GT(n->t_linear_w), n->tensors[n->t_linear_w].numel + n->tensors[n->t_linear_b].numel, 0.f, s))) return rc;
-            }
-            if (n->d.head == 1) {
+            float* lin_g = GT(n->t_linear_w);
+            const int64_t lin_n = accumulate ? 0 : n->tensors[n->t_linear_w].numel + n->tensors[n->t_linear_b].numel;
+            const bool pair = n->d.head != 3 && head_pair_fits(OD, FD);
+            if (!pair && lin_n && (rc = launch_fill(lin_g, lin_n, 0.f, s))) return rc;
+            if (n->d.head == 1 && pair) {
+                if ((rc = launch_l2norm_linear_bwd(o, norms, dout, dh2, T(n->t_h2_w), h1, dh1, N, OD, FD, lin_g, lin_n, s))) return rc;
+                if ((rc = lin_bwd(dh2, OD, h1, FD, n->t_h2_w, n->t_h2_b, nullptr))) return rc;
+                if ((rc = lin_bwd(dh1, FD, feat, FD, n->t_h0_w, n->t_h0_b, dfeat))) return rc;
+            } else if (n->d.head == 2 && pair) {
+                if ((rc = launch_l2norm_linear_bwd(o, norms, dout, dh2, T(n->t_h2_w), nullptr, dfeat, N, OD, FD, lin_g, lin_n, s))) return rc;
+                if ((rc = lin_bwd(dh2, OD, feat, FD, n->t_h2_w, n->t_h2_b, nullptr))) return rc;
+            } else if (n->d.head == 1) {
                 if ((rc = launch_l2norm_bwd(o, norms, dout, dh2, N, OD, s))) return rc;
                 if ((rc = lin_bwd(dh2, OD, h1, FD, n->t_h2_w, n->t_h2_b, dh1))) return rc;
                 if ((rc = launch_relu_bwd(dh1, h1, dh1, (int64_t)N * FD, s))) return rc;
diff --git a/online-continual-learning_amd/ffi.py b/online-continual-learning_amd/ffi.py
--- a/online-continual-learning_amd/ffi.py
+++ b/online-continual-learning_amd/ffi.py
@@ -36,7 +36,7 @@
     _fields_ = [("in_", vp), ("w", vp), ("out", vp), ("flags", i32), ("xf", i32), ("scale", vp), ("shift", vp), ("res", vp),
                 ("resmask", vp), ("stats", vp), ("xf_stats", vp), ("xf_gamma", vp), ("xf_beta", vp), ("xf_save_mean", vp),
                 ("xf_save_invstd", vp), ("xf_running_mean", vp), ("xf_running_var", vp), ("xf_nbt", vp), ("bnb_y", vp), ("bnb_z", vp),
-                ("bnb_mean", vp), ("bnb_invstd", vp), ("bnb_gamma", vp), ("bnb_beta", vp)]
+                ("bnb_mean", vp), ("bnb_invstd", vp), ("bnb_gamma", vp), ("bnb_beta", vp), ("resmask_bits", vp)]
 
 
 class TestWgradDesc(C.Structure):
@@ -56,12 +56,14 @@
     _fields_ = [(n, vp) for n in ("y", "z", "res", "stats", "gamma", "beta", "running_mean", "running_var", "nbt", "save_mean",
                                   "save_invstd", "frozen_mean", "frozen_var", "yb", "stats_b", "gamma_b", "beta_b", "running_mean_b",
                                   "running_var_b", "nbt_b", "save_mean_b", "save_invstd_b", "frozen_mean_b", "frozen_var_b")] + \
-              [("m_per_group", i64), ("groups", i32), ("c", i32), ("relu", i32), ("momentum", f32), ("eps", f32), ("reserved", i32)]
+              [("m_per_group", i64), ("groups", i32), ("c", i32), ("relu", i32), ("momentum", f32), ("eps", f32), ("reserved", i32),
+               ("mask", vp), ("feat", vp), ("pool_h", i32), ("pool_w", i32)]
 
 
 class TestBnBwdArgs(C.Structure):
     _fields_ = [("dz", vp), ("z", vp)] + [(n, vp * 2) for n in ("y", "mean", "invstd", "gamma", "beta", "dy", "dgamma", "dbeta")] + \
-              [("m_per_group", i64)] + _ints("groups", "c", "nsets", "accumulate", "frozen", "mask_from_y", "one_pass", "reserved")
+              [("m_per_group", i64)] + _ints("groups", "c", "nsets", "accumulate", "frozen", "mask_from_y", "one_pass", "reserved") + \
+              [("zbits", vp), ("dfeat", vp), ("dz_out", vp), ("pool_h", i32), ("pool_w", i32)]
 
 
 class TestNetForm(C.Structure):
@@ -128,6 +130,8 @@
     "ocl_test_bn_fwd": (C.c_int, [C.POINTER(TestBnFwdArgs), vp]),
     "ocl_test_bn_bwd": (C.c_int, [C.POINTER(TestBnBwdArgs), vp]),
     "ocl_test_bn_apply_e": (C.c_int, [vp, vp, vp, vp, vp, vp, i64, C.c_int, C.c_int, vp, vp, vp, C.c_int, vp]),
+    "ocl_test_head_fwd": (C.c_int, [vp, vp, vp, vp, vp, vp, vp, C.c_int, C.c_int, C.c_int, C.c_int, vp]),
+    "ocl_test_head_bwd": (C.c_int, [vp, vp, vp, vp, vp, vp, vp, C.c_int, C.c_int, C.c_int, vp, i64, C.c_int, vp]),
     "ocl_test_net_forms": (C.c_int, [C.c_int, C.c_int, C.c_int, C.c_int, C.c_int, C.POINTER(TestNetForm), C.c_int]),
     "ocl_test_small_op_path": (C.c_int, [C.c_int, C.POINTER(i64), C.c_int, C.POINTER(SmallOpPlan)]),
     "ocl_prof_enable": (C.c_int, [C.c_int]),
```

New measurement: 5062 stream images/s. 1.3% lower.
